# saholmes/stark-mlwe

Measured on AMD Instinct MI355X. Metric: prove ms + Fr-NTT achieved GB/s, 2^20/2^24 trace at 1/2/4/8 GPUs, higher is better.
Workload: dtype u256 (4x u64 Montgomery limbs, Pallas Fr); 1 GPU; one 2^20-row trace x 4 columns (2^20 rows per GPU), blowup 8: LDE (iNTT + coset NTT) + DEEP-ALI merge + FRI folds + Poseidon leaf hashes + Poseidon-Merkle trees (schedule [16,16,8]), kernels only; log_trace_per_gpu=20, log_blowup=3, field=pallas_fr

## Files before the change

stark_mlwe_amd/csrc/capi_core.hip:

```cpp
#include <algorithm>
#include <cstring>
#include "poseidon_launch.hpp"
#include "pow_table.hpp"

using namespace stark;

namespace stark {

static int32_t pool_poison_fill(stark_ctx* ctx, void* p, size_t bytes) {
    STARK_HIP(ctx, hipMemsetAsync(p, ctx->opt.pool_poison, bytes, ctx->stream));
    STARK_HIP(ctx, hipStreamSynchronize(ctx->stream));
    return STARK_OK;
}

int32_t ctx_scratch(stark_ctx* ctx, size_t bytes, void** out) {
    if (bytes > ctx->scratch_bytes) {
        if (ctx->scratch) STARK_HIP(ctx, hipStreamSynchronize(ctx->stream));
        ctx->scratch_bytes = 0; STARK_HIP(ctx, ctx->scratch.alloc(bytes)); ctx->scratch_bytes = bytes;
    }
    if (ctx->opt.pool_poison >= 0 && ctx->scratch_bytes) STARK_TRY(pool_poison_fill(ctx, ctx->scratch.p, ctx->scratch_bytes));
    *out = ctx->scratch.p; return STARK_OK;
}

int32_t ctx_upload_staged(stark_ctx* ctx, void* dst, const void* src, size_t bytes) {
    if (!bytes) return STARK_OK;
    auto& q = ctx->staged;
    for (size_t i = 0; i < q.size();) {
        if (hipEventQuery(q[i].done) == hipSuccess) { (void)hipEventDestroy(q[i].done); q[i] = std::move(q.back()); q.pop_back(); } else ++i;
    }
    (void)hipGetLastError();
    stark_ctx::StagedUpload u; u.host.reset(new uint8_t[bytes]); memcpy(u.host.get(), src, bytes);
    STARK_HIP(ctx, hipEventCreateWithFlags(&u.done, hipEventDisableTiming));
    const uint8_t* from = u.host.get();
    q.push_back(std::move(u));
    STARK_HIP(ctx, hipMemcpyAsync(dst, from, bytes, hipMemcpyHostToDevice, ctx->stream));
    STARK_HIP(ctx, hipEventRecord(q.back().done, ctx->stream));
    return STARK_OK;
}

static inline size_t pool_round(size_t bytes) {
    if (bytes < 256) return 256;
    if (bytes <= (1u << 20)) { size_t r = 256; while (r < bytes) r <<= 1; return r; }
    return (bytes + (1u << 20) - 1) & ~(size_t)((1u << 20) - 1);
}
int32_t ctx_alloc(stark_ctx* ctx, size_t bytes, void** out) {
    const size_t sz = pool_round(bytes);
    auto it = ctx->pool_free.find(sz);
    if (it != ctx->pool_free.end() && !it->second.empty()) {
        void* p = it->second.back(); it->second.pop_back(); ctx->pool_cached_bytes -= sz;
        ctx->pool_live[p] = sz; *out = p;
        return ctx->opt.pool_poison >= 0 ? pool_poison_fill(ctx, p, sz) : STARK_OK;
    }
    void* p = nullptr; hipError_t e = hipMalloc(&p, sz);
    if (e != hipSuccess) {
        (void)hipGetLastError();
        (void)hipStreamSynchronize(ctx->stream);
        for (auto& kv : ctx->pool_free) { for (void* q : kv.second) (void)hipFree(q); kv.second.clear(); }
        ctx->pool_cached_bytes = 0;
        e = hipMalloc(&p, sz);
        if (e != hipSuccess) { (void)hipGetLastError(); return ctx->fail(STARK_ERR_OOM, "device allocation of " + std::to_string(sz) + " bytes failed"); }
    }
    ctx->pool_live[p] = sz; *out = p;
    return ctx->opt.pool_poison >= 0 ? pool_poison_fill(ctx, p, sz) : STARK_OK;
}
void ctx_release(stark_ctx* ctx, void* p) {
    if (!p || !ctx) return;
    auto it = ctx->pool_live.find(p);
    if (it == ctx->pool_live.end()) { ctx->err = "ctx_release: the pointer is not a live block of this context's pool (left alone)"; return; }
    const size_t sz = it->second; ctx->pool_live.erase(it);
    ctx->pool_free[sz].push_back(p); ctx->pool_cached_bytes += sz;
}
int32_t ctx_enter(stark_ctx* ctx) {
    if (!ctx) return STARK_ERR_INVALID_ARG;
    int cur = -1;
    if (hipGetDevice(&cur) != hipSuccess || cur != ctx->device) STARK_HIP(ctx, hipSetDevice(ctx->device));
    return STARK_OK;
}

int32_t ctx_side_stream(stark_ctx* ctx, hipStream_t* out) {
    if (!ctx->side_stream) { STARK_HIP(ctx, hipStreamCreateWithFlags(&ctx->side_stream, hipStreamNonBlocking)); STARK_HIP(ctx, hipEventCreateWithFlags(&ctx->ev_fork, hipEventDisableTiming)); }
    *out = ctx->side_stream; return STARK_OK;
}
int32_t ctx_fork(stark_ctx* ctx, hipStream_t* side) {
    STARK_TRY(ctx_side_stream(ctx, side));
    if (hipEventRecord(ctx->ev_fork, ctx->stream) != hipSuccess || hipStreamWaitEvent(*side, ctx->ev_fork, 0) != hipSuccess) return ctx->fail(STARK_ERR_HIP, "fork");
    return STARK_OK;
}
int32_t ctx_join(stark_ctx* ctx) {
    if (hipEventRecord(ctx->ev_fork, ctx->side_stream) != hipSuccess || hipStreamWaitEvent(ctx->stream, ctx->ev_fork, 0) != hipSuccess) return ctx->fail(STARK_ERR_HIP, "join");
    return STARK_OK;
}

static int32_t params_finish(stark_ctx* ctx, stark_params* P) {
    if (host::rp_for_width(P->ref.t) < 0) return ctx->fail(STARK_ERR_UNSUPPORTED, "Poseidon width must be one of 9,17,33,65,129");
    P->kc = host::make_kernel_consts(P->ref);
    if (!P->kc.ok) return ctx->fail(STARK_ERR_UNSUPPORTED, "MDS matrix has a singular leading minor: LU/sparse kernel form unavailable");
    const host::KernelConsts& k = P->kc;
    std::vector<fr_t> blob; auto put = [&](const std::vector<fr_t>& v) { size_t off = blob.size(); blob.insert(blob.end(), v.begin(), v.end()); return off; };
    size_t o_rcf = put(k.rc_full), o_rcp = put(k.rc_partial), o_lu = put(k.lu), o_pre = put(k.lu_pre), o_row0 = put(k.row0), o_sp = put(k.sparse), o_mds = put(k.mds), o_mpre = put(k.mds_pre), o_gam = put(k.gamma);
    const size_t o_29 = blob.size();
    { std::vector<uint32_t> w29; for (auto* v : {&k.lu29, &k.lu_pre29, &k.row0_29, &k.sparse29, &k.gamma29, &k.mds29, &k.mds_pre29, &k.chain_a, &k.chain_g, &k.chain_w, &k.rc_full29}) w29.insert(w29.end(), v->begin(), v->end());
      while (w29.size() % 8) w29.push_back(0);
      blob.resize(o_29 + w29.size() / 8); memcpy((void*)(blob.data() + o_29), w29.data(), w29.size() * 4); }
    const size_t o_frag = blob.size(), frag_elems = (k.mds_frag.size() + sizeof(fr_t) - 1) / sizeof(fr_t);
    if (!k.mds_frag.empty()) { blob.resize(o_frag + 2 * frag_elems); memcpy((void*)(blob.data() + o_frag), k.mds_frag.data(), k.mds_frag.size()); memcpy((void*)(blob.data() + o_frag + frag_elems), k.mds_pre_frag.data(), k.mds_pre_frag.size()); }
    const size_t o_b8 = blob.size(), ef_elems = (k.blk8s_efrag.size() + sizeof(fr_t) - 1) / sizeof(fr_t), lf_bytes = k.blk8s_lfrag.size() + 1024, lf_elems = (lf_bytes + sizeof(fr_t) - 1) / sizeof(fr_t),
                 gf_elems = (k.blk8s_gfrag.size() + sizeof(fr_t) - 1) / sizeof(fr_t), rcs_elems = k.rc_partial_scaled.size(), un_elems = (k.blk8_unscale29.size() * 4 + sizeof(fr_t) - 1) / sizeof(fr_t);
    const bool have_b8 = !k.blk8s_efrag.empty();
    if (have_b8) { blob.resize(o_b8 + ef_elems + lf_elems + gf_elems + rcs_elems + un_elems);
                   int8_t* const b8 = (int8_t*)(blob.data() + o_b8);
                   memcpy(b8, k.blk8s_efrag.data(), k.blk8s_efrag.size());
                   memcpy(b8 + ef_elems * sizeof(fr_t), k.blk8s_lfrag.data(), k.blk8s_lfrag.size()); memcpy(b8 + ef_elems * sizeof(fr_t) + k.blk8s_lfrag.size(), k.blk8_lfrag.data() + k.blk8_lfrag.size() - 1024, 1024);
                   memcpy(b8 + (ef_elems + lf_elems) * sizeof(fr_t), k.blk8s_gfrag.data(), k.blk8s_gfrag.size());
                   memcpy(b8 + (ef_elems + lf_elems + gf_elems) * sizeof(fr_t), k.rc_partial_scaled.data(), rcs_elems * sizeof(fr_t));
                   memcpy(b8 + (ef_elems + lf_elems + gf_elems + rcs_elems) * sizeof(fr_t), k.blk8_unscale29.data(), k.blk8_unscale29.size() * 4); }
    STARK_TRY(P->blob.fill_sync(ctx, blob.data(), blob.size() * sizeof(fr_t)));
    fr_t* const dev = P->blob.fr();
    P->dev.t = k.t; P->dev.rf = k.rf; P->dev.rp = k.rp;
    P->dev.rc_full = dev + o_rcf; P->dev.rc_partial = dev + o_rcp; P->dev.lu = dev + o_lu; P->dev.lu_pre = dev + o_pre;
    P->dev.row0 = dev + o_row0; P->dev.sparse = dev + o_sp; P->dev.mds = dev + o_mds; P->dev.mds_pre = dev + o_mpre; P->dev.gamma = dev + o_gam;
    { const uint32_t* b29 = reinterpret_cast<const uint32_t*>(dev + o_29);
      P->dev.lu29 = b29; P->dev.lu_pre29 = b29 + k.lu29.size(); P->dev.row0_29 = P->dev.lu_pre29 + k.lu_pre29.size();
      P->dev.sparse29 = P->dev.row0_29 + k.row0_29.size(); P->dev.gamma29 = P->dev.sparse29 + k.sparse29.size();
      P->dev.mds29 = P->dev.gamma29 + k.gamma29.size(); P->dev.mds_pre29 = P->dev.mds29 + k.mds29.size();
      const uint32_t* ch = P->dev.mds_pre29 + k.mds_pre29.size();
      P->dev.chain_a = k.chain_a.empty() ? nullptr : ch; P->dev.chain_g = k.chain_a.empty() ? nullptr : ch + k.chain_a.size(); P->dev.chain_w = k.chain_a.empty() ? nullptr : ch + k.chain_a.size() + k.chain_g.size();
      P->dev.rc_full29 = ch + k.chain_a.size() + k.chain_g.size() + k.chain_w.size(); }
    P->dev.blk8_efrag = have_b8 ? (const void*)(dev + o_b8) : nullptr; P->dev.blk8_lfrag = have_b8 ? (const void*)(dev + o_b8 + ef_elems) : nullptr;
    P->dev.blk8_gfrag = have_b8 ? (const void*)(dev + o_b8 + ef_elems + lf_elems) : nullptr;
    P->dev.blk8_unit_frag = have_b8 ? (const void*)((const int8_t*)P->dev.blk8_lfrag + k.blk8s_lfrag.size()) : nullptr;
    P->dev.rc_partial_scaled = have_b8 ? dev + o_b8 + ef_elems + lf_elems + gf_elems : nullptr;
    P->dev.mds_frag = k.mds_frag.empty() ? nullptr : (const void*)(dev + o_frag); P->dev.mds_pre_frag = k.mds_frag.empty() ? nullptr : (const void*)(dev + o_frag + frag_elems);
    return STARK_OK;
}
static int32_t params_from_consts(stark_ctx* ctx, const host::PoseidonConsts& c, std::unique_ptr<stark_params>& out) {
    std::unique_ptr<stark_params> P(new stark_params()); P->ctx = ctx; P->ref = c;
    STARK_TRY(params_finish(ctx, P.get()));
    out = std::move(P); return STARK_OK;
}
static int32_t params_for_caller(stark_ctx* ctx, const host::PoseidonConsts& c, stark_params** out) {
    std::unique_ptr<stark_params> P; STARK_TRY(params_from_consts(ctx, c, P));
    P->ref_.bind(ctx); *out = P.release(); return STARK_OK;
}
int32_t ctx_transcript_params(stark_ctx* ctx, stark_params** out) {
    if (!ctx->tparams) STARK_TRY(params_from_consts(ctx, host::consts_transcript(), ctx->tparams));
    if (out) *out = ctx->tparams.get();
    return STARK_OK;
}
int32_t ctx_merkle_params(stark_ctx* ctx, int t, stark_params** out) {
    auto it = ctx->merkle_params.find(t);
    if (it == ctx->merkle_params.end()) {
        if (host::rp_for_width(t) < 0) return ctx->fail(STARK_ERR_UNSUPPORTED, "unsupported Poseidon width");
        std::unique_ptr<stark_params> P; STARK_TRY(params_from_consts(ctx, host::consts_for_width(t), P));
        *out = P.get(); ctx->merkle_params[t] = std::move(P); return STARK_OK;
    }
    *out = it->second.get(); return STARK_OK;
}
int32_t ctx_commit_params(stark_ctx* ctx, stark_params** out) {
    std::unique_ptr<stark_params>& slot = ctx->merkle_params[-17];
    if (!slot) STARK_TRY(params_from_consts(ctx, host::derive_consts("POSEIDON-T17-X5-SEED", 17, 8, 64), slot));
    *out = slot.get(); return STARK_OK;
}

}

extern "C" {

int32_t stark_version(void) { return 1; }

int32_t stark_ctx_create(int32_t device, void* stream, stark_ctx_t** out) {
    if (!out) return STARK_ERR_INVALID_ARG;
    int ndev = 0;
    if (hipGetDeviceCount(&ndev) != hipSuccess || ndev <= 0 || device < 0 || device >= ndev) return STARK_ERR_HIP;
    if (hipSetDevice(device) != hipSuccess) return STARK_ERR_HIP;
    std::unique_ptr<stark_ctx> c(new stark_ctx()); c->device = device;
    if (stream == STARK_STREAM_PRIVATE) { if (hipStreamCreateWithFlags(&c->stream, hipStreamNonBlocking) != hipSuccess) return STARK_ERR_HIP; c->own_stream = true; }
    else { c->stream = (hipStream_t)stream; c->own_stream = false; }
    if (hipEventCreate(&c->ev0) != hipSuccess || hipEventCreate(&c->ev1) != hipSuccess) return STARK_ERR_HIP;
    { int cus = 0; if (hipDeviceGetAttribute(&cus, hipDeviceAttributeMultiprocessorCount, device) == hipSuccess && cus > 0) c->num_cus = cus; }
    stark::ntt_set_attrs();
    stark::poseidon_set_attrs();
    *out = c.release(); return STARK_OK;
}
}
static void ctx_teardown(stark_ctx* ctx) {
    (void)hipSetDevice(ctx->device); (void)hipStreamSynchronize(ctx->stream);
    stark::comm_destroy(ctx);
    stark::ntt_plans_free(ctx);
    for (auto& kv : ctx->pool_free) for (void* q : kv.second) (void)hipFree(q);
    for (auto& kv : ctx->pool_live) (void)hipFree(kv.first);
    if (ctx->pinned) (void)hipHostFree(ctx->pinned);
    for (auto& u : ctx->staged) (void)hipEventDestroy(u.done);
    if (ctx->ev0) (void)hipEventDestroy(ctx->ev0); if (ctx->ev1) (void)hipEventDestroy(ctx->ev1);
    if (ctx->side_stream) (void)hipStreamDestroy(ctx->side_stream);
    if (ctx->ev_fork) (void)hipEventDestroy(ctx->ev_fork);
    if (ctx->own_stream) (void)hipStreamDestroy(ctx->stream);
    delete ctx;
}
namespace stark {
void ctx_ref(stark_ctx* c) { ++c->live_handles; }
void ctx_unref(stark_ctx* c) { if (--c->live_handles == 0 && c->destroy_pending) ctx_teardown(c); }
}
extern "C" {
int32_t stark_ctx_destroy(stark_ctx_t* ctx) {
    if (!ctx) return STARK_ERR_INVALID_ARG;
    if (ctx->destroy_pending) return STARK_ERR_INVALID_ARG;
    STARK_TRY(ctx_enter(ctx));
    (void)hipStreamSynchronize(ctx->stream);
    if (ctx->live_handles > 0) { ctx->destroy_pending = true; return STARK_OK; }
    ctx_teardown(ctx); return STARK_OK;
}
int32_t stark_ctx_sync(stark_ctx_t* ctx) { if (!ctx) return STARK_ERR_INVALID_ARG; STARK_TRY(ctx_enter(ctx)); STARK_HIP(ctx, hipStreamSynchronize(ctx->stream)); return STARK_OK; }
int32_t stark_ctx_trim(stark_ctx_t* ctx) {
    if (!ctx) return STARK_ERR_INVALID_ARG; STARK_TRY(ctx_enter(ctx));
    STARK_HIP(ctx, hipStreamSynchronize(ctx->stream));
    for (auto& kv : ctx->pool_free) { for (void* q : kv.second) (void)hipFree(q); kv.second.clear(); }
    ctx->pool_cached_bytes = 0;
    stark::ntt_plans_free(ctx);
    ctx->scratch.reset(); ctx->scratch_bytes = 0;
    return STARK_OK;
}
size_t stark_ctx_cached_bytes(stark_ctx_t* ctx) { return ctx ? ctx->pool_cached_bytes : 0; }
}
struct OptionDef { const char* key; const char* (*set)(stark_ctx::Options&, int64_t); };
static const OptionDef kOptions[] = {
    {"ntt_direct_max_log", [](stark_ctx::Options& o, int64_t v) -> const char* { if (v < 0 || v > 30) return "0..30"; o.ntt_direct_max_log = (int)v; return nullptr; }},
    {"ntt_merged_coset", [](stark_ctx::Options& o, int64_t v) -> const char* { o.ntt_merged_coset = v != 0; return nullptr; }},
    {"ntt_log_tile", [](stark_ctx::Options& o, int64_t v) -> const char* { if (v != -1 && (v < 8 || v > 12)) return "8..12, or -1 for the default"; o.ntt_log_tile_forced = v != -1; o.ntt_log_tile = v == -1 ? 11 : (int)v; return nullptr; }},
    {"ntt_min_waves", [](stark_ctx::Options& o, int64_t v) -> const char* { if (v != 2 && v != 4) return "2 or 4"; o.ntt_min_waves = (int)v; return nullptr; }},
    {"poseidon_lane_only", [](stark_ctx::Options& o, int64_t v) -> const char* { o.poseidon_lane_only = v != 0; return nullptr; }},
    {"sponge_one_wave", [](stark_ctx::Options& o, int64_t v) -> const char* { o.sponge_one_wave = v != 0; return nullptr; }},
    {"sponge_debug", [](stark_ctx::Options& o, int64_t v) -> const char* { o.sponge_debug = (int)v; return nullptr; }},
    {"merkle_node16_pair", [](stark_ctx::Options& o, int64_t v) -> const char* { o.merkle_node16_pair = v != 0; return nullptr; }},
    {"poseidon_block8", [](stark_ctx::Options& o, int64_t v) -> const char* { o.poseidon_block8 = v != 0; return nullptr; }},
    {"merkle_wave_pair", [](stark_ctx::Options& o, int64_t v) -> const char* { o.merkle_wave_pair = v != 0; return nullptr; }},
    {"fri_side_pair", [](stark_ctx::Options& o, int64_t v) -> const char* { o.fri_side_pair = v != 0; return nullptr; }},
    {"sumcheck_verify_batch_max_slots", [](stark_ctx::Options& o, int64_t v) -> const char* { if (v < 1) return "at least 1"; o.sumcheck_verify_batch_max_slots = (size_t)v; return nullptr; }},
    {"ntt_batch_max_elems", [](stark_ctx::Options& o, int64_t v) -> const char* { if (v < 1 || v > ((int64_t)1 << 28)) return "1..2^28"; o.ntt_batch_max_elems = (size_t)v; return nullptr; }},
    {"prove_batch_max_rows", [](stark_ctx::Options& o, int64_t v) -> const char* { if (v < 1 || v > ((int64_t)1 << 28)) return "1..2^28"; o.prove_batch_max_rows = (size_t)v; return nullptr; }},
    {"mle_log_tile", [](stark_ctx::Options& o, int64_t v) -> const char* { if (v != -1 && (v < 3 || v > 12)) return "3..12, or -1 for the default"; o.mle_log_tile = (int)v; return nullptr; }},
    {"mle_lane_contiguous", [](stark_ctx::Options& o, int64_t v) -> const char* { if (v < -1 || v > 1) return "0 or 1, or -1 for the default"; o.mle_lane_contiguous = (int)v; return nullptr; }},
    {"lagrange_max_partials", [](stark_ctx::Options& o, int64_t v) -> const char* { if (v != -1 && (v < 1 || v > ((int64_t)1 << 28))) return "1..2^28, or -1 for the default"; o.lagrange_max_partials = v == -1 ? (size_t)1 << 21 : (size_t)v; return nullptr; }},
    {"lagrange_wide_acc", [](stark_ctx::Options& o, int64_t v) -> const char* { if (v < -1 || v > 1) return "0 or 1, or -1 for the default"; o.lagrange_wide_acc = (int)v; return nullptr; }},
    {"lagrange_col_groups", [](stark_ctx::Options& o, int64_t v) -> const char* { if (v != -1 && (v < 1 || v > 65535)) return "1..65535, or -1 for automatic"; o.lagrange_col_groups = (int)v; return nullptr; }},
    {"pool_poison", [](stark_ctx::Options& o, int64_t v) -> const char* { if (v < -1 || v > 255) return "0..255, or -1 for off"; o.pool_poison = (int)v; return nullptr; }},
};
extern "C" {
int32_t stark_ctx_set_option(stark_ctx_t* ctx, const char* key, int64_t value) {
    if (!ctx || !key) return STARK_ERR_INVALID_ARG;
    STARK_TRY(ctx_enter(ctx));
    const std::string k(key);
    const OptionDef* def = nullptr; std::string known;
    for (const OptionDef& d : kOptions) { if (k == d.key) def = &d; known += (known.empty() ? "" : ", ") + std::string(d.key); }
    if (!def) return ctx->fail(STARK_ERR_INVALID_ARG, "unknown option '" + k + "' (" + known + ")");
    if (const char* range = def->set(ctx->opt, value)) return ctx->fail(STARK_ERR_INVALID_ARG, k + ": " + range);
    STARK_HIP(ctx, hipStreamSynchronize(ctx->stream));
    stark::ntt_plans_free(ctx);
    return STARK_OK;
}
const char* stark_last_error(stark_ctx_t* ctx) { return ctx ? ctx->err.c_str() : "null context"; }
int32_t stark_malloc(stark_ctx_t* ctx, size_t bytes, void** dptr) { if (!ctx || !dptr) return STARK_ERR_INVALID_ARG; STARK_TRY(ctx_enter(ctx)); STARK_HIP(ctx, hipMalloc(dptr, bytes ? bytes : 32)); return STARK_OK; }
int32_t stark_free(stark_ctx_t* ctx, void* dptr) { if (!ctx) return STARK_ERR_INVALID_ARG; STARK_TRY(ctx_enter(ctx)); STARK_HIP(ctx, hipStreamSynchronize(ctx->stream)); STARK_HIP(ctx, hipFree(dptr)); return STARK_OK; }
int32_t stark_memcpy_h2d(stark_ctx_t* ctx, void* d, const void* s, size_t bytes) {
    if (!ctx) return STARK_ERR_INVALID_ARG;
    STARK_TRY(ctx_enter(ctx));
    return DevMem::fill_sync(ctx, d, s, bytes); }
int32_t stark_memcpy_d2h(stark_ctx_t* ctx, void* d, const void* s, size_t bytes) {
    if (!ctx) return STARK_ERR_INVALID_ARG;
    STARK_TRY(ctx_enter(ctx));
    STARK_HIP(ctx, hipMemcpyAsync(d, s, bytes, hipMemcpyDeviceToHost, ctx->stream)); STARK_HIP(ctx, hipStreamSynchronize(ctx->stream)); return STARK_OK; }
int32_t stark_timer_start(stark_ctx_t* ctx) { if (!ctx) return STARK_ERR_INVALID_ARG; STARK_HIP(ctx, hipEventRecord(ctx->ev0, ctx->stream)); return STARK_OK; }
int32_t stark_timer_stop_ms(stark_ctx_t* ctx, float* ms) {
    if (!ctx || !ms) return STARK_ERR_INVALID_ARG;
    STARK_TRY(ctx_enter(ctx));
    STARK_HIP(ctx, hipEventRecord(ctx->ev1, ctx->stream)); STARK_HIP(ctx, hipEventSynchronize(ctx->ev1)); STARK_HIP(ctx, hipEventElapsedTime(ms, ctx->ev0, ctx->ev1)); return STARK_OK; }

}
#define STARK_DIAG_ITERS 2048
static __global__ void __launch_bounds__(1024) k_diag_mac_rate(uint32_t* out, uint32_t seed) {
    uint32_t a0 = seed + threadIdx.x, a1 = a0 * 3 + 1, a2 = a0 * 5 + 2, a3 = a0 * 7 + 3, a4 = a0 * 9 + 4, a5 = a0 * 11 + 5, a6 = a0 * 13 + 6, a7 = a0 * 15 + 7;
    uint64_t d0 = a0, d1 = a1, d2 = a2, d3 = a3, d4 = a4, d5 = a5, d6 = a6, d7 = a7; const uint32_t b = seed | 1;
#define STARK_DIAG_MAD(i) asm volatile("v_mad_u64_u32 %0, vcc, %1, %2, %0" : "+v"(d##i) : "v"(a##i), "v"(b) : "vcc");
    for (int i = 0; i < STARK_DIAG_ITERS; ++i) { STARK_DIAG_MAD(0) STARK_DIAG_MAD(1) STARK_DIAG_MAD(2) STARK_DIAG_MAD(3) STARK_DIAG_MAD(4) STARK_DIAG_MAD(5) STARK_DIAG_MAD(6) STARK_DIAG_MAD(7) }
#undef STARK_DIAG_MAD
// ... 52 lines not shown
```

stark_mlwe_amd/csrc/capi_poseidon.hip:

```cpp
#include <algorithm>
#include <cstring>
#include <type_traits>
#include "poseidon_launch.hpp"
#include "poseidon_dev.hpp"
#include "poseidon_pair.hpp"
#include "poseidon_coop.hpp"
#include "poseidon_chain.hpp"
#include "poseidon_wave.hpp"
#include "poseidon_transcript.hpp"
#include "fri_dev.hpp"
#include "merkle_batch.hpp"

using namespace stark;

static const size_t kMaxLds = 160 * 1024;
static inline int poseidon_block(int t) { return (size_t)t * 32 * 64 <= kMaxLds ? 64 : 32; }
static inline size_t poseidon_lds(int t, int block) { return (size_t)t * 32 * block; }
enum class PoseidonForm { Lane, WavePair, OneWave, FiveWave, Wide };
enum class PoseidonOp { MerkleLevel, LeafLayer, TrHash, ColumnSponges, RaggedSponges, DeviceTranscript };
constexpr size_t kChainMaxNodes = 256, kChainMaxLeaves = 2048, kChainMaxSponges = 512, kCoopMaxNodes = 4096, kCoopMaxLeaves = 4096, kCoopMaxSponges = 4096;
static PoseidonForm poseidon_form(const stark_ctx* ctx, const stark_params* p, PoseidonOp op, size_t n) {
    const PoseidonDev& d = p->dev;
    const bool lane_only = ctx->opt.poseidon_lane_only, one_wave = ctx->opt.sponge_one_wave;
    const bool chain = !lane_only && !one_wave && d.t == 17 && d.rf == 8 && d.rp == 64 && d.chain_a;
// ... 35 lines not shown
        stark_params* tp = nullptr; STARK_TRY(ctx_transcript_params(ctx, &tp));
        const host::PoseidonConsts& c = tp->ref;
        fr_t blob[17 + 51 + 40];
        for (auto& x : blob) x = host::h_zero();
        for (int j = 0; j < 17; ++j) blob[j] = init[j];
        fr_t x[17]; for (int j = 0; j < 17; ++j) x[j] = fr_pow5<PallasFr>(host::h_add(init[j], c.rc_full[j]));
        for (int i = 0; i < 17; ++i) {
            fr_t k = host::h_zero();
            for (int j = 0; j < 17; ++j) if (j != 4 && j != 5) k = host::h_add(k, host::h_mul(c.mds[(size_t)i * 17 + j], x[j]));
            blob[17 + i] = k; blob[34 + i] = c.mds[(size_t)i * 17 + 4]; blob[51 + i] = c.mds[(size_t)i * 17 + 5];
            uint32_t* m45 = reinterpret_cast<uint32_t*>(&blob[68]);
            const fr_t k20 = fr_from_u64<PallasFr>(1ull << FR29_SBOX_SHIFT);
            fr29_const_from<PallasFr>(host::h_mul(c.mds[(size_t)i * 17 + 4], k20), m45 + 9 * i); fr29_const_from<PallasFr>(host::h_mul(c.mds[(size_t)i * 17 + 5], k20), m45 + 9 * (17 + i));
        }
        DevMem d; STARK_TRY(d.fill_sync(ctx, blob, sizeof(blob)));
        ctx->leaf_init = std::move(d);
    }
    *out = ctx->leaf_init.fr(); return STARK_OK;
}

namespace stark {

static int32_t tr_frame(stark_ctx* ctx, const char* tag, fr_t** dev, int* np, int* ns) {
    const std::string key(tag);
    auto it = ctx->tr_frames.find(key);
    if (it == ctx->tr_frames.end()) {
        std::vector<fr_t> fr; const int p = host::tr_hash_frame(tag, fr);
        DevMem d; STARK_TRY(d.fill_sync(ctx, fr.data(), fr.size() * sizeof(fr_t)));
        it = ctx->tr_frames.emplace(key, std::move(d)).first; ctx->tr_frame_dims[key] = {p, (int)fr.size() - p};
    }
    *dev = it->second.fr(); *np = ctx->tr_frame_dims[key].first; *ns = ctx->tr_frame_dims[key].second; return STARK_OK;
}
static int32_t launch_tr_hash(stark_ctx* ctx, stark_params* tp, PoseidonForm form, const TrStream& T, fr_t* out_dev) {
    const bool ragged = T.layout == TrStream::Ragged;
    switch (form) {
    case PoseidonForm::FiveWave:
        if (ragged) hipLaunchKernelGGL(k_tr_hash_chain_ragged, dim3((unsigned)T.n), dim3(320), chain_lds_bytes(), ctx->stream, tp->dev, T, row_consts_of(ctx), out_dev);
        else hipLaunchKernelGGL(k_tr_hash_chain, dim3((unsigned)T.n), dim3(320), chain_lds_bytes(), ctx->stream, tp->dev, T, row_consts_of(ctx), out_dev);
        break;
    case PoseidonForm::OneWave:
        if (ragged) hipLaunchKernelGGL((k_tr_hash_coop<true, true>), dim3((unsigned)T.n), dim3(64), coop_lds_bytes(17), ctx->stream, tp->dev, T, out_dev);
        else if (T.layout == TrStream::Equal) hipLaunchKernelGGL(k_tr_hash_coop<false>, dim3((unsigned)T.n), dim3(64), coop_lds_bytes(17), ctx->stream, tp->dev, T, out_dev);
        else hipLaunchKernelGGL(k_tr_hash_coop<true>, dim3((unsigned)T.n), dim3(64), coop_lds_bytes(17), ctx->stream, tp->dev, T, out_dev);
        break;
    default: {
        const int block = 64;
        if (ragged) hipLaunchKernelGGL(k_tr_hash_ragged, dim3((unsigned)((T.n + block - 1) / block)), dim3(block), poseidon_lds(17, block), ctx->stream, tp->dev, T, out_dev);
        else hipLaunchKernelGGL(k_tr_hash, dim3((unsigned)((T.n + block - 1) / block)), dim3(block), poseidon_lds(17, block), ctx->stream, tp->dev, T, out_dev);
    } }
    STARK_HIP(ctx, hipGetLastError());
    return STARK_OK;
}
int32_t tr_hash_dev(stark_ctx* ctx, const char* tag, const fr_t* fields_dev, size_t k, size_t n, fr_t* out_dev) {
    stark_params* tp = nullptr; STARK_TRY(ctx_transcript_params(ctx, &tp));
    fr_t* frame = nullptr; int np = 0, ns = 0; STARK_TRY(tr_frame(ctx, tag, &frame, &np, &ns));
    if (n == 0) return STARK_OK;
    const TrStream T = TrStream::equal(frame, np, ns, fields_dev, k, n, host::h_tag("FSv1-TRANSCRIPT-INIT"));
    return launch_tr_hash(ctx, tp, poseidon_form(ctx, tp, PoseidonOp::TrHash, n), T, out_dev);
}
static int32_t tr_hash_columns(stark_ctx* ctx, const char* const tags[4], const fr_t* const cols[4], const fr_t* const* ptrs_dev, size_t nblocks, size_t n0, fr_t* out_dev) {
    stark_params* tp = nullptr; STARK_TRY(ctx_transcript_params(ctx, &tp));
    TrStream T{}; T.layout = ptrs_dev ? TrStream::BatchColumns : TrStream::Columns; T.n = nblocks; T.batch = ptrs_dev; T.cap = host::h_tag("FSv1-TRANSCRIPT-INIT");
    for (int c = 0; c < 4; ++c) {
        fr_t* frame = nullptr; int np = 0, ns = 0; STARK_TRY(tr_frame(ctx, tags[c], &frame, &np, &ns));
        T.prefix[c] = frame; T.np[c] = np; T.suffix[c] = frame + np; T.ns[c] = ns; T.fields[c] = cols ? cols[c] : nullptr; T.k[c] = n0;
    }
    return launch_tr_hash(ctx, tp, poseidon_form(ctx, tp, PoseidonOp::ColumnSponges, nblocks), T, out_dev);
}
int32_t tr_hash_columns4_dev(stark_ctx* ctx, const char* const tags[4], const fr_t* const cols[4], size_t n0, fr_t* out4_dev) {
    return tr_hash_columns(ctx, tags, cols, nullptr, 4, n0, out4_dev);
}
int32_t tr_hash_columns_batch_dev(stark_ctx* ctx, const char* const tags[4], const fr_t* const* ptrs_dev, size_t batch, size_t n0, fr_t* out_dev) {
    return tr_hash_columns(ctx, tags, nullptr, ptrs_dev, 4 * batch, n0, out_dev);
}
int32_t tr_hash_many_dev(stark_ctx* ctx, size_t n, const char* const* tags, const fr_t* const* fields, const size_t* k, fr_t* out_dev, bool column_sponges) {
    stark_params* tp = nullptr; STARK_TRY(ctx_transcript_params(ctx, &tp));
    std::vector<TrFrameRef> fr(n);
    for (size_t i = 0; i < n; ++i) { fr_t* frame = nullptr; STARK_TRY(tr_frame(ctx, tags[i], &frame, &fr[i].np, &fr[i].ns)); fr[i].frame = frame; }
    if (n == 0) return STARK_OK;
    if (n > 0x7fffffffu) return ctx->fail(STARK_ERR_UNSUPPORTED, "tr_hash_many: more than 2^31 - 1 items in one call");
    const std::vector<TrStream::Item> items = tr_ragged_items(fr.data(), fields, k, n);
    DevBuf d; STARK_HIP(ctx, d.alloc(ctx, n * sizeof(TrStream::Item))); STARK_TRY(ctx_upload_staged(ctx, d.p, items.data(), n * sizeof(TrStream::Item)));
    const TrStream T = tr_ragged_stream((const TrStream::Item*)d.p, n, host::h_tag("FSv1-TRANSCRIPT-INIT"));
    return launch_tr_hash(ctx, tp, poseidon_form(ctx, tp, column_sponges ? PoseidonOp::ColumnSponges : PoseidonOp::RaggedSponges, n), T, out_dev);
}
int32_t tr_hash_host1(stark_ctx* ctx, const char* tag, const std::vector<fr_t>& fields, fr_t* out) {
    DevBuf in, o; STARK_HIP(ctx, in.alloc(ctx, fields.size() * sizeof(fr_t))); STARK_HIP(ctx, o.alloc(ctx, sizeof(fr_t)));
    STARK_TRY(ctx_upload_staged(ctx, in.p, fields.data(), fields.size() * sizeof(fr_t)));
    STARK_TRY(tr_hash_dev(ctx, tag, in.fr(), fields.size(), 1, o.fr()));
    STARK_HIP(ctx, o.download_sync(out, sizeof(fr_t)));
    return STARK_OK;
}
int32_t tr_stream_on(stark_ctx* ctx, stark_params* tp, fr_t* state, uint32_t* pos, const fr_t* fields, size_t n, bool finish, fr_t* out) {
    if (poseidon_form(ctx, tp, PoseidonOp::DeviceTranscript, 1) == PoseidonForm::FiveWave)
        hipLaunchKernelGGL(k_tr_stream_chain, dim3(1), dim3(320), chain_lds_bytes(), ctx->stream, tp->dev, row_consts_of(ctx), state, pos, fields, (uint64_t)n, finish ? 1 : 0, finish ? out : (fr_t*)nullptr);
    else
        hipLaunchKernelGGL(k_tr_stream, dim3(1), dim3(64), coop_lds_bytes(17), ctx->stream, tp->dev, state, pos, fields, (uint64_t)n, finish ? 1 : 0, finish ? out : (fr_t*)nullptr);
    STARK_HIP(ctx, hipGetLastError()); return STARK_OK;
}
int32_t tr_batch_on(stark_ctx* ctx, stark_params* tp, const TrBatchStream& T, size_t n_for_form) {
    if (!T.n_active) return STARK_OK;
    if (poseidon_form(ctx, tp, PoseidonOp::DeviceTranscript, n_for_form) == PoseidonForm::FiveWave)
        for (uint32_t sg = 0; sg < (uint32_t)T.nseg; ++sg)
            hipLaunchKernelGGL(k_tr_batch_chain, dim3((unsigned)T.n_active), dim3(320), chain_lds_bytes(), ctx->stream, tp->dev, row_consts_of(ctx), T, sg);
    else
        hipLaunchKernelGGL(k_tr_batch, dim3((unsigned)T.n_active), dim3(64), coop_lds_bytes(17), ctx->stream, tp->dev, T);
    STARK_HIP(ctx, hipGetLastError()); return STARK_OK;
}

}

extern "C" {

int32_t stark_poseidon_permute_batch_dev(stark_ctx_t* ctx, stark_params_t* p, uint64_t* states, size_t n) {
    if (!ctx || !p || (!states && n)) return STARK_ERR_INVALID_ARG;
    STARK_TRY(ctx_enter(ctx));
    if (!n) return STARK_OK;
    const int block = poseidon_block(p->dev.t);
    hipLaunchKernelGGL(k_permute_batch, dim3((unsigned)((n + block - 1) / block)), dim3(block), poseidon_lds(p->dev.t, block), ctx->stream, p->dev, as_fr(states), n);
    STARK_HIP(ctx, hipGetLastError()); return STARK_OK;
}
int32_t stark_poseidon_permute_batch(stark_ctx_t* ctx, stark_params_t* p, uint64_t* states, size_t n) {
    if (!ctx || !p || (!states && n)) return STARK_ERR_INVALID_ARG;
    STARK_TRY(ctx_enter(ctx));
    size_t bytes = n * p->dev.t * sizeof(fr_t); DevBuf d; CallerUploads up(ctx); STARK_HIP(ctx, up.up(d, states, bytes));
    STARK_TRY(stark_poseidon_permute_batch_dev(ctx, p, (uint64_t*)d.p, n));
    STARK_HIP(ctx, up.download_sync(states, d.p, bytes));
    return STARK_OK;
}
static int32_t hash_stream(stark_ctx_t* ctx, stark_params_t* p, int mode, const uint64_t* a, size_t na, const uint64_t* b, size_t nb, const fr_t& tag, size_t n, uint64_t* out) {
    DevBuf da, db, dout; CallerUploads up(ctx);
    STARK_HIP(ctx, up.up(da, a, n * na * sizeof(fr_t))); STARK_HIP(ctx, up.up(db, b, n * nb * sizeof(fr_t))); STARK_HIP(ctx, dout.alloc(ctx, n * sizeof(fr_t)));
    const int block = poseidon_block(p->dev.t);
    hipLaunchKernelGGL(k_hash_stream, dim3((unsigned)((n + block - 1) / block)), dim3(block), poseidon_lds(p->dev.t, block), ctx->stream, p->dev, mode, da.fr(), na, db.fr(), nb, tag, n, dout.fr());
    STARK_HIP(ctx, hipGetLastError());
    STARK_HIP(ctx, up.download_sync(out, dout.p, n * sizeof(fr_t)));
    return STARK_OK;
}
int32_t stark_poseidon_hash_with_ds_dynamic(stark_ctx_t* ctx, stark_params_t* p, const uint64_t* ds, size_t nds, const uint64_t* in, size_t cnt, size_t n, uint64_t* out) {
    if (!ctx || !p || !out || (!ds && nds) || (!in && cnt)) return STARK_ERR_INVALID_ARG;
    STARK_TRY(ctx_enter(ctx));
    if (!n) return STARK_OK;
    return hash_stream(ctx, p, 0, ds, nds, in, cnt, host::h_zero(), n, out);
}
int32_t stark_poseidon_hash_with_ds(stark_ctx_t* ctx, stark_params_t* p, const uint64_t* in, size_t cnt, const uint64_t* ds_tag, uint64_t* out) {
    if (!ctx || !p || !out || !ds_tag || (!in && cnt)) return STARK_ERR_INVALID_ARG;
    STARK_TRY(ctx_enter(ctx));
    if (p->dev.t != 17) return ctx->fail(STARK_ERR_INVALID_ARG, "hash_with_ds is the fixed t=17 sponge");
    return hash_stream(ctx, p, 1, nullptr, 0, in, cnt, load_fr(ds_tag), 1, out);
}
}
static int32_t pair_block8_form(stark_ctx* ctx, const stark_params* p, bool* on) {
    *on = ctx->opt.poseidon_block8 && p->dev.t == 17 && p->dev.rp % 8 == 0;
    if (*on && (!p->dev.blk8_efrag || !p->dev.blk8_lfrag || !p->dev.blk8_unit_frag || !p->dev.blk8_gfrag || !p->dev.rc_partial_scaled)) return ctx->fail(STARK_ERR_UNSUPPORTED, "poseidon_block8: the parameter set has no block-8 tables");
    return STARK_OK;
}
template <class DS>
static int32_t launch_ds(stark_ctx_t* ctx, hipStream_t st, stark_params_t* p, const DS& D, fr_t* out) {
    if (!D.n_out) return STARK_OK;
    const int t = p->dev.t; const unsigned nodes = (unsigned)D.n_out, pairs = (unsigned)((D.n_out + 63) / 64);
    bool b8 = false; STARK_TRY(pair_block8_form(ctx, p, &b8));
    switch (poseidon_form(ctx, p, PoseidonOp::MerkleLevel, D.n_out)) {
    case PoseidonForm::FiveWave: hipLaunchKernelGGL(k_hash_ds_chain<DS>, dim3(nodes), dim3(320), chain_lds_bytes(), st, p->dev, D, row_consts_of(ctx), out); break;
    case PoseidonForm::OneWave:
        if (t == 17) hipLaunchKernelGGL((k_hash_ds_coop<17, DS>), dim3(nodes), dim3(64), coop_lds_bytes(17), st, p->dev, D, out);
        else hipLaunchKernelGGL((k_hash_ds_coop<9, DS>), dim3(nodes), dim3(64), coop_lds_bytes(9), st, p->dev, D, out);
        break;
    case PoseidonForm::WavePair:
        if constexpr (std::is_same<DS, DsStream>::value) {
            if (t == 17 && ctx->opt.merkle_node16_pair && D.mode == 0 && D.arity == 16 && D.n_in == 16 * D.n_out) {
                if (b8) hipLaunchKernelGGL(k_node16_pair<true>, dim3(pairs), dim3(128), pair_lds_bytes(17), st, p->dev, D.arity_f, D.level_f, D.label_f, D.pos0, D.in0, D.n_out, out);
                else hipLaunchKernelGGL(k_node16_pair<false>, dim3(pairs), dim3(128), pair_lds_bytes(17), st, p->dev, D.arity_f, D.level_f, D.label_f, D.pos0, D.in0, D.n_out, out);
                break;
            }
        }
        if (t == 17 && b8) hipLaunchKernelGGL((k_hash_ds2<17, DS, true>), dim3(pairs), dim3(128), pair_lds_bytes(17), st, p->dev, D, out);
        else if (t == 17) hipLaunchKernelGGL((k_hash_ds2<17, DS>), dim3(pairs), dim3(128), pair_lds_bytes(17), st, p->dev, D, out);
        else hipLaunchKernelGGL((k_hash_ds2<9, DS>), dim3(pairs), dim3(128), pair_lds_bytes(9), st, p->dev, D, out);
        break;
    case PoseidonForm::Wide:
        if (t == 33) hipLaunchKernelGGL((k_hash_ds_wave<33, DS>), dim3(nodes), dim3(64), wave_lds_bytes(t), st, p->dev, D, out);
        else if (t == 65) hipLaunchKernelGGL((k_hash_ds_wave<65, DS>), dim3(nodes), dim3(64), wave_lds_bytes(t), st, p->dev, D, out);
        else hipLaunchKernelGGL((k_hash_ds_wave<129, DS>), dim3(nodes), dim3(64), wave_lds_bytes(t), st, p->dev, D, out);
        break;
    case PoseidonForm::Lane: {
        const int block = poseidon_block(t);
        hipLaunchKernelGGL(k_hash_ds<DS>, dim3((unsigned)((D.n_out + block - 1) / block)), dim3(block), poseidon_lds(t, block), st, p->dev, D, out);
    } }
    STARK_HIP(ctx, hipGetLastError()); return STARK_OK;
}
int32_t stark::hash_ds_on(stark_ctx* ctx, hipStream_t st, stark_params* p, const DsStream& D, fr_t* out) { return launch_ds(ctx, st, p, D, out); }
int32_t stark::hash_ds_on(stark_ctx* ctx, hipStream_t st, stark_params* p, const DsGatherStream& D, fr_t* out) { return launch_ds(ctx, st, p, D, out); }
int32_t stark::hash_ds_on(stark_ctx* ctx, hipStream_t st, stark_params* p, const DsBatchStream& D, fr_t* out) { return launch_ds(ctx, st, p, D, out); }
int32_t stark::hash_ds_on(stark_ctx* ctx, hipStream_t st, stark_params* p, const DsBatchPairStream& D, fr_t* out) { return launch_ds(ctx, st, p, D, out); }
int32_t stark::hash_ds_on(stark_ctx* ctx, hipStream_t st, stark_params* p, const DsBatchPairPtrStream& D, fr_t* out) { return launch_ds(ctx, st, p, D, out); }
static void lds_attr(const void* kernel) { (void)hipFuncSetAttribute(kernel, hipFuncAttributeMaxDynamicSharedMemorySize, (int)kMaxLds); }
template <class DS>
static void ds_attrs() {
    lds_attr((const void*)k_hash_ds<DS>); lds_attr((const void*)k_hash_ds2<17, DS>); lds_attr((const void*)k_hash_ds2<17, DS, true>); lds_attr((const void*)k_hash_ds2<9, DS>); lds_attr((const void*)k_hash_ds_chain<DS>);
}
void stark::poseidon_set_attrs() {
    ds_attrs<DsStream>(); ds_attrs<DsGatherStream>(); ds_attrs<DsBatchStream>(); ds_attrs<DsBatchPairStream>(); ds_attrs<DsBatchPairPtrStream>();
    for (const void* k : {(const void*)k_leaf_pair, (const void*)k_permute_batch, (const void*)k_tr_hash, (const void*)k_hash_stream, (const void*)k_leaf_pair2<false>, (const void*)k_leaf_pair2<true>, (const void*)k_node16_pair<false>, (const void*)k_node16_pair<true>,
                          (const void*)k_tr_hash_chain, (const void*)k_tr_hash_chain_ragged, (const void*)k_tr_hash_ragged, (const void*)k_leaf_pair_chain, (const void*)k_tr_stream_chain, (const void*)k_tr_batch_chain})
        lds_attr(k);
}
extern "C" {
int32_t stark_poseidon_hash_ds_batch_dev(stark_ctx_t* ctx, stark_params_t* p, size_t arity, uint32_t level, uint64_t pos0, uint64_t label, const uint64_t* in, size_t n_in, uint64_t* out) {
    if (!ctx || !p || !in || !out || arity == 0) return STARK_ERR_INVALID_ARG;
    STARK_TRY(ctx_enter(ctx));
    if (host::width_for_arity(arity) != p->dev.t) return ctx->fail(STARK_ERR_INVALID_ARG, "arity incompatible with Poseidon width");
    STARK_TRY(ctx_enter(ctx));
    return hash_ds_on(ctx, ctx->stream, p, DsStream::make(0, arity, level, pos0, label, as_fr(in), nullptr, n_in), as_fr(out));
}
int32_t stark_poseidon_hash_ds_batch(stark_ctx_t* ctx, stark_params_t* p, size_t arity, uint32_t level, uint64_t pos0, uint64_t label, const uint64_t* in, size_t n_in, uint64_t* out) {
    if (!ctx || !p || !in || !out || arity == 0) return STARK_ERR_INVALID_ARG;
    STARK_TRY(ctx_enter(ctx));
    size_t n_out = (n_in + arity - 1) / arity; DevBuf di, dout; CallerUploads up(ctx); STARK_HIP(ctx, up.up(di, in, n_in * sizeof(fr_t))); STARK_HIP(ctx, dout.alloc(ctx, n_out * sizeof(fr_t)));
    STARK_TRY(stark_poseidon_hash_ds_batch_dev(ctx, p, arity, level, pos0, label, (const uint64_t*)di.p, n_in, (uint64_t*)dout.p));
    STARK_HIP(ctx, up.download_sync(out, dout.p, n_out * sizeof(fr_t)));
    return STARK_OK;
}
}
namespace stark {
static bool same_consts(const host::PoseidonConsts& a, const host::PoseidonConsts& b) {
    if (a.t != b.t || a.rf != b.rf || a.rp != b.rp || a.mds.size() != b.mds.size() || a.rc_full.size() != b.rc_full.size() || a.rc_partial.size() != b.rc_partial.size()) return false;
    for (size_t i = 0; i < a.mds.size(); ++i) if (!fr_eq(a.mds[i], b.mds[i])) return false;
    for (size_t i = 0; i < a.rc_full.size(); ++i) if (!fr_eq(a.rc_full[i], b.rc_full[i])) return false;
    for (size_t i = 0; i < a.rc_partial.size(); ++i) if (!fr_eq(a.rc_partial[i], b.rc_partial[i])) return false;
    return true;
}
int32_t leaf_pair_hash_on(stark_ctx* ctx, hipStream_t st, const fr_t* f, const fr_t* f_next, size_t n, size_t m, fr_t* h) {
    if (!n) return STARK_OK;
    stark_params* tp = nullptr; STARK_TRY(ctx_transcript_params(ctx, &tp));
    fr_t* init = nullptr; STARK_TRY(ctx_leaf_init(ctx, &init));
    const LeafStream L{init, f, f_next, m, n};
    bool b8 = false; STARK_TRY(pair_block8_form(ctx, tp, &b8));
    switch (poseidon_form(ctx, tp, PoseidonOp::LeafLayer, n)) {
    case PoseidonForm::FiveWave: hipLaunchKernelGGL(k_leaf_pair_chain, dim3((unsigned)n), dim3(320), chain_lds_bytes(), st, tp->dev, row_consts_of(ctx), L, h); break;
    case PoseidonForm::OneWave: hipLaunchKernelGGL(k_leaf_pair_coop, dim3((unsigned)n), dim3(64), coop_lds_bytes(17), st, tp->dev, L, h); break;
    case PoseidonForm::WavePair:
        if (b8) hipLaunchKernelGGL(k_leaf_pair2<true>, dim3((unsigned)((n + 63) / 64)), dim3(128), pair_lds_bytes(17), st, tp->dev, init + 17, f, f_next, n, m, h);
        else hipLaunchKernelGGL(k_leaf_pair2<false>, dim3((unsigned)((n + 63) / 64)), dim3(128), pair_lds_bytes(17), st, tp->dev, init + 17, f, f_next, n, m, h);
        break;
    default: hipLaunchKernelGGL(k_leaf_pair, dim3((unsigned)((n + 63) / 64)), dim3(64), poseidon_lds(17, 64), st, tp->dev, L, h);
    }
    STARK_HIP(ctx, hipGetLastError()); return STARK_OK;
}
}
extern "C" {
int32_t stark_leaf_pair_hash_dev(stark_ctx_t* ctx, stark_params_t* tp, const uint64_t* f, const uint64_t* f_next, size_t n, size_t m, uint64_t* h) {
    if (!ctx || (!f && n) || (!h && n) || m == 0) return STARK_ERR_INVALID_ARG;
    STARK_TRY(ctx_enter(ctx));
    if (tp) {
        if (tp->dev.t != 17) return ctx->fail(STARK_ERR_INVALID_ARG, "leaf hash uses the t=17 transcript permutation");
        stark_params* mine = nullptr; STARK_TRY(ctx_transcript_params(ctx, &mine));
        if (tp != mine && !same_consts(tp->ref, mine->ref)) return ctx->fail(STARK_ERR_INVALID_ARG, "hash_leaf_pair is defined over transcript::default_params(); the handle holds other constants");
    }
    return leaf_pair_hash_on(ctx, ctx->stream, as_fr(f), as_fr(f_next), n, m, as_fr(h));
}
int32_t stark_leaf_pair_hash(stark_ctx_t* ctx, stark_params_t* tp, const uint64_t* f, const uint64_t* f_next, size_t n, size_t m, uint64_t* h) {
    if (!ctx || (!f && n) || (!h && n) || m == 0) return STARK_ERR_INVALID_ARG;
    STARK_TRY(ctx_enter(ctx));
    size_t nn = f_next ? (n + m - 1) / m : 0; DevBuf df, dn, dh; CallerUploads up(ctx);
    STARK_HIP(ctx, up.up(df, f, n * sizeof(fr_t))); STARK_HIP(ctx, up.up(dn, f_next, nn * sizeof(fr_t))); STARK_HIP(ctx, dh.alloc(ctx, n * sizeof(fr_t)));
    STARK_TRY(stark_leaf_pair_hash_dev(ctx, tp, (const uint64_t*)df.p, f_next ? (const uint64_t*)dn.p : nullptr, n, m, (uint64_t*)dh.p));
    STARK_HIP(ctx, up.download_sync(h, dh.p, n * sizeof(fr_t))); return STARK_OK;
}
int32_t stark_tr_hash_fields_tagged_dev(stark_ctx_t* ctx, stark_params_t* tp, const char* tag, const uint64_t* fields, size_t k, size_t n, uint64_t* out) {
    if (!ctx || !tag || (!fields && k && n) || (!out && n)) return STARK_ERR_INVALID_ARG;
    STARK_TRY(ctx_enter(ctx));
    (void)tp;
    return tr_hash_dev(ctx, tag, as_fr(fields), k, n, as_fr(out));
}
int32_t stark_tr_hash_fields_tagged(stark_ctx_t* ctx, stark_params_t* tp, const char* tag, const uint64_t* fields, size_t k, size_t n, uint64_t* out) {
    if (!ctx || !tag || (!fields && k && n) || (!out && n)) return STARK_ERR_INVALID_ARG;
    STARK_TRY(ctx_enter(ctx));
    DevBuf di, dout; CallerUploads up(ctx); STARK_HIP(ctx, up.up(di, fields, n * k * sizeof(fr_t))); STARK_HIP(ctx, dout.alloc(ctx, n * sizeof(fr_t)));
    STARK_TRY(stark_tr_hash_fields_tagged_dev(ctx, tp, tag, (const uint64_t*)di.p, k, n, (uint64_t*)dout.p));
    STARK_HIP(ctx, up.download_sync(out, dout.p, n * sizeof(fr_t))); return STARK_OK;
}
int32_t stark_tr_hash_many_dev(stark_ctx_t* ctx, size_t n, const char* const* tags, const uint64_t* const* fields, const size_t* k, uint64_t* out) {
    if (!ctx) return STARK_ERR_INVALID_ARG;
    if (!n) return STARK_OK;
    if (!tags || !k || !out) return STARK_ERR_INVALID_ARG;
    STARK_TRY(ctx_enter(ctx));
    const uintptr_t o0 = (uintptr_t)out, o1 = o0 + n * sizeof(fr_t);
    for (size_t i = 0; i < n; ++i) {
        if (!tags[i]) return ctx->fail(STARK_ERR_INVALID_ARG, "tr_hash_many: null tag " + std::to_string(i));
        if (!k[i]) continue;
        if (!fields || !fields[i]) return ctx->fail(STARK_ERR_INVALID_ARG, "tr_hash_many: null fields with k > 0, item " + std::to_string(i));
        const uintptr_t f0 = (uintptr_t)fields[i];
        if (f0 < o1 && o0 < f0 + k[i] * sizeof(fr_t)) return ctx->fail(STARK_ERR_INVALID_ARG, "tr_hash_many: out overlaps the fields of item " + std::to_string(i));
    }
    return tr_hash_many_dev(ctx, n, tags, reinterpret_cast<const fr_t* const*>(fields), k, as_fr(out), false);
}

}
namespace stark {
int32_t merkle_build_on(stark_ctx* ctx, hipStream_t st, stark_params* p, size_t arity, uint64_t label, const fr_t* leaves, size_t n, int pairs, const fr_t* cp, size_t cp_div,
                        uint64_t first_pos, uint32_t level0, size_t stop_at_len, DevBuf&& level0_block, std::unique_ptr<stark_tree>& out) {
    if (n == 0) return ctx->fail(STARK_ERR_INVALID_ARG, "no leaves");
    if (host::width_for_arity(arity) != p->dev.t) return ctx->fail(STARK_ERR_INVALID_ARG, "arity incompatible with Poseidon width");
    if (arity == 1 && n > 1) return ctx->fail(STARK_ERR_UNSUPPORTED, "arity 1 with more than one leaf never terminates in the reference");
    std::unique_ptr<stark_tree> T(new stark_tree(ctx, p, arity, label));
    auto add_level = [&](DevBuf&& b, size_t len) { T->levels.push_back(b.fr()); T->lens.push_back(len); T->blocks.push_back(std::move(b)); };
    const bool moved_in = level0_block.p && !pairs;
// ... 178 lines not shown
```

stark_mlwe_amd/csrc/fr29.hpp:

```cpp
#pragma once
#include "fr.hpp"

namespace stark {

constexpr uint32_t FR_M29 = (1u << 29) - 1;
struct fr29_t { uint32_t l[9]; };
struct fr_wide29 { uint64_t c[18]; };

template <class F> constexpr uint32_t fr_p29(int i) {
    const int lo = 29 * i, w = lo >> 5, s = lo & 31;
    const uint64_t x = (w < 8 ? (uint64_t)F::P(w) : 0ull) | (w + 1 < 8 ? ((uint64_t)F::P(w + 1) << 32) : 0ull);
    return (uint32_t)(x >> s) & FR_M29;
}

template <class F> constexpr int fr29_max_terms() {
    int nz = 0;
    for (int j = 1; j < 9; ++j) nz += fr_p29<F>(j) != 0 ? 1 : 0;
    return (64 - (nz + 1)) / 8;
}

FR_HD fr29_t fr29_unpack(const fr_t& x) {
    fr29_t r;
#pragma unroll
    for (int i = 0; i < 9; ++i) {
        const int lo = 29 * i, w = lo >> 5, s = lo & 31;
        uint32_t v = x.v[w] >> s;
        if (s > 3 && w + 1 < 8) v |= x.v[w + 1] << (32 - s);
        r.l[i] = v & FR_M29;
    }
    return r;
}
FR_HD void fr_wide29_zero(fr_wide29& w) {
#pragma unroll
    for (int k = 0; k < 18; ++k) w.c[k] = 0;
}
FR_HD void fr_wide29_mac(fr_wide29& w, const uint32_t* __restrict__ a_, const fr29_t& b) {
#if defined(__HIP_DEVICE_COMPILE__)
    typedef const __attribute__((address_space(4))) uint32_t* cptr_t;
    cptr_t a = (cptr_t)a_;
#else
    const uint32_t* a = a_;
#endif
#pragma unroll
    for (int i = 0; i < 9; ++i) {
        const uint32_t ai = a[i];
#pragma unroll
        for (int j = 0; j < 9; ++j) w.c[i + j] += (uint64_t)ai * b.l[j];
    }
}
FR_HD void fr_wide29_mac_regs(fr_wide29& w, const uint32_t* a, const fr29_t& b) {
#pragma unroll
    for (int i = 0; i < 9; ++i)
#pragma unroll
        for (int j = 0; j < 9; ++j) w.c[i + j] += (uint64_t)a[i] * b.l[j];
}
FR_HD void fr_wide29_norm(fr_wide29& w) {
#pragma unroll
    for (int k = 0; k < 17; ++k) { w.c[k + 1] += w.c[k] >> 29; w.c[k] &= FR_M29; }
}
template <class F, bool MAC_POW2 = false> FR_HD void fr_wide29_mont(fr_wide29& w, uint32_t* l) {
    uint32_t pj[9];
#pragma unroll
    for (int j = 1; j < 9; ++j) pj[j] = fr_p29<F>(j);
#if defined(__HIP_DEVICE_COMPILE__)
    if (MAC_POW2) {
#pragma unroll
        for (int j = 1; j < 9; ++j) if (fr_p29<F>(j) != 0 && (fr_p29<F>(j) & (fr_p29<F>(j) - 1)) == 0) asm("" : "+v"(pj[j]));
    }
#endif
#pragma unroll
    for (int k = 0; k < 9; ++k) {
        const uint64_t t = w.c[k];
        const uint32_t m = (0u - (uint32_t)t) & FR_M29;
        w.c[k + 1] += (t + FR_M29) >> 29;
#pragma unroll
        for (int j = 1; j < 9; ++j)
            if (fr_p29<F>(j) != 0) w.c[k + j] += (uint64_t)m * pj[j];
    }
    uint64_t carry = 0;
#pragma unroll
    for (int i = 0; i < 9; ++i) { const uint64_t v = w.c[9 + i] + carry; l[i] = i < 8 ? ((uint32_t)v & FR_M29) : (uint32_t)v; carry = v >> 29; }
}
template <class F> FR_HD fr_t fr29_pack_reduce(const uint32_t* l) {
    uint32_t t[9];
#pragma unroll
    for (int wd = 0; wd < 8; ++wd) {
        const int lo = 32 * wd, i = lo / 29, s = lo - 29 * i;
        uint32_t v = l[i] >> s;
        if (i + 1 < 9) v |= l[i + 1] << (29 - s);
        if (29 - s + 29 < 32 && i + 2 < 9) v |= l[i + 2] << (58 - s);
        t[wd] = v;
    }
    t[8] = 0;
    fr_cond_sub<F>(t, t[8]);
    fr_t z;
#pragma unroll
    for (int i = 0; i < 8; ++i) z.v[i] = t[i];
    return z;
}
template <class F> FR_HD fr_t fr_wide29_reduce_lazy(fr_wide29& w) {
    uint32_t l[9]; fr_wide29_mont<F>(w, l);
    fr_t z;
#pragma unroll
    for (int wd = 0; wd < 8; ++wd) {
        const int lo = 32 * wd, i = lo / 29, s = lo - 29 * i;
        uint32_t v = l[i] >> s;
        if (i + 1 < 9) v |= l[i + 1] << (29 - s);
        if (29 - s + 29 < 32 && i + 2 < 9) v |= l[i + 2] << (58 - s);
        z.v[wd] = v;
    }
    return z;
}
template <class F, bool MAC_POW2 = false> FR_HD fr_t fr_wide29_reduce(fr_wide29& w) {
    uint32_t l[9]; fr_wide29_mont<F, MAC_POW2>(w, l);
    return fr29_pack_reduce<F>(l);
}
template <class F> FR_HD void lazy_reduce29(fr29_t& a) {
    const uint32_t q = a.l[8] >> 22; const int64_t k = q ? (int64_t)q - 1 : 0;
    int64_t carry = 0;
#pragma unroll
    for (int i = 0; i < 9; ++i) {
        const int64_t d = (int64_t)a.l[i] - k * (int64_t)fr_p29<F>(i) + carry;
        if (i < 8) { a.l[i] = (uint32_t)d & FR_M29; carry = d >> 29; } else a.l[8] = (uint32_t)d;
    }
}
template <class F> FR_HD fr_t fr29_canon_lazy(fr29_t v) {
    lazy_reduce29<F>(v);
    fr_t z = fr29_pack_reduce<F>(v.l);
    fr_cond_sub<F>(z.v, 0u);
    return z;
}

template <class F, bool MAC_POW2 = false> FR_HD fr29_t fr29_sqr_mont(const fr29_t& a) {
    fr_wide29 w; fr_wide29_zero(w);
#pragma unroll
    for (int i = 0; i < 9; ++i) {
        w.c[2 * i] += (uint64_t)a.l[i] * a.l[i];
#pragma unroll
        for (int j = i + 1; j < 9; ++j) w.c[i + j] += (uint64_t)a.l[i] * (a.l[j] << 1);
    }
    fr29_t r; fr_wide29_mont<F, MAC_POW2>(w, r.l); return r;
}
template <class F, bool MAC_POW2 = false> FR_HD fr29_t fr29_mul_mont(const fr29_t& a, const fr29_t& b) {
    fr_wide29 w; fr_wide29_zero(w);
#pragma unroll
    for (int i = 0; i < 9; ++i)
#pragma unroll
        for (int j = 0; j < 9; ++j) w.c[i + j] += (uint64_t)a.l[i] * b.l[j];
    fr29_t r; fr_wide29_mont<F, MAC_POW2>(w, r.l); return r;
}
constexpr int FR29_SBOX_SHIFT = 20;
template <class F> FR_HD fr_t fr_pow5_r29(const fr_t& x) {
    const fr29_t u = fr29_unpack(x);
    const fr29_t x2 = fr29_sqr_mont<F>(u), x4 = fr29_sqr_mont<F>(x2), x5 = fr29_mul_mont<F>(u, x4);
    return fr29_pack_reduce<F>(x5.l);
}

FR_HD void fr29_norm(fr29_t& a) {
#pragma unroll
    for (int i = 0; i < 8; ++i) { a.l[i + 1] += a.l[i] >> 29; a.l[i] &= FR_M29; }
}
template <class F> FR_HD void fr29_partial_reduce(fr29_t& x) {
    constexpr uint64_t d = (uint64_t)fr_p29<F>(8) + 1, magic = ((1ull << 52) + d - 1) / d;
    fr29_norm(x);
    const uint32_t q = (uint32_t)(((uint64_t)x.l[8] * magic) >> 52);
    int64_t carry = 0;
#pragma unroll
    for (int i = 0; i < 9; ++i) {
        const int64_t t = (int64_t)x.l[i] + carry - (int64_t)((uint64_t)q * fr_p29<F>(i));
        if (i < 8) { x.l[i] = (uint32_t)t & FR_M29; carry = t >> 29; } else x.l[8] = (uint32_t)t;
    }
}
template <class F> FR_HD void ntt29_butterfly(fr29_t& a, fr29_t& b, const fr29_t& tw, const uint32_t* __restrict__ D, bool norm) {
    if (norm) { fr29_norm(a); fr29_norm(b); }
    const fr29_t p = fr29_mul_mont<F, true>(tw, b);
#pragma unroll
    for (int k = 0; k < 9; ++k) { const uint32_t av = a.l[k]; a.l[k] = av + p.l[k]; b.l[k] = av + D[k] - p.l[k]; }
}
template <class F, bool FRESH> FR_HD void ntt29_butterfly_w1(fr29_t& a, fr29_t& b, const uint32_t* __restrict__ D) {
    if (!FRESH) fr29_partial_reduce<F>(b);
#pragma unroll
    for (int k = 0; k < 9; ++k) { const uint32_t av = a.l[k], bv = b.l[k]; a.l[k] = av + bv; b.l[k] = av + D[k] - bv; }
}
template <class F, int HEAD> FR_HD void ntt29_head(fr29_t (&x)[1 << HEAD], const fr29_t& w1, const fr29_t& w2, const fr29_t& w3, const uint32_t* __restrict__ D) {
#pragma unroll
    for (int g = 0; g < (1 << (HEAD - 1)); ++g) ntt29_butterfly_w1<F, true>(x[2 * g], x[2 * g + 1], D);
    if constexpr (HEAD >= 2) {
#pragma unroll
        for (int g = 0; g < (1 << (HEAD - 2)); ++g) {
            ntt29_butterfly_w1<F, false>(x[4 * g], x[4 * g + 2], D);
            ntt29_butterfly<F>(x[4 * g + 1], x[4 * g + 3], w2, D, false);
        }
    }
    if constexpr (HEAD == 3) {
        ntt29_butterfly_w1<F, false>(x[0], x[4], D);
        ntt29_butterfly<F>(x[1], x[5], w1, D, false);
        ntt29_butterfly<F>(x[2], x[6], w2, D, false);
        ntt29_butterfly<F>(x[3], x[7], w3, D, false);
    }
}
FR_HD bool ntt29_norm_before(int s) { return s > 1 && (s - 1) % 3 == 0; }
FR_HD bool ntt29_norm_after(int stages) { return stages >= 1 && (stages - 1) % 3 == 2; }
template <class F> inline void ntt29_offset(uint32_t D[9]) {
    uint64_t cy = 0; uint32_t c[9];
    for (int i = 0; i < 9; ++i) { const uint64_t v = (uint64_t)fr_p29<F>(i) * 4 + cy; c[i] = i < 8 ? (uint32_t)(v & FR_M29) : (uint32_t)v; cy = v >> 29; }
    for (int i = 0; i < 9; ++i) D[i] = c[i] + (i < 8 ? (1u << 29) : 0u) - (i > 0 ? 1u : 0u);
}

template <class F> inline void fr29_const_from(const fr_t& c_R, uint32_t out[9]) {
    const fr_t c32 = fr_mul_portable<F>(c_R, fr_from_u64<F>(32));
    const fr29_t u = fr29_unpack(c32);
    for (int i = 0; i < 9; ++i) out[i] = u.l[i];
}

}
```

stark_mlwe_amd/csrc/host_util.hpp:

```cpp
#pragma once
#include <cstdint>
#include <cstring>
#include <string>
#include <vector>
#include "fr.hpp"
#include "fr29.hpp"

namespace stark {
namespace host {

struct Blake3 {
    static constexpr uint32_t kIV[8] = {0x6A09E667u, 0xBB67AE85u, 0x3C6EF372u, 0xA54FF53Au, 0x510E527Fu, 0x9B05688Cu, 0x1F83D9ABu, 0x5BE0CD19u};
    enum : uint32_t { F_CHUNK_START = 1, F_CHUNK_END = 2, F_PARENT = 4, F_ROOT = 8 };
    static uint32_t ror(uint32_t x, unsigned n) { return (x >> n) | (x << (32 - n)); }
    static void mix(uint32_t* v, int a, int b, int c, int d, uint32_t x, uint32_t y) {
        v[a] += v[b] + x; v[d] = ror(v[d] ^ v[a], 16); v[c] += v[d]; v[b] = ror(v[b] ^ v[c], 12);
        v[a] += v[b] + y; v[d] = ror(v[d] ^ v[a], 8);  v[c] += v[d]; v[b] = ror(v[b] ^ v[c], 7);
    }
    static void compress(const uint32_t h[8], const uint8_t block[64], uint32_t blen, uint64_t ctr, uint32_t flags, uint32_t out[16]) {
        static const uint8_t sched[7][16] = {
            {0, 1, 2, 3, 4, 5, 6, 7, 8, 9, 10, 11, 12, 13, 14, 15}, {2, 6, 3, 10, 7, 0, 4, 13, 1, 11, 12, 5, 9, 14, 15, 8},
            {3, 4, 10, 12, 13, 2, 7, 14, 6, 5, 9, 0, 11, 15, 8, 1}, {10, 7, 12, 9, 14, 3, 13, 15, 4, 0, 11, 2, 5, 8, 1, 6},
            {12, 13, 9, 11, 15, 10, 14, 8, 7, 2, 5, 3, 0, 1, 6, 4}, {9, 14, 11, 5, 8, 12, 15, 1, 13, 3, 0, 10, 2, 6, 4, 7},
            {11, 15, 5, 0, 1, 9, 8, 6, 14, 10, 2, 12, 3, 4, 7, 13}};
// ... 2 lines not shown
        for (int i = 0; i < 8; ++i) v[i] = h[i];
        for (int i = 0; i < 4; ++i) v[8 + i] = kIV[i];
        v[12] = (uint32_t)ctr; v[13] = (uint32_t)(ctr >> 32); v[14] = blen; v[15] = flags;
        for (int r = 0; r < 7; ++r) {
            const uint8_t* s = sched[r];
            mix(v, 0, 4, 8, 12, m[s[0]], m[s[1]]);   mix(v, 1, 5, 9, 13, m[s[2]], m[s[3]]);
            mix(v, 2, 6, 10, 14, m[s[4]], m[s[5]]);  mix(v, 3, 7, 11, 15, m[s[6]], m[s[7]]);
            mix(v, 0, 5, 10, 15, m[s[8]], m[s[9]]);  mix(v, 1, 6, 11, 12, m[s[10]], m[s[11]]);
            mix(v, 2, 7, 8, 13, m[s[12]], m[s[13]]); mix(v, 3, 4, 9, 14, m[s[14]], m[s[15]]);
        }
        for (int i = 0; i < 8; ++i) { out[i] = v[i] ^ v[i + 8]; out[i + 8] = v[i + 8] ^ h[i]; }
    }
    struct Node { uint32_t h[8]; uint8_t block[64]; uint32_t blen; uint64_t ctr; uint32_t flags; };
    static void cv_of(const Node& n, uint32_t extra, uint32_t cv[8]) { uint32_t o[16]; compress(n.h, n.block, n.blen, n.ctr, n.flags | extra, o); memcpy(cv, o, 32); }
    static Node chunk_node(const uint8_t* p, size_t len, uint64_t index) {
        Node n; memcpy(n.h, kIV, 32); n.ctr = index;
        size_t off = 0; bool first = true;
        while (len - off > 64) {
            uint32_t o[16]; compress(n.h, p + off, 64, index, first ? F_CHUNK_START : 0, o); memcpy(n.h, o, 32);
            off += 64; first = false;
        }
        memset(n.block, 0, 64); memcpy(n.block, p + off, len - off); n.blen = (uint32_t)(len - off);
        n.flags = (first ? F_CHUNK_START : 0) | F_CHUNK_END;
        return n;
    }
    static Node subtree(const uint8_t* p, size_t len, uint64_t index) {
        if (len <= 1024) return chunk_node(p, len, index);
        size_t chunks = (len + 1023) / 1024, left = 1; while (left * 2 < chunks) left *= 2;
        Node l = subtree(p, left * 1024, index), r = subtree(p + left * 1024, len - left * 1024, index + left);
        Node n; memcpy(n.h, kIV, 32); n.ctr = 0; n.blen = 64; n.flags = F_PARENT;
        uint32_t a[8], b[8]; cv_of(l, 0, a); cv_of(r, 0, b);
        for (int i = 0; i < 8; ++i) for (int j = 0; j < 4; ++j) { n.block[4 * i + j] = (uint8_t)(a[i] >> (8 * j)); n.block[32 + 4 * i + j] = (uint8_t)(b[i] >> (8 * j)); }
        return n;
    }
    static void hash(const uint8_t* p, size_t len, uint8_t out[32]) {
        Node root = subtree(p, len, 0);
        if (root.flags & F_PARENT) root.ctr = 0;
        uint32_t cv[8]; cv_of(root, F_ROOT, cv);
        for (int i = 0; i < 8; ++i) for (int j = 0; j < 4; ++j) out[4 * i + j] = (uint8_t)(cv[i] >> (8 * j));
    }
};

struct ChaCha12Rng {
    uint32_t st[16]; uint32_t out[16]; unsigned have = 0;
    explicit ChaCha12Rng(const uint8_t seed[32]) {
        st[0] = 0x61707865u; st[1] = 0x3320646eu; st[2] = 0x79622d32u; st[3] = 0x6b206574u;
        for (int i = 0; i < 8; ++i) st[4 + i] = (uint32_t)seed[4 * i] | (uint32_t)seed[4 * i + 1] << 8 | (uint32_t)seed[4 * i + 2] << 16 | (uint32_t)seed[4 * i + 3] << 24;
        st[12] = st[13] = st[14] = st[15] = 0;
    }
    static uint32_t rol(uint32_t x, unsigned n) { return (x << n) | (x >> (32 - n)); }
    void block() {
        uint32_t x[16]; memcpy(x, st, 64);
        auto Q = [&](int a, int b, int c, int d) {
            x[a] += x[b]; x[d] = rol(x[d] ^ x[a], 16); x[c] += x[d]; x[b] = rol(x[b] ^ x[c], 12);
            x[a] += x[b]; x[d] = rol(x[d] ^ x[a], 8);  x[c] += x[d]; x[b] = rol(x[b] ^ x[c], 7); };
        for (int i = 0; i < 6; ++i) { Q(0, 4, 8, 12); Q(1, 5, 9, 13); Q(2, 6, 10, 14); Q(3, 7, 11, 15); Q(0, 5, 10, 15); Q(1, 6, 11, 12); Q(2, 7, 8, 13); Q(3, 4, 9, 14); }
        for (int i = 0; i < 16; ++i) out[i] = x[i] + st[i];
        if (++st[12] == 0) ++st[13];
        have = 16;
    }
    uint32_t next_u32() { if (!have) block(); return out[16 - have--]; }
    uint64_t next_u64() { uint64_t lo = next_u32(), hi = next_u32(); return lo | hi << 32; }
};

typedef PallasFr PF;
inline fr_t h_one() { return fr_one<PF>(); }
inline fr_t h_zero() { return fr_zero<PF>(); }
inline fr_t h_mul(const fr_t& a, const fr_t& b) { return fr_mul<PF>(a, b); }
inline fr_t h_add(const fr_t& a, const fr_t& b) { return fr_add<PF>(a, b); }
inline fr_t h_sub(const fr_t& a, const fr_t& b) { return fr_sub<PF>(a, b); }
inline fr_t h_u64(uint64_t x) { return fr_from_u64<PF>(x); }
inline fr_t h_from_le_bytes_mod_order(const uint8_t* b, size_t n) {
    fr_t acc = h_zero(); const fr_t two32 = h_u64(1ull << 32);
    size_t nw = (n + 3) / 4;
    for (size_t k = nw; k-- > 0;) {
        uint32_t w = 0; for (size_t j = 0; j < 4; ++j) if (4 * k + j < n) w |= (uint32_t)b[4 * k + j] << (8 * j);
        acc = h_add(h_mul(acc, two32), h_u64(w));
    }
    return acc;
}
inline void h_to_bytes_le(const fr_t& a, uint8_t out[32]) {
    fr_t c = fr_to_canonical<PF>(a);
    for (int i = 0; i < 8; ++i) for (int j = 0; j < 4; ++j) out[4 * i + j] = (uint8_t)(c.v[i] >> (8 * j));
}
inline fr_t h_fr_from_hash(const char* tag, const std::vector<uint8_t>& data) {
    std::vector<uint8_t> buf(tag, tag + strlen(tag)); buf.insert(buf.end(), data.begin(), data.end());
    uint8_t d[32]; Blake3::hash(buf.data(), buf.size(), d);
    uint8_t wide[64]; memset(wide, 0, 64); memcpy(wide, d, 32);
    return h_from_le_bytes_mod_order(wide, 64);
}
inline fr_t h_tag(const char* s) {
    size_t n = strlen(s);
    if (n <= 32) { uint8_t le[32] = {0}; memcpy(le, s, n); return h_from_le_bytes_mod_order(le, 32); }
    fr_t acc = h_zero();
    for (size_t off = 0; off < n; off += 32) { uint8_t le[32] = {0}; size_t c = n - off < 32 ? n - off : 32; memcpy(le, s + off, c); acc = h_add(acc, h_from_le_bytes_mod_order(le, 32)); }
    return acc;
}
inline std::vector<fr_t> h_words(const char* s) {
    std::vector<fr_t> out; size_t n = strlen(s);
    for (size_t off = 0; off < n; off += 31) { uint8_t le[32] = {0}; size_t c = n - off < 31 ? n - off : 31; memcpy(le, s + off, c); out.push_back(h_from_le_bytes_mod_order(le, 32)); }
    return out;
}
inline int tr_hash_frame(const char* tag, std::vector<fr_t>& frame) {
    const fr_t AB = h_tag("FSv1-ABSORB-BYTES"), CH = h_tag("FSv1-CHALLENGE");
    frame.clear();
    frame.push_back(AB); for (auto& w : h_words("FRI/FS")) frame.push_back(w);
    frame.push_back(AB); for (auto& w : h_words(tag)) frame.push_back(w);
    const int np = (int)frame.size();
    frame.push_back(CH); frame.push_back(AB); for (auto& w : h_words("out")) frame.push_back(w);
    return np;
}

struct PoseidonConsts {
    int t = 0, rf = 0, rp = 0;
    std::vector<fr_t> mds;
    std::vector<fr_t> rc_full;
    std::vector<fr_t> rc_partial;
};
inline void put64(std::vector<uint8_t>& v, uint64_t x) { for (int j = 0; j < 8; ++j) v.push_back((uint8_t)(x >> (8 * j))); }
inline PoseidonConsts derive_consts(const std::string& seed, int t, int rf, int rp) {
    PoseidonConsts c; c.t = t; c.rf = rf; c.rp = rp;
    c.mds.resize((size_t)t * t); c.rc_full.resize((size_t)rf * t); c.rc_partial.resize(rp);
    for (int i = 0; i < t; ++i) for (int j = 0; j < t; ++j) { std::vector<uint8_t> d; put64(d, i); put64(d, j); d.insert(d.end(), seed.begin(), seed.end()); c.mds[(size_t)i * t + j] = h_fr_from_hash("POSEIDON-MDS", d); }
    for (int r = 0; r < rf; ++r) for (int i = 0; i < t; ++i) { std::vector<uint8_t> d; put64(d, r); put64(d, i); d.insert(d.end(), seed.begin(), seed.end()); c.rc_full[(size_t)r * t + i] = h_fr_from_hash("POSEIDON-RC-FULL", d); }
    for (int r = 0; r < rp; ++r) { std::vector<uint8_t> d; put64(d, r); d.insert(d.end(), seed.begin(), seed.end()); c.rc_partial[r] = h_fr_from_hash("POSEIDON-RC-PART", d); }
    return c;
}
inline int width_for_arity(size_t arity) { return arity <= 8 ? 9 : arity <= 16 ? 17 : arity <= 32 ? 33 : arity <= 64 ? 65 : arity <= 128 ? 129 : -1; }
inline int rp_for_width(int t) { switch (t) { case 9: return 60; case 17: return 64; case 33: return 68; case 65: return 76; case 129: return 84; default: return -1; } }
inline PoseidonConsts consts_for_width(int t) {
    std::string seed = "POSEIDON-PALLAS-T"; for (int j = 0; j < 8; ++j) seed.push_back((char)(((uint64_t)t >> (8 * j)) & 0xff));
    return derive_consts(seed, t, 8, rp_for_width(t));
}
inline PoseidonConsts consts_transcript() { return derive_consts("POSEIDON-T17-X5-TRANSCRIPT", 17, 8, 64); }

struct KernelConsts {
    int t = 0, rf = 0, rp = 0;
    std::vector<fr_t> rc_full, rc_partial;
    std::vector<fr_t> lu, lu_pre;
    std::vector<fr_t> row0;
    std::vector<fr_t> sparse;
    std::vector<fr_t> mds;
    std::vector<fr_t> mds_pre;
    std::vector<fr_t> gamma;
    std::vector<uint32_t> lu29, lu_pre29, row0_29, sparse29, gamma29;
    std::vector<uint32_t> mds29, mds_pre29;
    std::vector<uint32_t> rc_full29;
    std::vector<int8_t> mds_frag, mds_pre_frag;
    std::vector<uint32_t> chain_a, chain_g, chain_w;
    std::vector<int8_t> blk8_efrag, blk8_lfrag, blk8_gfrag;
    std::vector<uint32_t> gamma8_29;
    std::vector<fr_t> blk8_lambda, rc_partial_scaled;
    std::vector<int8_t> blk8s_efrag, blk8s_lfrag, blk8s_gfrag;
    std::vector<uint32_t> blk8_unscale29;
    bool ok = false;
};
template <class Pred> inline std::vector<uint32_t> to_radix29(const std::vector<fr_t>& v, Pred scaled) {
    const fr_t k = fr_from_u64<PF>(1ull << FR29_SBOX_SHIFT);
    std::vector<uint32_t> o(v.size() * 9);
    for (size_t i = 0; i < v.size(); ++i) fr29_const_from<PF>(scaled(i) ? fr_mul<PF>(v[i], k) : v[i], &o[9 * i]);
    return o;
}
inline void mfma_frag_of(fr_t g, int8_t* out) {
    const fr_t k256 = fr_from_u64<PF>(256);
    int8_t d[32][32];
    for (int b = 0; b < 32; ++b, g = h_mul(g, k256)) {
        const fr_t c = fr_to_canonical<PF>(g); int cy = 0;
        for (int k = 0; k < 32; ++k) { const int v = (int)((c.v[k >> 2] >> (8 * (k & 3))) & 0xff) + 0x80 + cy; cy = v >> 8; d[b][k] = (int8_t)((v & 0xff) - 0x80); }
    }
    for (int l = 0; l < 64; ++l) for (int j = 0; j < 16; ++j) out[(size_t)l * 16 + j] = d[16 * (l >> 5) + j][l & 31];
}
inline std::vector<int8_t> mfma_frags(const fr_t* mat, int rows, int cols, const fr_t& scale) {
    std::vector<int8_t> out((size_t)rows * cols * 64 * 16, 0);
    for (int i = 0; i < rows; ++i) for (int e = 0; e < cols; ++e) mfma_frag_of(h_mul(mat[(size_t)i * cols + e], scale), &out[((size_t)i * cols + e) * 64 * 16]);
    return out;
}
inline std::vector<int8_t> mfma_frags(const std::vector<fr_t>& mat, int t) { return mfma_frags(mat.data(), t, t, fr_from_u64<PF>(1ull << FR29_SBOX_SHIFT)); }
inline bool mat_inverse(std::vector<fr_t> a, int n, std::vector<fr_t>& inv) {
    inv.assign((size_t)n * n, h_zero()); for (int i = 0; i < n; ++i) inv[(size_t)i * n + i] = h_one();
    for (int c = 0; c < n; ++c) {
        int p = -1; for (int r = c; r < n; ++r) if (!fr_is_zero(a[(size_t)r * n + c])) { p = r; break; }
        if (p < 0) return false;
        if (p != c) for (int k = 0; k < n; ++k) { std::swap(a[(size_t)p * n + k], a[(size_t)c * n + k]); std::swap(inv[(size_t)p * n + k], inv[(size_t)c * n + k]); }
        fr_t pi = fr_inv<PF>(a[(size_t)c * n + c]);
        for (int k = 0; k < n; ++k) { a[(size_t)c * n + k] = h_mul(a[(size_t)c * n + k], pi); inv[(size_t)c * n + k] = h_mul(inv[(size_t)c * n + k], pi); }
        for (int r = 0; r < n; ++r) if (r != c) {
            fr_t f = a[(size_t)r * n + c]; if (fr_is_zero(f)) continue;
            for (int k = 0; k < n; ++k) { a[(size_t)r * n + k] = h_sub(a[(size_t)r * n + k], h_mul(f, a[(size_t)c * n + k])); inv[(size_t)r * n + k] = h_sub(inv[(size_t)r * n + k], h_mul(f, inv[(size_t)c * n + k])); }
        }
    }
    return true;
}
inline bool lu_pack(const std::vector<fr_t>& m, int n, std::vector<fr_t>& lu) {
    lu = m;
    for (int k = 0; k < n; ++k) {
        if (fr_is_zero(lu[(size_t)k * n + k])) return false;
        fr_t pi = fr_inv<PF>(lu[(size_t)k * n + k]);
        for (int i = k + 1; i < n; ++i) {
            fr_t f = h_mul(lu[(size_t)i * n + k], pi); lu[(size_t)i * n + k] = f;
            for (int j = k + 1; j < n; ++j) lu[(size_t)i * n + j] = h_sub(lu[(size_t)i * n + j], h_mul(f, lu[(size_t)k * n + j]));
        }
    }
    return true;
}
inline KernelConsts make_kernel_consts(const PoseidonConsts& c) {
    KernelConsts k; k.t = c.t; k.rf = c.rf; k.rp = c.rp; k.rc_full = c.rc_full; k.rc_partial = c.rc_partial; k.mds = c.mds;
    const int t = c.t, n = t - 1;
    k.row0.assign(c.mds.begin(), c.mds.begin() + t);
    std::vector<fr_t> cur = c.mds;
    k.sparse.assign((size_t)c.rp * (2 * t - 1), h_zero());
    for (int r = c.rp - 1; r >= 0; --r) {
        std::vector<fr_t> hat((size_t)n * n), hinv;
        for (int i = 0; i < n; ++i) for (int j = 0; j < n; ++j) hat[(size_t)i * n + j] = cur[(size_t)(i + 1) * t + (j + 1)];
        if (!mat_inverse(hat, n, hinv)) return k;
        fr_t* sp = &k.sparse[(size_t)r * (2 * t - 1)];
        sp[0] = cur[0];
        for (int j = 0; j < n; ++j) { fr_t acc = h_zero(); for (int q = 0; q < n; ++q) acc = h_add(acc, h_mul(cur[(size_t)0 * t + (q + 1)], hinv[(size_t)q * n + j])); sp[1 + j] = acc; }
        for (int i = 0; i < n; ++i) sp[t + i] = cur[(size_t)(i + 1) * t + 0];
        std::vector<fr_t> nxt((size_t)t * t);
        for (int j = 0; j < t; ++j) nxt[j] = c.mds[j];
        for (int i = 0; i < n; ++i) for (int j = 0; j < t; ++j) { fr_t acc = h_zero(); for (int q = 0; q < n; ++q) acc = h_add(acc, h_mul(hat[(size_t)i * n + q], c.mds[(size_t)(q + 1) * t + j])); nxt[(size_t)(i + 1) * t + j] = acc; }
        cur.swap(nxt);
    }
    if (c.rp % 4) return k;
    k.gamma.assign((size_t)(c.rp / 4) * 6, h_zero());
    for (int b = 0; b < c.rp / 4; ++b)
        for (int q = 1; q < 4; ++q)
            for (int p2 = 0; p2 < q; ++p2) {
                const fr_t* uq = &k.sparse[(size_t)(4 * b + q) * (2 * t - 1)];
                const fr_t* wp = &k.sparse[(size_t)(4 * b + p2) * (2 * t - 1)];
                fr_t acc = h_zero();
                for (int j = 1; j < t; ++j) acc = h_add(acc, h_mul(uq[j], wp[t - 1 + j]));
                k.gamma[(size_t)b * 6 + q * (q - 1) / 2 + p2] = acc;
            }
    if (!lu_pack(c.mds, t, k.lu)) return k;
    if (!lu_pack(cur, t, k.lu_pre)) return k;
    k.mds_pre = cur;
    const auto upper = [t](size_t i) { return (int)(i % t) >= (int)(i / t); };
    const auto all = [](size_t) { return true; };
    const auto a_and_w = [t](size_t i) { const int c = (int)(i % (2 * t - 1)); return c == 0 || c >= t; };
    k.lu29 = to_radix29(k.lu, upper); k.lu_pre29 = to_radix29(k.lu_pre, upper); k.row0_29 = to_radix29(k.row0, all);
    k.sparse29 = to_radix29(k.sparse, a_and_w); k.gamma29 = to_radix29(k.gamma, all);
    k.mds29 = to_radix29(k.mds, all); k.mds_pre29 = to_radix29(k.mds_pre, all);
    k.rc_full29.resize(k.rc_full.size() * 9);
    for (size_t i = 0; i < k.rc_full.size(); ++i) { const fr29_t u = fr29_unpack(k.rc_full[i]); for (int j = 0; j < 9; ++j) k.rc_full29[9 * i + j] = u.l[j]; }
    if (t == 17) { k.mds_frag = mfma_frags(k.mds, t); k.mds_pre_frag = mfma_frags(k.mds_pre, t); }
    if (t == 17 && c.rp % 8 == 0) {
        const int nb = c.rp / 8, w = 2 * t - 1;
        const fr_t s20 = fr_from_u64<PF>(1ull << FR29_SBOX_SHIFT);
        std::vector<fr_t> g8((size_t)nb * 28, h_zero()), um((size_t)8 * n), wm((size_t)n * 8);
        const fr_t kappa = fr_inv<PF>(s20), a_inv = fr_inv<PF>(c.mds[0]);
        std::vector<fr_t> yinv(c.rp), ums((size_t)8 * n), wms((size_t)n * 8);
        k.blk8_lambda.assign((size_t)c.rp + 1, h_one()); k.rc_partial_scaled.resize(c.rp);
        for (int q = 0; q < c.rp; ++q) {
            const fr_t l5k = h_mul(fr_pow5<PF>(k.blk8_lambda[q]), kappa);
            k.blk8_lambda[q + 1] = h_mul(l5k, a_inv); yinv[q] = fr_inv<PF>(l5k);
            k.rc_partial_scaled[q] = h_mul(k.blk8_lambda[q], c.rc_partial[q]);
        }
        k.blk8_unscale29.resize(9); fr29_const_from<PF>(fr_inv<PF>(k.blk8_lambda[c.rp]), k.blk8_unscale29.data());
        for (int b = 0; b < nb; ++b) {
            for (int q = 0; q < 8; ++q) for (int j = 1; j < t; ++j) {
                um[(size_t)q * n + (j - 1)] = k.sparse[(size_t)(8 * b + q) * w + j];
                wm[(size_t)(j - 1) * 8 + q] = k.sparse[(size_t)(8 * b + q) * w + t - 1 + j];
            }
            const std::vector<int8_t> ef = mfma_frags(um.data(), 8, n, h_one()), lf = mfma_frags(wm.data(), n, 8, s20);
            k.blk8_efrag.insert(k.blk8_efrag.end(), ef.begin(), ef.end()); k.blk8_lfrag.insert(k.blk8_lfrag.end(), lf.begin(), lf.end());
            for (int q = 1; q < 8; ++q) for (int p2 = 0; p2 < q; ++p2) {
                fr_t acc = h_zero();
                for (int j = 0; j < n; ++j) acc = h_add(acc, h_mul(um[(size_t)q * n + j], wm[(size_t)j * 8 + p2]));
                g8[(size_t)b * 28 + q * (q - 1) / 2 + p2] = acc;
                k.blk8_gfrag.resize(k.blk8_gfrag.size() + 1024); mfma_frag_of(h_mul(acc, s20), &k.blk8_gfrag[k.blk8_gfrag.size() - 1024]);
                k.blk8s_gfrag.resize(k.blk8s_gfrag.size() + 1024); mfma_frag_of(h_mul(h_mul(acc, k.blk8_lambda[8 * b + q + 1]), yinv[8 * b + p2]), &k.blk8s_gfrag[k.blk8s_gfrag.size() - 1024]);
            }
            for (int q = 0; q < 8; ++q) for (int j = 0; j < n; ++j) {
                ums[(size_t)q * n + j] = h_mul(um[(size_t)q * n + j], k.blk8_lambda[8 * b + q + 1]);
                wms[(size_t)j * 8 + q] = h_mul(wm[(size_t)j * 8 + q], yinv[8 * b + q]);
            }
            const std::vector<int8_t> efs = mfma_frags(ums.data(), 8, n, h_one()), lfs = mfma_frags(wms.data(), n, 8, h_one());
            k.blk8s_efrag.insert(k.blk8s_efrag.end(), efs.begin(), efs.end()); k.blk8s_lfrag.insert(k.blk8s_lfrag.end(), lfs.begin(), lfs.end());
        }
        k.blk8_lfrag.resize(k.blk8_lfrag.size() + 1024); mfma_frag_of(h_one(), &k.blk8_lfrag[k.blk8_lfrag.size() - 1024]);
        k.gamma8_29 = to_radix29(g8, all);
    }
    if (t == 17 && c.rp == 64) {
        const int rp = c.rp, w = 2 * t - 1;
        const fr_t scale = fr_from_u64<PF>(1ull << 25);
        auto limbs = [&](const fr_t& v, uint32_t* out) { const fr29_t u = fr29_unpack(h_mul(v, scale)); for (int i = 0; i < 9; ++i) out[i] = u.l[i]; };
        k.chain_a.assign((size_t)rp * 64, 0u); k.chain_g.assign((size_t)rp * 9 * 64, 0u); k.chain_w.assign((size_t)rp * (t - 1) * 9, 0u);
        for (int q = 0; q < rp; ++q) {
            uint32_t l[9]; limbs(k.sparse[(size_t)q * w], l);
            for (int i = 0; i < 9; ++i) k.chain_a[(size_t)q * 64 + 16 + i] = l[i];
            for (int j = 1; j < t; ++j) limbs(k.sparse[(size_t)q * w + t - 1 + j], &k.chain_w[((size_t)q * (t - 1) + (j - 1)) * 9]);
        }
        for (int q = 1; q < rp; ++q)
            for (int p2 = 0; p2 < q; ++p2) {
                const fr_t* uq = &k.sparse[(size_t)q * w]; const fr_t* wp = &k.sparse[(size_t)p2 * w];
                fr_t acc = h_zero();
                for (int j = 1; j < t; ++j) acc = h_add(acc, h_mul(uq[j], wp[t - 1 + j]));
                uint32_t l[9]; limbs(acc, l);
                if (q == p2 + 1) { for (int i = 0; i < 9; ++i) k.chain_a[(size_t)p2 * 64 + 32 + i] = l[i]; }
                else for (int i = 0; i < 9; ++i) k.chain_g[((size_t)p2 * 9 + i) * 64 + q] = l[i];
            }
    }
    k.ok = true;
    return k;
}

inline void permute_dense(fr_t* s, const PoseidonConsts& c) {
    const int t = c.t, half = c.rf / 2; std::vector<fr_t> o(t);
    auto mds = [&]() { for (int i = 0; i < t; ++i) { fr_t acc = h_zero(); for (int j = 0; j < t; ++j) acc = h_add(acc, h_mul(c.mds[(size_t)i * t + j], s[j])); o[i] = acc; } for (int i = 0; i < t; ++i) s[i] = o[i]; };
    for (int r = 0; r < half; ++r) { for (int i = 0; i < t; ++i) s[i] = fr_pow5<PF>(h_add(s[i], c.rc_full[(size_t)r * t + i])); mds(); }
    for (int r = 0; r < c.rp; ++r) { s[0] = fr_pow5<PF>(h_add(s[0], c.rc_partial[r])); mds(); }
    for (int r = half; r < c.rf; ++r) { for (int i = 0; i < t; ++i) s[i] = fr_pow5<PF>(h_add(s[i], c.rc_full[(size_t)r * t + i])); mds(); }
}

}
}
```

stark_mlwe_amd/csrc/hostcheck.cpp:

```cpp
#include <algorithm>
#include <atomic>
#include <cstring>
#include <vector>
#include "fr.hpp"
#include "host_util.hpp"
#include "poseidon_dev.hpp"
#include "fri_plan.hpp"
#include "fri_verify.hpp"
#include "fri_verify_batch.hpp"
#include "mfma_digits.hpp"
#include "poseidon_chain.hpp"
#include "fri_batch.hpp"
#include "ntt_batch_plan.hpp"
#include "sumcheck_impl.hpp"
#include "mle_dev.hpp"
#include "merkle_batch.hpp"
#include "lagrange_dev.hpp"

using namespace stark;

static fr_t ld4(const uint64_t* p) { fr_t x; for (int i = 0; i < 4; ++i) { x.v[2 * i] = (uint32_t)p[i]; x.v[2 * i + 1] = (uint32_t)(p[i] >> 32); } return x; }
static void st4(uint64_t* p, const fr_t& x) { for (int i = 0; i < 4; ++i) p[i] = (uint64_t)x.v[2 * i] | ((uint64_t)x.v[2 * i + 1] << 32); }

static int g_alloc_fill = 0;
static std::vector<uint64_t> hc_block(size_t bytes) { std::vector<uint64_t> v((bytes + 7) / 8 + 1); memset(v.data(), g_alloc_fill, v.size() * sizeof(uint64_t)); return v; }
static std::vector<fr_t> hc_fr_block(size_t n) { std::vector<fr_t> v(n); if (n) memset((void*)v.data(), g_alloc_fill, n * sizeof(fr_t)); return v; }
struct HostArena {
    std::vector<std::vector<uint64_t>> mem;
    int32_t alloc(size_t bytes, void** out) { mem.push_back(hc_block(bytes)); *out = mem.back().data(); return 0; }
    int32_t upload(void* dst, const void* src, size_t bytes) { memcpy(dst, src, bytes); return 0; }
    template <class T> int32_t put(const std::vector<T>& h, T** out) {
        void* p = nullptr; alloc(std::max<size_t>(h.size(), 1) * sizeof(T), &p);
        if (!h.empty()) upload(p, h.data(), h.size() * sizeof(T));
        *out = (T*)p; return 0;
    }
    int32_t download(void* dst, const void* src, size_t bytes) { memcpy(dst, src, bytes); return 0; }
};

struct HcParams { host::PoseidonConsts ref; host::KernelConsts kc; PoseidonDev dev; };
static void bind(HcParams* P) {
    P->kc = host::make_kernel_consts(P->ref);
    P->dev.t = P->kc.t; P->dev.rf = P->kc.rf; P->dev.rp = P->kc.rp; P->dev.rc_full = P->kc.rc_full.data(); P->dev.rc_partial = P->kc.rc_partial.data();
    P->dev.lu = P->kc.lu.data(); P->dev.lu_pre = P->kc.lu_pre.data(); P->dev.row0 = P->kc.row0.data(); P->dev.sparse = P->kc.sparse.data(); P->dev.mds = P->kc.mds.data(); P->dev.mds_pre = P->kc.mds_pre.data(); P->dev.gamma = P->kc.gamma.data();
    P->dev.lu29 = P->kc.lu29.data(); P->dev.lu_pre29 = P->kc.lu_pre29.data(); P->dev.row0_29 = P->kc.row0_29.data(); P->dev.sparse29 = P->kc.sparse29.data(); P->dev.gamma29 = P->kc.gamma29.data(); P->dev.mds29 = P->kc.mds29.data(); P->dev.mds_pre29 = P->kc.mds_pre29.data(); P->dev.rc_full29 = P->kc.rc_full29.data();
    P->dev.mds_frag = nullptr; P->dev.mds_pre_frag = nullptr; P->dev.blk8_efrag = nullptr; P->dev.blk8_lfrag = nullptr; P->dev.blk8_unit_frag = nullptr; P->dev.blk8_gfrag = nullptr; P->dev.rc_partial_scaled = nullptr;
    P->dev.chain_a = P->kc.chain_a.empty() ? nullptr : P->kc.chain_a.data(); P->dev.chain_g = P->kc.chain_g.empty() ? nullptr : P->kc.chain_g.data(); P->dev.chain_w = P->kc.chain_w.empty() ? nullptr : P->kc.chain_w.data();
}

extern "C" {

int hc_set_alloc_fill(int byte) { if (byte < 0 || byte > 255) return -1; const int old = g_alloc_fill; g_alloc_fill = byte; return old; }
int hc_alloc_probe(size_t bytes, uint8_t* out) { const std::vector<uint64_t> v = hc_block(bytes); memcpy(out, v.data(), bytes); return 0; }

int hc_fr_op(int field, int op, const uint64_t* a, const uint64_t* b, uint64_t* out) {
    fr_t x = ld4(a), y = b ? ld4(b) : x, z;
    if (field == 0) {
        switch (op) { case 0: z = fr_add<PallasFr>(x, y); break; case 1: z = fr_sub<PallasFr>(x, y); break; case 2: z = fr_mul<PallasFr>(x, y); break; case 3: z = fr_inv<PallasFr>(x); break;
            case 4: z = fr_from_u64<PallasFr>(a[0]); break; case 5: z = fr_to_canonical<PallasFr>(x); break; case 6: z = fr_root_of_unity<PallasFr>((unsigned)a[0]); break;
            case 7: z = fr_pow_u64<PallasFr>(x, b[0]); break; case 8: z = fr_pow5_r29<PallasFr>(x); break; default: return -1; }
    } else {
        switch (op) { case 0: z = fr_add<Bls12381Fr>(x, y); break; case 1: z = fr_sub<Bls12381Fr>(x, y); break; case 2: z = fr_mul<Bls12381Fr>(x, y); break; case 3: z = fr_inv<Bls12381Fr>(x); break;
            case 4: z = fr_from_u64<Bls12381Fr>(a[0]); break; case 5: z = fr_to_canonical<Bls12381Fr>(x); break; case 6: z = fr_root_of_unity<Bls12381Fr>((unsigned)a[0]); break;
            case 7: z = fr_pow_u64<Bls12381Fr>(x, b[0]); break; case 8: z = fr_pow5_r29<Bls12381Fr>(x); break; default: return -1; }
    }
    st4(out, z); return 0;
}
int hc_wide_dot(const uint64_t* a, const uint64_t* b, size_t n, uint64_t* out) {
    DotAcc d; d.init();
    for (size_t i = 0; i < n; ++i) { uint32_t c[9]; fr29_const_from<PF>(ld4(a + 4 * i), c); d.mac(c, ld4(b + 4 * i)); }
    st4(out, d.finish()); return 0;
}
int hc_wide_dot32(const uint64_t* a, const uint64_t* b, size_t n, uint64_t* out) {
    if (n > 24) return -1;
    fr_wide w; fr_wide_zero(w);
    for (size_t i = 0; i < n; ++i) fr_wide_mac_f<PF>(w, ld4(a + 4 * i), ld4(b + 4 * i));
    st4(out, fr_wide_reduce<PF>(w)); return 0;
}
}
template <class F> static int hc_ntt29_impl(uint64_t* data, int log_b, int inverse, uint64_t* max_limb, uint64_t* max_top) {
    if (log_b < 1 || log_b > 16) return -1;
    const size_t B = (size_t)1 << log_b;
    fr_t w = fr_root_of_unity<F>((unsigned)log_b); if (inverse) w = fr_inv<F>(w);
    const fr_t k32 = fr_from_u64<F>(32);
    std::vector<fr29_t> tw(B / 2), x(B);
    { fr_t acc = k32; for (size_t i = 0; i < B / 2; ++i) { tw[i] = fr29_unpack(acc); acc = fr_mul<F>(acc, w); } }
    uint32_t D[9]; ntt29_offset<F>(D);
    auto brev = [&](size_t v) { size_t r = 0; for (int i = 0; i < log_b; ++i) r |= ((v >> i) & 1) << (log_b - 1 - i); return r; };
    for (size_t p = 0; p < B; ++p) x[brev(p)] = fr29_unpack(ld4(data + 4 * p));
    uint64_t ml = 0, mt = 0;
    const int head = log_b >= 3 ? 3 : log_b;
    {
        const fr29_t w1 = tw[log_b >= 3 ? B >> 3 : 0], w2 = tw[log_b >= 2 ? B >> 2 : 0], w3 = tw[log_b >= 3 ? 3 * (B >> 3) : 0];
        for (size_t g = 0; g < (B >> head); ++g) {
            fr29_t* xs = &x[g << head];
            if (head == 3) ntt29_head<F, 3>(*reinterpret_cast<fr29_t (*)[8]>(xs), w1, w2, w3, D);
            else if (head == 2) ntt29_head<F, 2>(*reinterpret_cast<fr29_t (*)[4]>(xs), w1, w2, w3, D);
            else ntt29_head<F, 1>(*reinterpret_cast<fr29_t (*)[2]>(xs), w1, w2, w3, D);
        }
    }
    for (int s = head + 1; s <= log_b; ++s) {
        const size_t half = (size_t)1 << (s - 1); const bool nrm = ntt29_norm_before(s);
        for (size_t bq = 0; bq < B / 2; ++bq) {
            const size_t j = bq & (half - 1), grp = bq >> (s - 1), i0 = (grp << s) + j, i1 = i0 + half;
            fr29_t a = x[i0], b = x[i1];
            { fr29_t bb = b, aa = a; if (nrm) { fr29_norm(bb); fr29_norm(aa); } for (int k = 0; k < 8; ++k) { ml = std::max<uint64_t>(ml, bb.l[k]); ml = std::max<uint64_t>(ml, aa.l[k]); } mt = std::max<uint64_t>(mt, std::max(bb.l[8], aa.l[8])); }
            ntt29_butterfly<F>(a, b, tw[j << (log_b - s)], D, nrm);
            x[i0] = a; x[i1] = b;
        }
    }
    const bool nrm_out = ntt29_norm_after(log_b);
    fr_t mult = k32; if (inverse) mult = fr_mul<F>(k32, fr_inv<F>(fr_from_u64<F>((uint64_t)B)));
    for (size_t k = 0; k < B; ++k) {
        fr29_t y = x[k];
        for (int i = 0; i < 8; ++i) ml = std::max<uint64_t>(ml, nrm_out ? 0 : y.l[i]);
        if (inverse) {
            if (nrm_out) fr29_norm(y);
            mt = std::max<uint64_t>(mt, y.l[8]);
            const fr29_t r = fr29_mul_mont<F>(fr29_unpack(mult), y);
            st4(data + 4 * k, fr29_pack_reduce<F>(r.l));
        } else {
            fr29_partial_reduce<F>(y);
            st4(data + 4 * k, fr29_pack_reduce<F>(y.l));
        }
    }
    if (max_limb) *max_limb = ml; if (max_top) *max_top = mt;
    return 0;
}
extern "C" {
int hc_partial_reduce(int field, uint32_t* limbs, size_t n) {
    for (size_t i = 0; i < n; ++i) {
        fr29_t x; for (int k = 0; k < 9; ++k) x.l[k] = limbs[9 * i + k];
        if (field == 0) fr29_partial_reduce<PallasFr>(x); else fr29_partial_reduce<Bls12381Fr>(x);
        for (int k = 0; k < 9; ++k) limbs[9 * i + k] = x.l[k];
    }
    return 0;
}
int hc_ntt29(int field, uint64_t* data, int log_b, int inverse, uint64_t* max_limb, uint64_t* max_top) {
    return field == 0 ? hc_ntt29_impl<PallasFr>(data, log_b, inverse, max_limb, max_top) : hc_ntt29_impl<Bls12381Fr>(data, log_b, inverse, max_limb, max_top);
}
int hc_blake3(const uint8_t* p, size_t n, uint8_t* out32) { host::Blake3::hash(p, n, out32); return 0; }
int hc_chacha12_u64s(const uint8_t* seed32, size_t n, uint64_t* out) { host::ChaCha12Rng r(seed32); for (size_t i = 0; i < n; ++i) out[i] = r.next_u64(); return 0; }
int hc_from_le_bytes_mod_order(const uint8_t* b, size_t n, uint64_t* out) { st4(out, host::h_from_le_bytes_mod_order(b, n)); return 0; }
int hc_to_bytes_le(const uint64_t* a, uint8_t* out32) { host::h_to_bytes_le(ld4(a), out32); return 0; }

void* hc_params_new(int kind, int t, const char* seed) {
    HcParams* P = new HcParams();
    P->ref = kind == 0 ? host::consts_for_width(t) : kind == 1 ? host::consts_transcript() : host::derive_consts(seed, 17, 8, 64);
    bind(P); return P;
}
void* hc_params_upload(int t, int rf, int rp, const uint64_t* mds, const uint64_t* rc_full, const uint64_t* rc_partial) {
    if (!mds || !rc_full || !rc_partial || t < 2 || rf <= 0 || (rf & 1) || rp <= 0) return nullptr;
    HcParams* P = new HcParams();
    P->ref.t = t; P->ref.rf = rf; P->ref.rp = rp;
    P->ref.mds.resize((size_t)t * t); P->ref.rc_full.resize((size_t)rf * t); P->ref.rc_partial.resize(rp);
    for (size_t i = 0; i < P->ref.mds.size(); ++i) P->ref.mds[i] = ld4(mds + 4 * i);
    for (size_t i = 0; i < P->ref.rc_full.size(); ++i) P->ref.rc_full[i] = ld4(rc_full + 4 * i);
    for (size_t i = 0; i < P->ref.rc_partial.size(); ++i) P->ref.rc_partial[i] = ld4(rc_partial + 4 * i);
    bind(P); return P;
}
int hc_params_ok(void* h) { return ((HcParams*)h)->kc.ok ? 1 : 0; }
void hc_params_free(void* h) { delete (HcParams*)h; }
int hc_params_export(void* h, uint64_t* mds, uint64_t* rc_full, uint64_t* rc_partial) {
    HcParams* P = (HcParams*)h;
    for (size_t i = 0; i < P->ref.mds.size(); ++i) st4(mds + 4 * i, P->ref.mds[i]);
    for (size_t i = 0; i < P->ref.rc_full.size(); ++i) st4(rc_full + 4 * i, P->ref.rc_full[i]);
    for (size_t i = 0; i < P->ref.rc_partial.size(); ++i) st4(rc_partial + 4 * i, P->ref.rc_partial[i]);
    return 0;
}
int hc_full_round_linear(void* h, int which, int pre, uint64_t* states, size_t n) {
    HcParams* P = (HcParams*)h; const int t = P->dev.t;
    if (t != 17 || P->kc.mds_frag.empty()) return -1;
    std::vector<fr_t> st(t), out(t);
    const std::vector<int8_t>& F = pre ? P->kc.mds_pre_frag : P->kc.mds_frag;
    for (size_t s = 0; s < n; ++s) {
        for (int j = 0; j < t; ++j) st[j] = ld4(states + 4 * (s * t + j));
        if (which == 0) { ArrayState a{st.data()}; apply_lu(a, pre ? P->dev.lu_pre29 : P->dev.lu29, t); out = st; }
        else {
            std::vector<fr_t> xd(t); for (int e = 0; e < t; ++e) xd[e] = recode_signed(st[e]);
            for (int i = 0; i < t; ++i) {
                int32_t S[32];
                for (int r = 0; r < 32; ++r) { int64_t acc = 0;
                    for (int e = 0; e < t; ++e) for (int kh = 0; kh < 2; ++kh) { const int8_t* a = &F[((((size_t)i * t + e) * 64) + (r + 32 * kh)) * 16];
                        const int8_t* b = reinterpret_cast<const int8_t*>(xd[e].v) + 16 * kh; for (int j = 0; j < 16; ++j) acc += (int64_t)a[j] * b[j]; }
                    if (acc > 0x7fffffffll || acc < -0x80000000ll) return -2; S[r] = (int32_t)acc; }
                int64_t col[9]; mfma_cols_of_sums(S, col);
                out[i] = mfma_finish_cols(col);
            }
        }
        for (int j = 0; j < t; ++j) st4(states + 4 * (s * t + j), out[j]);
    }
    return 0;
}
size_t hc_mfma_frag_table(void* h, int pre, int8_t* out, size_t cap) {
    HcParams* P = (HcParams*)h; const std::vector<int8_t>& F = pre ? P->kc.mds_pre_frag : P->kc.mds_frag;
    if (out) memcpy(out, F.data(), std::min(cap, F.size()));
    return F.size();
}
int hc_mfma_finish(const int32_t* sums, size_t n, uint64_t* out) {
    for (size_t s = 0; s < n; ++s) {
        const int32_t* S = sums + 32 * s;
        for (int c = 0; c < 32; ++c) if (S[c] >= (1 << 24) || S[c] <= -(1 << 24)) return -1;
        int64_t col[9]; mfma_cols_of_sums(S, col);
        st4(out + 4 * s, mfma_finish_cols(col));
    }
    return 0;
}
int hc_mfma_finish_limbs(const int32_t* sums, size_t n, uint32_t* out) {
    for (size_t s = 0; s < n; ++s) {
        const int32_t* S = sums + 32 * s;
        for (int c = 0; c < 32; ++c) if (S[c] >= (1 << 24) || S[c] <= -(1 << 24)) return -1;
        int64_t col[9]; mfma_cols_of_sums(S, col);
        mfma_finish_limbs(col, out + 9 * s);
    }
    return 0;
}
int hc_sbox_lazy29(const uint32_t* l, const uint32_t* c, size_t n, uint64_t* out, uint64_t* colmax) {
    for (size_t s = 0; s < n; ++s) {
        const uint32_t* ls = l + 9 * s; const uint32_t* cs = c + 9 * s;
        for (int i = 0; i < 9; ++i) if (ls[i] >= (i < 8 ? 1u << 29 : 1u << 24) || cs[i] >= (i < 8 ? 1u << 29 : 1u << 23)) return -1;
        const fr_t z = sbox_lazy29(ls, cs);
        Lazy29Wide wide; const fr29_t x5 = wide.pow5(ls, cs);
        const fr_t zw = fr29_pack_reduce<PF>(x5.l);
        if (colmax) { colmax[2 * s] = (uint64_t)wide.max_col; colmax[2 * s + 1] = (uint64_t)(wide.max_col >> 64); }
        if ((wide.max_col >> 64) == 0 && memcmp(&z, &zw, sizeof(fr_t)) != 0) return -2;
        st4(out + 4 * s, z);
    }
    return 0;
}
static int blk8_tile_sums(const int8_t* const* frag, const fr_t* xd, int K, int32_t* S) {
    for (int r = 0; r < 32; ++r) { int64_t acc = 0;
        for (int k = 0; k < K; ++k) for (int kh = 0; kh < 2; ++kh) { const int8_t* a = frag[k] + (size_t)(r + 32 * kh) * 16;
            const int8_t* b = reinterpret_cast<const int8_t*>(xd[k].v) + 16 * kh; for (int j = 0; j < 16; ++j) acc += (int64_t)a[j] * b[j]; }
        if (acc >= (1 << 24) || acc <= -(1 << 24)) return -2; S[r] = (int32_t)acc; }
    return 0;
}
static fr_t blk8_finish_sums(const int32_t* S) { int64_t col[9]; mfma_cols_of_sums(S, col); return mfma_finish_cols(col); }
static void blk8_finish_sums_limbs(const int32_t* S, uint32_t* l) { int64_t col[9]; mfma_cols_of_sums(S, col); mfma_finish_limbs(col, l); }
static int blk8_tile(const int8_t* const* frag, const fr_t* xd, int K, fr_t& out) { int32_t S[32]; const int rc = blk8_tile_sums(frag, xd, K, S); if (rc) return rc; out = blk8_finish_sums(S); return 0; }
static std::atomic<int32_t> g_blk8_row23_max{0};
int32_t hc_blk8_row23_max(int reset) { return reset ? g_blk8_row23_max.exchange(0) : g_blk8_row23_max.load(); }
int hc_permute_block8(void* h, uint64_t* states, size_t n) {
    HcParams* P = (HcParams*)h; const host::KernelConsts& k = P->kc; const int t = k.t, half = k.rf / 2;
    if (t != 17 || k.blk8s_efrag.empty() || k.blk8s_gfrag.empty() || k.blk8_unscale29.empty() || k.mds_frag.empty()) return -1;
    const int8_t* unit = k.blk8_lfrag.data() + k.blk8_lfrag.size() - 1024;
    std::vector<fr_t> st(t), xd(t), o(t);
    auto sbox = [&](int r) { for (int j = 0; j < t; ++j) xd[j] = recode_signed(fr_pow5_r29<PF>(fr_add<PF>(st[j], k.rc_full[(size_t)r * t + j]))); };
    auto product = [&](const std::vector<int8_t>& F, int next) -> int {
        for (int i = 0; i < t; ++i) {
            const int8_t* fr[17]; for (int e = 0; e < t; ++e) fr[e] = &F[((size_t)i * t + e) * 1024];
            int32_t S[32]; const int rc = blk8_tile_sums(fr, xd.data(), t, S); if (rc) return rc;
            if (next < 0) o[i] = blk8_finish_sums(S);
            else { uint32_t l[9]; blk8_finish_sums_limbs(S, l); o[i] = recode_signed(sbox_lazy29(l, &k.rc_full29[((size_t)next * t + i) * 9])); }
        }
        if (next < 0) st = o; else xd = o;
        return 0; };
    for (size_t s = 0; s < n; ++s) {
        for (int j = 0; j < t; ++j) st[j] = ld4(states + 4 * (s * t + j));
        sbox(0);
        for (int r = 0; r < half; ++r) { const int rc = product(r == half - 1 ? k.mds_pre_frag : k.mds_frag, r == half - 1 ? -1 : r + 1); if (rc) return rc; }
        fr_t s0 = st[0], rec[17], y[8], yd[9], kx[23];
        for (int j = 1; j < t; ++j) rec[j] = recode_signed(st[j]);
        const int nb = k.rp / 8;
        for (int b = 0; b < nb; ++b) {
            const int8_t* ef = k.blk8s_efrag.data() + (size_t)b * 8 * 16 * 1024; const int8_t* lf = k.blk8s_lfrag.data() + (size_t)b * 16 * 8 * 1024;
            const int8_t* gf = k.blk8s_gfrag.data() + (size_t)b * 28 * 1024;
            for (int j = 0; j < 16; ++j) kx[j] = rec[1 + j];
            for (int q = 0; q < 8; ++q) {
                const int8_t* fr[23]; for (int j = 0; j < 16; ++j) fr[j] = ef + ((size_t)q * 16 + j) * 1024;
                for (int p2 = 0; p2 < q; ++p2) { fr[16 + p2] = gf + ((size_t)q * (q - 1) / 2 + p2) * 1024; kx[16 + p2] = yd[p2]; }
                int32_t S[32]; { const int rc = blk8_tile_sums(fr, kx, 16 + q, S); if (rc) return rc; }
                if (q == 7) { int32_t m = 0; for (int c = 0; c < 32; ++c) m = std::max(m, S[c] < 0 ? -S[c] : S[c]);
                              int32_t seen = g_blk8_row23_max.load(); while (m > seen && !g_blk8_row23_max.compare_exchange_weak(seen, m)) {} }
                const fr_t H = blk8_finish_sums(S);
                y[q] = fr_pow5_r29<PF>(fr_add<PF>(s0, k.rc_partial_scaled[8 * b + q]));
                yd[q] = recode_signed(y[q]);
                s0 = fr_add<PF>(y[q], H);
            }
            for (int j = 1; j < t; ++j) {
                const int8_t* fr[9]; for (int p2 = 0; p2 < 8; ++p2) fr[p2] = lf + ((size_t)(j - 1) * 8 + p2) * 1024; fr[8] = unit;
                yd[8] = rec[j];
                if (b == nb - 1) {
                    int32_t S[32]; { const int rc = blk8_tile_sums(fr, yd, 9, S); if (rc) return rc; }
                    uint32_t l[9]; blk8_finish_sums_limbs(S, l); xd[j] = recode_signed(sbox_lazy29(l, &k.rc_full29[((size_t)half * t + j) * 9]));
                } else { fr_t z; { const int rc = blk8_tile(fr, yd, 9, z); if (rc) return rc; } rec[j] = recode_signed(z); }
            }
        }
        s0 = fr_mul_c29(k.blk8_unscale29.data(), s0);
        xd[0] = recode_signed(fr_pow5_r29<PF>(fr_add<PF>(s0, k.rc_full[(size_t)half * t])));
        for (int r = half; r < k.rf; ++r) { const int rc = product(k.mds_frag, r == k.rf - 1 ? -1 : r + 1); if (rc) return rc; }
        for (int j = 0; j < t; ++j) st4(states + 4 * (s * t + j), st[j]);
    }
    return 0;
}
size_t hc_blk8_table(void* h, int which, void* out, size_t cap) {
    HcParams* P = (HcParams*)h; const host::KernelConsts& k = P->kc;
    if (which >= 4) {
        std::vector<uint8_t> lam;
        if (which == 8 && !k.blk8_lambda.empty()) { lam.resize(k.blk8_lambda.size() * sizeof(fr_t) + k.blk8_unscale29.size() * 4);
            memcpy(lam.data(), k.blk8_lambda.data(), k.blk8_lambda.size() * sizeof(fr_t)); memcpy(lam.data() + k.blk8_lambda.size() * sizeof(fr_t), k.blk8_unscale29.data(), k.blk8_unscale29.size() * 4); }
        const void* src = which == 4 ? (const void*)k.blk8s_efrag.data() : which == 5 ? (const void*)k.blk8s_lfrag.data() : which == 6 ? (const void*)k.blk8s_gfrag.data() : which == 7 ? (const void*)k.rc_partial_scaled.data() : (const void*)lam.data();
        const size_t len = which == 4 ? k.blk8s_efrag.size() : which == 5 ? k.blk8s_lfrag.size() : which == 6 ? k.blk8s_gfrag.size() : which == 7 ? k.rc_partial_scaled.size() * sizeof(fr_t) : which == 8 ? lam.size() : 0;
        if (out && len) memcpy(out, src, std::min(cap, len));
        return len;
    }
    const void* src = which == 0 ? (const void*)k.blk8_efrag.data() : which == 1 ? (const void*)k.blk8_lfrag.data() : which == 3 ? (const void*)k.blk8_gfrag.data() : (const void*)k.gamma8_29.data();
    const size_t len = which == 0 ? k.blk8_efrag.size() : which == 1 ? k.blk8_lfrag.size() : which == 3 ? k.blk8_gfrag.size() : k.gamma8_29.size() * 4;
    if (out && len) memcpy(out, src, std::min(cap, len));
    return len;
}
size_t hc_rc_full29_table(void* h, uint32_t* out, size_t cap) {
    const std::vector<uint32_t>& v = ((HcParams*)h)->kc.rc_full29;
    if (out && !v.empty()) memcpy(out, v.data(), std::min(cap, v.size()) * 4);
    return v.size();
}
int hc_blk8_finish_with_base(void* h, const int32_t* sums, const uint64_t* bases, size_t n, uint64_t* out) {
    HcParams* P = (HcParams*)h; if (P->kc.blk8_lfrag.empty()) return -3;
    const int8_t* unit = P->kc.blk8_lfrag.data() + P->kc.blk8_lfrag.size() - 1024;
    for (size_t s = 0; s < n; ++s) {
        const fr_t bd = recode_signed(ld4(bases + 4 * s)); int32_t U[32], S[32];
        if (blk8_tile_sums(&unit, &bd, 1, U)) return -1;
        for (int c = 0; c < 32; ++c) { const int64_t v = (int64_t)sums[32 * s + c] + U[c]; if (v >= (1 << 24) || v <= -(1 << 24)) return -1; S[c] = (int32_t)v; }
        st4(out + 4 * s, blk8_finish_sums(S));
    }
    return 0;
}
int hc_permute_kernel_form(void* h, uint64_t* states, size_t n) {
    HcParams* P = (HcParams*)h; int t = P->dev.t; std::vector<fr_t> st(t);
    for (size_t i = 0; i < n; ++i) { for (int j = 0; j < t; ++j) st[j] = ld4(states + 4 * (i * t + j)); ArrayState s{st.data()}; permute_core(s, P->dev, false); for (int j = 0; j < t; ++j) st4(states + 4 * (i * t + j), st[j]); }
    return 0;
}
int hc_permute_chain_model(void* h, uint64_t* states, size_t n) {
    HcParams* P = (HcParams*)h; const int t = P->ref.t, half = P->ref.rf / 2; if (!P->dev.chain_a) return -1;
    std::vector<fr_t> st(t), o(t);
    auto dense = [&](const std::vector<fr_t>& M) { for (int i = 0; i < t; ++i) { fr_t acc = host::h_zero(); for (int j = 0; j < t; ++j) acc = host::h_add(acc, host::h_mul(M[(size_t)i * t + j], st[j])); o[i] = acc; } st = o; };
    for (size_t i = 0; i < n; ++i) {
        for (int j = 0; j < t; ++j) st[j] = ld4(states + 4 * (i * t + j));
        for (int r = 0; r < half; ++r) { for (int j = 0; j < t; ++j) st[j] = fr_pow5<PallasFr>(host::h_add(st[j], P->ref.rc_full[(size_t)r * t + j])); dense(r == half - 1 ? P->kc.mds_pre : P->kc.mds); }
        chain_partial_model(st.data(), P->dev);
        for (int r = half; r < P->ref.rf; ++r) { for (int j = 0; j < t; ++j) st[j] = fr_pow5<PallasFr>(host::h_add(st[j], P->ref.rc_full[(size_t)r * t + j])); dense(P->kc.mds); }
        for (int j = 0; j < t; ++j) st4(states + 4 * (i * t + j), st[j]);
    }
    return 0;
}
int hc_row_consts(uint32_t* out14) { const RowConstsHost K = row_consts_host(); for (int i = 0; i < 9; ++i) out14[i] = K.ni[i]; for (int i = 0; i < 5; ++i) out14[9 + i] = K.t[i]; return 0; }
size_t hc_chain_table(void* h, int which, uint32_t* out, size_t cap) {
    HcParams* P = (HcParams*)h; const std::vector<uint32_t>& v = which == 0 ? P->kc.chain_a : which == 1 ? P->kc.chain_g : P->kc.chain_w;
    if (out) for (size_t i = 0; i < v.size() && i < cap; ++i) out[i] = v[i];
    return v.size();
}
int hc_permute_dense(void* h, uint64_t* states, size_t n) {
    HcParams* P = (HcParams*)h; int t = P->ref.t; std::vector<fr_t> st(t);
    for (size_t i = 0; i < n; ++i) { for (int j = 0; j < t; ++j) st[j] = ld4(states + 4 * (i * t + j)); host::permute_dense(st.data(), P->ref); for (int j = 0; j < t; ++j) st4(states + 4 * (i * t + j), st[j]); }
    return 0;
}
}
static void leaf_init(fr_t init[17]) {
    const fr_t AB = host::h_tag("FSv1-ABSORB-BYTES"), CH = host::h_tag("FSv1-CHALLENGE");
    for (int j = 0; j < 17; ++j) init[j] = host::h_zero();
    init[0] = AB; init[1] = host::h_words("FRI/leaf/poseidon")[0]; init[2] = AB; init[3] = host::h_words("FRI/leaf")[0];
    init[6] = CH; init[7] = AB; init[8] = host::h_words("leaf")[0]; init[16] = host::h_tag("FSv1-TRANSCRIPT-INIT");
}
extern "C" {
int hc_leaf_pair(void* tparams, const uint64_t* f, const uint64_t* f_next, size_t n, size_t m, uint64_t* hout) {
    HcParams* P = (HcParams*)tparams;
    fr_t init[17]; leaf_init(init);
    std::vector<fr_t> fv(n), nv(f_next ? (n + m - 1) / m : 0);
    for (size_t i = 0; i < fv.size(); ++i) fv[i] = ld4(f + 4 * i);
    for (size_t i = 0; i < nv.size(); ++i) nv[i] = ld4(f_next + 4 * i);
    const LeafStream L{init, fv.data(), f_next ? nv.data() : nullptr, m, n};
    fr_t st[17];
    for (size_t i = 0; i < n; ++i) { ArrayState s{st}; st4(hout + 4 * i, leaf_pair_body(s, P->dev, L, i)); }
    return 0;
}
int hc_hash_ds_level(void* params, int mode, size_t arity, uint32_t level, uint64_t pos0, uint64_t label, const uint64_t* in0, const uint64_t* in1, size_t n_in, uint64_t* out) {
    HcParams* P = (HcParams*)params;
    std::vector<fr_t> a(n_in), b(in1 ? n_in : 0), st(P->dev.t);
    for (size_t i = 0; i < n_in; ++i) { a[i] = ld4(in0 + 4 * i); if (in1) b[i] = ld4(in1 + 4 * i); }
    const DsStream D = DsStream::make(mode, arity, level, pos0, label, a.data(), in1 ? b.data() : nullptr, n_in);
    for (size_t k = 0; k < D.n_out; ++k) { ArrayState s{st.data()}; st4(out + 4 * k, hash_ds_body(s, P->dev, D, k)); }
    return 0;
}
int hc_tr_hash(void* tparams, const char* tag, const uint64_t* fields, size_t k, size_t n, uint64_t* out) {
    HcParams* P = (HcParams*)tparams;
    std::vector<fr_t> fr; const int np = host::tr_hash_frame(tag, fr);
    std::vector<fr_t> fl(n * k); for (size_t i = 0; i < n * k; ++i) fl[i] = ld4(fields + 4 * i);
    const TrStream T = TrStream::equal(fr.data(), np, (int)fr.size() - np, fl.data(), k, n, host::h_tag("FSv1-TRANSCRIPT-INIT"));
    fr_t st[17];
    for (size_t i = 0; i < n; ++i) { ArrayState s{st}; st4(out + 4 * i, tr_hash_body(s, P->dev, T, i)); }
    return 0;
}
int hc_tr_frame_dims(const char* tag, int* np, int* ns) { std::vector<fr_t> fr; *np = host::tr_hash_frame(tag, fr); *ns = (int)fr.size() - *np; return 0; }
int hc_tr_hash_many(void* tparams, size_t n, const char* const* tags, const uint64_t* const* fields, const size_t* k, uint64_t* out, size_t* launch_order) {
    HcParams* P = (HcParams*)tparams;
    std::vector<std::vector<fr_t>> frames(n), fl(n); std::vector<TrFrameRef> fr(n); std::vector<const fr_t*> fp(n, nullptr);
    for (size_t i = 0; i < n; ++i) {
        const int np = host::tr_hash_frame(tags[i], frames[i]); fr[i] = TrFrameRef{frames[i].data(), np, (int)frames[i].size() - np};
        if (!k[i]) continue;
        if (!fields || !fields[i]) return -1;
        fl[i].resize(k[i]); for (size_t q = 0; q < k[i]; ++q) fl[i][q] = ld4(fields[i] + 4 * q);
        fp[i] = fl[i].data();
    }
    const std::vector<TrStream::Item> items = tr_ragged_items(fr.data(), fp.data(), k, n);
    const TrStream T = tr_ragged_stream(items.data(), n, host::h_tag("FSv1-TRANSCRIPT-INIT"));
    fr_t st[17];
    for (size_t j = 0; j < n; ++j) {
        ArrayState s{st}; size_t slot = n; const fr_t d = tr_hash_body<true>(s, P->dev, T, j, &slot);
        if (slot >= n) return -2;
        st4(out + 4 * slot, d); if (launch_order) launch_order[j] = slot;
    }
    return 0;
}
size_t hc_mixed_prove_groups(size_t B, const size_t* n0, const size_t* schedule, const size_t* sched_off, const size_t* r, size_t* group_of, size_t* order) {
    const std::vector<std::vector<size_t>> G = mixed_prove_groups(B, n0, schedule, sched_off, r);
    size_t pos = 0;
    for (size_t g = 0; g < G.size(); ++g) for (size_t i : G[g]) { group_of[i] = g; order[pos++] = i; }
    return G.size();
}
int hc_hash_stream(void* params, int mode, const uint64_t* a, size_t na, const uint64_t* b, size_t nb, const uint64_t* tag, size_t n, uint64_t* out) {
    HcParams* P = (HcParams*)params;
    std::vector<fr_t> av(n * na), bv(n * nb), st(P->dev.t);
    for (size_t i = 0; i < n * na; ++i) av[i] = ld4(a + 4 * i); for (size_t i = 0; i < n * nb; ++i) bv[i] = ld4(b + 4 * i);
    for (size_t k = 0; k < n; ++k) { ArrayState s{st.data()}; st4(out + 4 * k, hash_stream_body(s, P->dev, mode, av.data(), na, bv.data(), nb, tag ? ld4(tag) : host::h_zero(), k)); }
    return 0;
}

struct HcHasher : TrHasher {
    void* tp; explicit HcHasher(void* p) : tp(p) {}
    int32_t hash(const char* tag, const fr_t* fields, size_t k, size_t n, fr_t* out) override {
        std::vector<uint64_t> in(4 * k * n), o(4 * n);
        for (size_t i = 0; i < k * n; ++i) st4(in.data() + 4 * i, fields[i]);
        int rc = hc_tr_hash(tp, tag, in.data(), k, n, o.data()); if (rc) return rc;
        for (size_t i = 0; i < n; ++i) out[i] = ld4(o.data() + 4 * i);
        return 0;
    }
};
struct HcPlan { FriPlan plan; void* tp; };
void* hc_fri_plan_create(void* tparams, const uint64_t* roots, size_t n0, const size_t* schedule, size_t L, size_t r) {
    std::vector<fr_t> rt(L + 1); for (size_t l = 0; l <= L; ++l) rt[l] = ld4(roots + 4 * l);
    HcPlan* P = new HcPlan(); P->tp = tparams; P->plan.r = r; std::string err;
    if (!P->plan.shape.make(n0, schedule, L, rt.data(), err)) { delete P; return nullptr; }
    HcHasher H(tparams); if (fri_plan_make(P->plan, H)) { delete P; return nullptr; }
    return P;
}
size_t hc_fri_plan_num_requests(void* p) { return ((HcPlan*)p)->plan.req.size(); }
int hc_fri_plan_requests(void* p, uint32_t* kind, uint32_t* which, uint32_t* level, uint64_t* index) {
// ... 496 lines not shown
```

stark_mlwe_amd/csrc/mfma_digits.hpp:

```cpp
#pragma once
#include "fr.hpp"
#include "fr29.hpp"

namespace stark {

typedef PallasFr PF;
static_assert(fr_p29<PF>(4) < (1u << 10) && fr_p29<PF>(5) == 0 && fr_p29<PF>(6) == 0 && fr_p29<PF>(7) == 0 && fr_p29<PF>(8) == (1u << 22), "r = 2^254 + t with t below 2^126");

FR_HD fr_t recode_signed(const fr_t& x) {
    fr_t y; uint64_t c = 0;
#pragma unroll
    for (int i = 0; i < 8; ++i) { const uint64_t t = (uint64_t)x.v[i] + 0x80808080u + c; y.v[i] = (uint32_t)t ^ 0x80808080u; c = t >> 32; }
    return y;
}
template <class V> FR_HD void mfma_fold_rows(int64_t* col, const V& lo, const V& hi) {
#pragma unroll
    for (int q = 0; q < 4; ++q)
#pragma unroll
        for (int hh = 0; hh < 2; ++hh)
#pragma unroll
            for (int p = 0; p < 2; ++p) {
                const V& a = hh ? hi : lo;
                const int64_t pair = (int64_t)a[4 * q + 2 * p] + (int64_t)a[4 * q + 2 * p + 1] * 256;
                const int c = 8 * q + 4 * hh + 2 * p, k = (8 * c) / 29, sh = 8 * c - 29 * k;
                col[k] += pair * ((int64_t)1 << sh);
            }
}
FR_HD void mfma_finish_limbs(int64_t* col, uint32_t* l) {
#pragma unroll
    for (int k = 0; k < 8; ++k) { col[k + 1] += col[k] >> 29; l[k] = (uint32_t)col[k] & FR_M29; }
    const int64_t top = col[8];
    const int32_t q1 = (int32_t)(top >> 22) - 1;
    l[8] = ((uint32_t)top & ((1u << 22) - 1)) + (1u << 22);
    int64_t carry = 0;
#pragma unroll
    for (int i = 0; i < 5; ++i) { const int64_t d = (int64_t)l[i] - (int64_t)q1 * (int64_t)fr_p29<PF>(i) + carry; l[i] = (uint32_t)d & FR_M29; carry = d >> 29; }
    int32_t c32 = (int32_t)carry;
#pragma unroll
    for (int i = 5; i < 9; ++i) { const int32_t d = (int32_t)l[i] + c32; if (i < 8) { l[i] = (uint32_t)d & FR_M29; c32 = d >> 29; } else l[8] = (uint32_t)d; }
}
FR_HD fr_t mfma_finish_cols(int64_t* col) {
    uint32_t l[9];
    mfma_finish_limbs(col, l);
    fr_t z = fr29_pack_reduce<PF>(l);
    fr_cond_sub<PF>(z.v, 0u);
    return z;
}
FR_HD fr_t sbox_lazy29(const uint32_t* l, const uint32_t* __restrict__ c_) {
#if defined(__HIP_DEVICE_COMPILE__)
    typedef const __attribute__((address_space(4))) uint32_t* cptr_t;
    cptr_t c = (cptr_t)c_;
#else
    const uint32_t* c = c_;
#endif
    fr29_t u;
#pragma unroll
    for (int i = 0; i < 9; ++i) u.l[i] = l[i] + c[i];
    const fr29_t x2 = fr29_sqr_mont<PF>(u), x4 = fr29_sqr_mont<PF>(x2), x5 = fr29_mul_mont<PF>(u, x4);
    return fr29_pack_reduce<PF>(x5.l);
}
#if !defined(__HIP_DEVICE_COMPILE__)
inline void mfma_cols_of_sums(const int32_t* S, int64_t* col) {
    int32_t lo[16], hi[16];
    for (int reg = 0; reg < 16; ++reg) { const int row = (reg & 3) + 8 * (reg >> 2); lo[reg] = S[row]; hi[reg] = S[row + 4]; }
    for (int k = 0; k < 9; ++k) col[k] = 0;
    mfma_fold_rows(col, lo, hi);
}
struct Lazy29Wide {
    typedef unsigned __int128 u128;
    u128 max_col = 0;
    void mont(u128* w, uint32_t* l) {
        for (int k = 0; k < 9; ++k) {
            const u128 t = w[k]; if (t > max_col) max_col = t;
            const uint32_t m = (0u - (uint32_t)t) & FR_M29;
            w[k + 1] += (t + FR_M29) >> 29;
            for (int j = 1; j < 9; ++j) if (fr_p29<PF>(j) != 0) w[k + j] += (u128)m * fr_p29<PF>(j);
        }
        u128 carry = 0;
        for (int i = 0; i < 9; ++i) { const u128 v = w[9 + i] + carry; if (w[9 + i] > max_col) max_col = w[9 + i]; l[i] = i < 8 ? ((uint32_t)v & FR_M29) : (uint32_t)v; carry = v >> 29; }
    }
    fr29_t sqr(const fr29_t& a) {
        u128 w[18]; for (int k = 0; k < 18; ++k) w[k] = 0;
        for (int i = 0; i < 9; ++i) { w[2 * i] += (u128)a.l[i] * a.l[i]; for (int j = i + 1; j < 9; ++j) w[i + j] += (u128)a.l[i] * ((uint64_t)a.l[j] << 1); }
        fr29_t r; mont(w, r.l); return r;
    }
    fr29_t mul(const fr29_t& a, const fr29_t& b) {
        u128 w[18]; for (int k = 0; k < 18; ++k) w[k] = 0;
        for (int i = 0; i < 9; ++i) for (int j = 0; j < 9; ++j) w[i + j] += (u128)a.l[i] * b.l[j];
        fr29_t r; mont(w, r.l); return r;
    }
    fr29_t pow5(const uint32_t* l, const uint32_t* c) {
        fr29_t u; for (int i = 0; i < 9; ++i) u.l[i] = l[i] + c[i];
        const fr29_t x2 = sqr(u), x4 = sqr(x2); return mul(u, x4);
    }
};
#endif

}
```

stark_mlwe_amd/csrc/poseidon_pair.hpp:

```cpp
#pragma once
#include "fr.hpp"
#include "dev_common.hpp"
#include "poseidon_params.hpp"
#include "poseidon_dev.hpp"
#include "poseidon_streams.hpp"
#include "mfma_digits.hpp"

#if defined(__HIPCC__)
namespace stark {

template <int T> struct PairCfg {
#ifndef STARK_NXD17
#define STARK_NXD17 5
#endif
    static constexpr int NXD = T == 17 ? STARK_NXD17 : 2;
#ifndef STARK_NXU17
#define STARK_NXU17 8
#endif
    static constexpr int NXU = T == 17 ? STARK_NXU17 : (T - 1) / 2;
    static constexpr int NX = (T - 1) / 2;
    static constexpr int EXTRA = 3;
    __host__ __device__ static constexpr int xslot(int p) { return p == 0 ? 0 : T + (p - 1); }
    __host__ __device__ static constexpr int dslot(int q) { return 1 + (q % NXD); }
    __host__ __device__ static constexpr size_t lds_bytes() { return (size_t)(T + EXTRA) * 2 * 64 * 16; }
};
static inline size_t pair_lds_bytes(int t) { return t == 17 ? PairCfg<17>::lds_bytes() : PairCfg<9>::lds_bytes(); }

struct PairState {
    uint4* st;
    int lane; bool isY;
    __device__ __forceinline__ fr_t ld(int j) const {
        uint4 lo = st[(2 * j) * 64 + lane], hi = st[(2 * j + 1) * 64 + lane];
        fr_t x; x.v[0] = lo.x; x.v[1] = lo.y; x.v[2] = lo.z; x.v[3] = lo.w; x.v[4] = hi.x; x.v[5] = hi.y; x.v[6] = hi.z; x.v[7] = hi.w; return x;
    }
    __device__ __forceinline__ void sto(int j, const fr_t& x) const {
        st[(2 * j) * 64 + lane] = make_uint4(x.v[0], x.v[1], x.v[2], x.v[3]);
        st[(2 * j + 1) * 64 + lane] = make_uint4(x.v[4], x.v[5], x.v[6], x.v[7]);
    }
};

template <int T>
__device__ __forceinline__ void pair_apply_lu(const PairState& s, const uint32_t* lu) {
    const int yo = s.isY ? 1 : 0;
#pragma unroll 1
    for (int k = 0; 2 * k < T; ++k) {
        const int i = 2 * k + yo; const bool have = i < T;
        fr_t res;
        if (have) { DotAcc w; w.init(); _Pragma("unroll 1") for (int j = i; j < T; ++j) w.mac(c29(lu, i * T + j), s.ld(j)); res = w.finish(); }
        __syncthreads();
        if (have) s.sto(i, res);
    }
    __syncthreads();
#pragma unroll 1
    for (int k = 0; T - 1 - 2 * k >= 1; ++k) {
        const int i = T - 1 - 2 * k - yo; const bool have = i >= 1;
        fr_t res;
        if (have) { DotAcc w; w.init(); _Pragma("unroll 1") for (int j = 0; j < i; ++j) w.mac(c29(lu, i * T + j), s.ld(j)); res = fr_add<PF>(s.ld(i), w.finish()); }
        __syncthreads();
        if (have) s.sto(i, res);
    }
    __syncthreads();
}
template <int T, bool RECODE = false>
__device__ __forceinline__ void pair_sbox_full(const PairState& s, const fr_t* rc) {
    const int j0 = s.isY ? PairCfg<T>::NX : 0, j1 = s.isY ? T : PairCfg<T>::NX;
    for (int j = j0; j < j1; ++j) { const fr_t x = fr_pow5_r29<PF>(fr_add<PF>(s.ld(j), rc[j])); s.sto(j, RECODE ? recode_signed(x) : x); }
    __syncthreads();
}

typedef int mfma_v4i __attribute__((ext_vector_type(4)));
typedef int mfma_v16i __attribute__((ext_vector_type(16)));
__device__ __forceinline__ void mfma_zero_tile(mfma_v16i (&acc)[2]) {
#pragma unroll
    for (int ct = 0; ct < 2; ++ct)
#pragma unroll
        for (int r = 0; r < 16; ++r) acc[ct][r] = 0;
}
__device__ __forceinline__ void mfma_post_cols(const mfma_v16i (&acc)[2], int64_t* col) {
    mfma_v16i lo, hi;
#pragma unroll
    for (int r = 0; r < 16; ++r) {
        const auto sw = __builtin_amdgcn_permlane32_swap((unsigned)acc[0][r], (unsigned)acc[1][r], false, false);
        lo[r] = (int)sw[0]; hi[r] = (int)sw[1];
    }
#pragma unroll
    for (int k = 0; k < 9; ++k) col[k] = 0;
    mfma_fold_rows(col, lo, hi);
}
__device__ __forceinline__ fr_t mfma_post(const mfma_v16i (&acc)[2]) {
    int64_t col[9];
    mfma_post_cols(acc, col);
    return mfma_finish_cols(col);
}
__device__ __forceinline__ void pair_sto_sbox29(const PairState& s, int j, const uint32_t* l, const uint32_t* rc29, bool recode) {
    const fr_t y = sbox_lazy29(l, rc29);
    s.sto(j, recode ? recode_signed(y) : y);
}
__device__ __forceinline__ void pair_mds_sbox_mfma(const PairState& s, const void* frag, const uint32_t* rc29, bool recode) {
    constexpr int T = 17;
    const int lane = s.lane, h = lane >> 5;
    mfma_v4i b[T][2];
#pragma unroll
    for (int e = 0; e < T; ++e)
#pragma unroll
        for (int ct = 0; ct < 2; ++ct) { const uint4 u = s.st[(2 * e + h) * 64 + 32 * ct + (lane & 31)]; b[e][ct] = mfma_v4i{(int)u.x, (int)u.y, (int)u.z, (int)u.w}; }
    __syncthreads();
    const mfma_v4i* A = reinterpret_cast<const mfma_v4i*>(frag) + lane;
#pragma unroll 1
    for (int i = s.isY ? 1 : 0; i < T; i += 2) {
        mfma_v16i acc[2];
        mfma_zero_tile(acc);
        const mfma_v4i* Ai = A + (size_t)i * T * 64;
#pragma unroll
        for (int e = 0; e < T; ++e) {
            const mfma_v4i a = Ai[(size_t)e * 64];
#pragma unroll
            for (int ct = 0; ct < 2; ++ct) acc[ct] = __builtin_amdgcn_mfma_i32_32x32x32_i8(a, b[e][ct], acc[ct], 0, 0, 0);
        }
        int64_t col[9];
        mfma_post_cols(acc, col);
        if (rc29) { uint32_t l[9]; mfma_finish_limbs(col, l); pair_sto_sbox29(s, i, l, c29(rc29, i), recode); }
        else s.sto(i, mfma_finish_cols(col));
    }
    __syncthreads();
}

struct Blk8Tabs {
    const mfma_v4i* efrag;
    const mfma_v4i* lfrag;
    const mfma_v4i* unit;
    const mfma_v4i* gfrag;
    const fr_t* rc;
};
struct Blk8Cfg {
    static constexpr int NLX = 8;
    __host__ __device__ static constexpr int ymail(int q) { return 17 + (q & 1); }
    __host__ __device__ static constexpr int hmail(int q) { return (q & 1) ? 19 : 0; }
};
__device__ __forceinline__ void blk8_load_frags16(mfma_v4i (&a)[16], const mfma_v4i* A, int lane) {
#pragma unroll
    for (int e = 0; e < 16; ++e) a[e] = (A + (size_t)e * 64)[lane];
}
__device__ __forceinline__ mfma_v4i blk8_b_of_slot(const PairState& s, int j, int ct) {
    const uint4 u = s.st[(2 * j + (s.lane >> 5)) * 64 + 32 * ct + (s.lane & 31)];
    return mfma_v4i{(int)u.x, (int)u.y, (int)u.z, (int)u.w};
}
template <int Q>
__device__ __forceinline__ void blk8_round_x(const PairState& s, const Blk8Tabs& Tb, fr_t& s0, mfma_v4i (&b)[8][2]) {
    __builtin_amdgcn_sched_barrier(0);
    const fr_t y = fr_pow5_r29<PF>(fr_add<PF>(s0, Tb.rc[Q]));
    s.sto(Blk8Cfg::ymail(Q), recode_signed(y));
    __syncthreads();
    s0 = fr_add<PF>(y, s.ld(Blk8Cfg::hmail(Q)));
    b[Q][0] = blk8_b_of_slot(s, Blk8Cfg::ymail(Q), 0); b[Q][1] = blk8_b_of_slot(s, Blk8Cfg::ymail(Q), 1);
}
template <int Q>
__device__ __forceinline__ void blk8_round_y(const PairState& s, const Blk8Tabs& Tb, mfma_v4i (&b)[8][2], mfma_v4i (&a)[16], mfma_v4i (&g)[7]) {
    __builtin_amdgcn_sched_barrier(0);
    const int lane = s.lane;
    mfma_v16i acc[2];
    mfma_zero_tile(acc);
#pragma unroll
    for (int e = 0; e < 16; ++e)
#pragma unroll
        for (int ct = 0; ct < 2; ++ct) acc[ct] = __builtin_amdgcn_mfma_i32_32x32x32_i8(a[e], blk8_b_of_slot(s, e + 1, ct), acc[ct], 0, 0, 0);
    if constexpr (Q > 0) {
#pragma unroll
        for (int p = 0; p < Q; ++p)
#pragma unroll
            for (int ct = 0; ct < 2; ++ct) acc[ct] = __builtin_amdgcn_mfma_i32_32x32x32_i8(g[p], b[p][ct], acc[ct], 0, 0, 0);
    }
    if constexpr (Q < 7) {
        blk8_load_frags16(a, Tb.efrag + (size_t)(Q + 1) * 16 * 64, lane);
#pragma unroll
        for (int p = 0; p <= Q; ++p) g[p] = (Tb.gfrag + (size_t)((Q + 1) * Q / 2 + p) * 64)[lane];
    }
    s.sto(Blk8Cfg::hmail(Q), mfma_post(acc));
    __syncthreads();
    b[Q][0] = blk8_b_of_slot(s, Blk8Cfg::ymail(Q), 0); b[Q][1] = blk8_b_of_slot(s, Blk8Cfg::ymail(Q), 1);
}
template <int NLX>
__device__ __forceinline__ void blk8_lane_rows(const PairState& s, const Blk8Tabs& Tb, const mfma_v4i (&b)[8][2], bool last, const uint32_t* rc29_next = nullptr, bool recode_next = true) {
    static_assert(NLX >= 1 && NLX <= 15, "shares");
    const int lane = s.lane;
    const int j0 = s.isY ? NLX + 1 : 1, j1 = s.isY ? 16 : NLX;
    const mfma_v4i aunit = Tb.unit[lane];
    mfma_v4i a[8];
#pragma unroll
    for (int p = 0; p < 8; ++p) a[p] = (Tb.lfrag + ((size_t)(j0 - 1) * 8 + p) * 64)[lane];
#pragma unroll 1
    for (int j = j0; j <= j1; ++j) {
        mfma_v16i acc[2];
        mfma_zero_tile(acc);
#pragma unroll
        for (int p = 0; p < 8; ++p)
#pragma unroll
            for (int ct = 0; ct < 2; ++ct) acc[ct] = __builtin_amdgcn_mfma_i32_32x32x32_i8(a[p], b[p][ct], acc[ct], 0, 0, 0);
#pragma unroll
        for (int ct = 0; ct < 2; ++ct) acc[ct] = __builtin_amdgcn_mfma_i32_32x32x32_i8(aunit, blk8_b_of_slot(s, j, ct), acc[ct], 0, 0, 0);
        const int jn = j < j1 ? j + 1 : j1;
#pragma unroll
        for (int p = 0; p < 8; ++p) a[p] = (Tb.lfrag + ((size_t)(jn - 1) * 8 + p) * 64)[lane];
        if (rc29_next) { int64_t col[9]; uint32_t l[9]; mfma_post_cols(acc, col); mfma_finish_limbs(col, l); pair_sto_sbox29(s, j, l, c29(rc29_next, j), recode_next); }
        else { const fr_t z = mfma_post(acc); s.sto(j, last ? z : recode_signed(z)); }
    }
    __syncthreads();
}
template <int NLX>
__device__ __forceinline__ void pair_block8(const PairState& s, const Blk8Tabs& Tb, fr_t& s0, bool last, const uint32_t* rc29_next = nullptr, const fr_t* rc_next = nullptr, bool recode_next = true,
                                            const uint32_t* unscale29 = nullptr) {
    mfma_v4i b[8][2];
    if (!s.isY) {
        blk8_round_x<0>(s, Tb, s0, b); blk8_round_x<1>(s, Tb, s0, b); blk8_round_x<2>(s, Tb, s0, b); blk8_round_x<3>(s, Tb, s0, b);
        blk8_round_x<4>(s, Tb, s0, b); blk8_round_x<5>(s, Tb, s0, b); blk8_round_x<6>(s, Tb, s0, b); blk8_round_x<7>(s, Tb, s0, b);
    } else {
        mfma_v4i a[16], g[7];
        blk8_load_frags16(a, Tb.efrag, s.lane);
        blk8_round_y<0>(s, Tb, b, a, g); blk8_round_y<1>(s, Tb, b, a, g); blk8_round_y<2>(s, Tb, b, a, g); blk8_round_y<3>(s, Tb, b, a, g);
        blk8_round_y<4>(s, Tb, b, a, g); blk8_round_y<5>(s, Tb, b, a, g); blk8_round_y<6>(s, Tb, b, a, g); blk8_round_y<7>(s, Tb, b, a, g);
    }
    __builtin_amdgcn_sched_barrier(0);
    if (rc29_next && !s.isY) { s0 = fr_mul_c29(unscale29, s0); const fr_t y = fr_pow5_r29<PF>(fr_add<PF>(s0, rc_next[0])); s.sto(0, recode_next ? recode_signed(y) : y); }
    blk8_lane_rows<NLX>(s, Tb, b, last, rc29_next, recode_next);
}

template <int T>
__device__ __forceinline__ fr_t pair_lane_update(const uint32_t* sp, int j, const fr_t& base, const fr29_t& x0, const fr29_t& x1, const fr29_t& x2, const fr29_t& x3) {
    constexpr int W = 2 * T - 1;
    fr_wide29 u; fr_wide29_zero(u);
    fr_wide29_mac(u, c29(sp, 0 * W + T - 1 + j), x0); fr_wide29_mac(u, c29(sp, 1 * W + T - 1 + j), x1);
    fr_wide29_mac(u, c29(sp, 2 * W + T - 1 + j), x2); fr_wide29_mac(u, c29(sp, 3 * W + T - 1 + j), x3);
    return fr_add<PF>(base, fr_wide29_reduce_lazy<PF>(u));
}

template <int T, bool BLK8 = false, bool FUSE = BLK8>
__device__ __forceinline__ fr_t pair_permute(const PairState& s, const PoseidonDev& P, bool only0, int r_begin = 0) {
    static_assert(!BLK8 || T == 17, "8-round blocks exist for t = 17");
    static_assert(!FUSE || BLK8, "the fused hand-over belongs to the 8-round form");
    typedef PairCfg<T> Cfg;
    constexpr int NXD = Cfg::NXD, NXU = Cfg::NXU, W = 2 * T - 1;
    const int half = P.rf / 2;
    if constexpr (FUSE) {
        if (r_begin < half) pair_sbox_full<T, true>(s, P.rc_full + r_begin * T);
        for (int r = r_begin; r < half; ++r)
            pair_mds_sbox_mfma(s, (r == half - 1) ? P.mds_pre_frag : P.mds_frag, (r == half - 1) ? nullptr : c29(P.rc_full29, (size_t)(r + 1) * T), true);
    } else
    for (int r = r_begin; r < half; ++r) {
        if constexpr (T == 17) { pair_sbox_full<T, true>(s, P.rc_full + r * T); pair_mds_sbox_mfma(s, (r == half - 1) ? P.mds_pre_frag : P.mds_frag, nullptr, true); }
        else { pair_sbox_full<T>(s, P.rc_full + r * T); pair_apply_lu<T>(s, (r == half - 1) ? P.lu_pre29 : P.lu29); }
    }
    fr_t s0 = fr_zero<PF>();
    if (!s.isY) s0 = s.ld(0);
    if constexpr (BLK8) {
        for (int j = s.isY ? 9 : 1; j <= (s.isY ? 16 : 8); ++j) s.sto(j, recode_signed(s.ld(j)));
        __syncthreads();
        const int nb = P.rp / 8;
#pragma unroll 1
        for (int b = 0; b < nb; ++b) {
            const Blk8Tabs Tb{reinterpret_cast<const mfma_v4i*>(P.blk8_efrag) + (size_t)b * 8 * 16 * 64, reinterpret_cast<const mfma_v4i*>(P.blk8_lfrag) + (size_t)b * 16 * 8 * 64,
                              reinterpret_cast<const mfma_v4i*>(P.blk8_unit_frag), reinterpret_cast<const mfma_v4i*>(P.blk8_gfrag) + (size_t)b * 28 * 64,
                              P.rc_partial_scaled + 8 * b};
            if constexpr (FUSE) pair_block8<Blk8Cfg::NLX>(s, Tb, s0, b == nb - 1, b == nb - 1 ? c29(P.rc_full29, (size_t)half * T) : nullptr, P.rc_full + half * T, !(only0 && half == P.rf - 1), P.blk8_unscale29());
            else pair_block8<Blk8Cfg::NLX>(s, Tb, s0, b == nb - 1);
        }
        if constexpr (!FUSE) { if (!s.isY) s0 = fr_mul_c29(P.blk8_unscale29(), s0); }
    } else
    for (int b = 0; b < P.rp / 4; ++b) {
        const uint32_t* sp = c29(P.sparse29, (size_t)(4 * b) * W);
        const uint32_t* g = c29(P.gamma29, (size_t)b * 6);
        if (!s.isY) {
            fr_t keep[NXD];
#pragma unroll
            for (int j = 0; j < NXD; ++j) keep[j] = s.ld(1 + j);
            __syncthreads();
#define STARK_PAIR_ROUND(q)                                                                           \
            {                                                                                         \
                __builtin_amdgcn_sched_barrier(0);                      \
                const fr_t xq = fr_pow5_r29<PF>(fr_add<PF>(s0, P.rc_partial[4 * b + q]));              \
                s.sto(Cfg::xslot(q), xq);                                                             \
                fr_wide29 acc; fr_wide29_zero(acc);                                                   \
                fr_wide29_mac(acc, c29(sp, q * W), fr29_unpack(xq));                                  \
                if (q > 0) fr_wide29_mac(acc, c29(g, q * (q - 1) / 2 + 0), fr29_unpack(s.ld(Cfg::xslot(0)))); \
                if (q > 1) fr_wide29_mac(acc, c29(g, q * (q - 1) / 2 + 1), fr29_unpack(s.ld(Cfg::xslot(1)))); \
                if (q > 2) fr_wide29_mac(acc, c29(g, q * (q - 1) / 2 + 2), fr29_unpack(s.ld(Cfg::xslot(2)))); \
                if (1 + q + NXD > fr29_max_terms<PF>()) fr_wide29_norm(acc);    \
                _Pragma("unroll") for (int j = 0; j < NXD; ++j) fr_wide29_mac(acc, c29(sp, q * W + 1 + j), fr29_unpack(keep[j])); \
                const fr_t part = fr_wide29_reduce<PF>(acc);                                          \
                __syncthreads();                                        \
                s0 = fr_add<PF>(part, s.ld(Cfg::dslot(q)));                                           \
            }
            STARK_PAIR_ROUND(0) STARK_PAIR_ROUND(1) STARK_PAIR_ROUND(2) STARK_PAIR_ROUND(3)
#undef STARK_PAIR_ROUND
            const fr29_t x0 = fr29_unpack(s.ld(Cfg::xslot(0))), x1 = fr29_unpack(s.ld(Cfg::xslot(1))), x2 = fr29_unpack(s.ld(Cfg::xslot(2))), x3 = fr29_unpack(s.ld(Cfg::xslot(3)));
#pragma unroll
            for (int j = 1; j <= NXD; ++j) { __builtin_amdgcn_sched_barrier(0); s.sto(j, pair_lane_update<T>(sp, j, keep[j - 1], x0, x1, x2, x3)); }
#pragma unroll 1
            for (int j = NXD + 1; j <= NXU; ++j) s.sto(j, pair_lane_update<T>(sp, j, s.ld(j), x0, x1, x2, x3));
        } else {
            __syncthreads();
            for (int q = 0; q < 4; ++q) {
                DotAcc acc; acc.init();
#pragma unroll 1
                for (int j = NXD + 1; j < T; ++j) acc.mac(c29(sp, q * W + j), s.ld(j));
                const fr_t dy = acc.finish();
                s.sto(Cfg::dslot(q), dy);
                __syncthreads();
            }
            const fr29_t x0 = fr29_unpack(s.ld(Cfg::xslot(0))), x1 = fr29_unpack(s.ld(Cfg::xslot(1))), x2 = fr29_unpack(s.ld(Cfg::xslot(2))), x3 = fr29_unpack(s.ld(Cfg::xslot(3)));
#pragma unroll 1
            for (int j = NXU + 1; j < T; ++j) s.sto(j, pair_lane_update<T>(sp, j, s.ld(j), x0, x1, x2, x3));
        }
        __syncthreads();
    }
    if constexpr (!FUSE) {
        if (!s.isY) s.sto(0, s0);
        __syncthreads();
    }
    for (int r = half; r < P.rf; ++r) {
        const bool squeeze = only0 && r == P.rf - 1;
        if constexpr (FUSE) {  }
        else if constexpr (T == 17) { if (squeeze) pair_sbox_full<T>(s, P.rc_full + r * T); else pair_sbox_full<T, true>(s, P.rc_full + r * T); }
        else pair_sbox_full<T>(s, P.rc_full + r * T);
        if (squeeze) {
            const int j0 = s.isY ? Cfg::NX : 0, j1 = s.isY ? T : Cfg::NX;
            DotAcc acc; acc.init();
#pragma unroll 1
            for (int j = j0; j < j1; ++j) acc.mac(c29(P.row0_29, j), s.ld(j));
            s.sto(T + (s.isY ? 1 : 0), acc.finish());
            __syncthreads();
            fr_t out = fr_add<PF>(s.ld(T + 0), s.ld(T + 1));
            __syncthreads();
            return out;
        }
        if constexpr (FUSE) pair_mds_sbox_mfma(s, P.mds_frag, r == P.rf - 1 ? nullptr : c29(P.rc_full29, (size_t)(r + 1) * T), !(only0 && r + 1 == P.rf - 1));
        else if constexpr (T == 17) pair_mds_sbox_mfma(s, P.mds_frag, nullptr, true); else pair_apply_lu<T>(s, P.lu29);
    }
    return s.ld(0);
}

__device__ __forceinline__ PairState pair_setup(uint4* lds) {
    PairState s; s.st = lds; s.lane = threadIdx.x & 63;
    s.isY = __builtin_amdgcn_readfirstlane((int)(threadIdx.x >> 6)) != 0;
    return s;
}

template <bool BLK8>
__global__ void __launch_bounds__(128) __attribute__((amdgpu_waves_per_eu(2))) k_leaf_pair2(PoseidonDev P, const fr_t* __restrict__ leafc, const fr_t* __restrict__ f,
                                                    const fr_t* __restrict__ f_next, size_t n, size_t m, fr_t* __restrict__ h) {
    extern __shared__ uint4 lds[];
    PairState s = pair_setup(lds);
    const size_t i = (size_t)blockIdx.x * 64 + s.lane; const bool live = i < n; const size_t ii = live ? i : n - 1;
    const fr_t x4 = fr_pow5_r29<PF>(fr_add<PF>(ldg(f + ii), P.rc_full[4]));
    const fr_t x5 = fr_pow5_r29<PF>(fr_add<PF>(f_next ? ldg(f_next + ii / m) : fr_zero<PF>(), P.rc_full[5]));
    const int j0 = s.isY ? PairCfg<17>::NX : 0, j1 = s.isY ? 17 : PairCfg<17>::NX;
    const uint32_t* m45 = reinterpret_cast<const uint32_t*>(leafc + 51);
    const fr29_t x4u = fr29_unpack(x4), x5u = fr29_unpack(x5);
    for (int j = j0; j < j1; ++j) {
        fr_wide29 w; fr_wide29_zero(w);
        fr_wide29_mac(w, c29(m45, j), x4u); fr_wide29_mac(w, c29(m45, 17 + j), x5u);
        s.sto(j, fr_add<PF>(leafc[j], fr_wide29_reduce<PF>(w)));
    }
    __syncthreads();
    fr_t out = pair_permute<17, BLK8>(s, P, true, 1);
    if (live && !s.isY) stg(h + i, out);
}

template <int T, class DS, bool BLK8 = false>
__global__ void __launch_bounds__(128) __attribute__((amdgpu_waves_per_eu(2))) k_hash_ds2(PoseidonDev P, DS D, fr_t* __restrict__ out) {
    extern __shared__ uint4 lds[];
    constexpr int rate = T - 1;
    PairState s = pair_setup(lds);
    const size_t k0 = (size_t)blockIdx.x * 64 + s.lane; const bool live = k0 < D.n_out; const size_t k = live ? k0 : D.n_out - 1;
    const int o0 = s.isY ? PairCfg<T>::NX : 0, o1 = s.isY ? T : PairCfg<T>::NX;
    for (int j = o0; j < o1; ++j) s.sto(j, fr_zero<PF>());
    __syncthreads();
    const size_t total = D.total(k), nperm = (total + rate - 1) / rate;
    const size_t max_perm = (D.max_total() + rate - 1) / rate;
    const size_t skip = max_perm - nperm;
    size_t q = 0; fr_t res = fr_zero<PF>();
    for (size_t pidx = 0; pidx < max_perm; ++pidx) {
        if (pidx >= skip) {
            if (skip && pidx == skip) for (int j = o0; j < o1; ++j) s.sto(j, fr_zero<PF>());
            for (int cur = 0; cur < rate && q < total; ++cur, ++q) {
                if (cur < o0 || cur >= o1) continue;
                s.sto(cur, fr_add<PF>(s.ld(cur), D.elem(k, q)));
            }
        }
        __syncthreads();
        res = pair_permute<T, BLK8, false>(s, P, pidx + 1 == max_perm);
        __syncthreads();
    }
    if (live && !s.isY) stg(out + k0, res);
}

template <bool BLK8>
__global__ void __launch_bounds__(128) __attribute__((amdgpu_waves_per_eu(2))) k_node16_pair(PoseidonDev P, fr_t arity_f, fr_t level_f, fr_t label_f, uint64_t pos0,
                                                    const fr_t* __restrict__ in, size_t n_out, fr_t* __restrict__ out) {
    extern __shared__ uint4 lds[];
    PairState s = pair_setup(lds);
    const size_t k0 = (size_t)blockIdx.x * 64 + s.lane; const bool live = k0 < n_out; const size_t k = live ? k0 : n_out - 1;
    const fr_t* c = in + k * 16;
    static_assert(PairCfg<17>::NX == 8, "X fills elements 0..7");
    if (!s.isY) {
        s.sto(0, arity_f); s.sto(1, level_f); s.sto(2, fr_from_u64<PF>(pos0 + k)); s.sto(3, label_f);
#pragma unroll
        for (int j = 4; j < 8; ++j) s.sto(j, ldg(c + (j - 4)));
    } else {
#pragma unroll
        for (int j = 8; j < 16; ++j) s.sto(j, ldg(c + (j - 4)));
        s.sto(16, fr_zero<PF>());
    }
    __syncthreads();
    pair_permute<17, BLK8>(s, P, false);
    if (!s.isY) {
#pragma unroll
        for (int j = 0; j < 4; ++j) s.sto(j, fr_add<PF>(s.ld(j), ldg(c + 12 + j)));
        s.sto(4, fr_add<PF>(s.ld(4), fr_one<PF>()));
    }
// ... 8 lines not shown
```

stark_mlwe_amd/csrc/poseidon_params.hpp:

```cpp
#pragma once
#include "fr.hpp"
namespace stark {
struct PoseidonDev {
    int t, rf, rp;
    const fr_t* rc_full;
    const fr_t* rc_partial;
    const fr_t* lu;
    const fr_t* lu_pre;
    const fr_t* row0;
    const fr_t* sparse;
    const fr_t* mds;
    const fr_t* mds_pre;
    const fr_t* gamma;
    const uint32_t* lu29; const uint32_t* lu_pre29; const uint32_t* row0_29; const uint32_t* sparse29; const uint32_t* gamma29;
    const uint32_t* mds29; const uint32_t* mds_pre29;
    const void* mds_frag; const void* mds_pre_frag;
    const uint32_t* chain_a; const uint32_t* chain_g; const uint32_t* chain_w;
    const void* blk8_efrag; const void* blk8_lfrag; const void* blk8_unit_frag; const void* blk8_gfrag;
    const fr_t* rc_partial_scaled;
    FR_HD const uint32_t* blk8_unscale29() const { return reinterpret_cast<const uint32_t*>(rc_partial_scaled + rp); }
    const uint32_t* rc_full29;
};

}
```

Measured before the change: 11.71 million trace rows/s.

## Keep Poseidon block-8 partial-round state in lazy radix-29 form

The block-8 partial-round chain now carries the state as unreduced 29-bit limbs. Round constants are prestored in radix-29 and folded into the MFMA column sums. Each round does a lazy pow5 and adds the packed slot without a full modular reduction or pack/unpack. The lane-row outputs of non-final blocks are finished straight to recoded digits. This shortens the serial dependency chain of partial rounds, but it relies on lazy-limb bound invariants that the added host checks try to validate.

```diff
diff --git a/stark_mlwe_amd/csrc/capi_core.hip b/stark_mlwe_amd/csrc/capi_core.hip
--- a/stark_mlwe_amd/csrc/capi_core.hip
+++ b/stark_mlwe_amd/csrc/capi_core.hip
@@ -105,15 +105,15 @@
     const size_t o_frag = blob.size(), frag_elems = (k.mds_frag.size() + sizeof(fr_t) - 1) / sizeof(fr_t);
     if (!k.mds_frag.empty()) { blob.resize(o_frag + 2 * frag_elems); memcpy((void*)(blob.data() + o_frag), k.mds_frag.data(), k.mds_frag.size()); memcpy((void*)(blob.data() + o_frag + frag_elems), k.mds_pre_frag.data(), k.mds_pre_frag.size()); }
     const size_t o_b8 = blob.size(), ef_elems = (k.blk8s_efrag.size() + sizeof(fr_t) - 1) / sizeof(fr_t), lf_bytes = k.blk8s_lfrag.size() + 1024, lf_elems = (lf_bytes + sizeof(fr_t) - 1) / sizeof(fr_t),
-                 gf_elems = (k.blk8s_gfrag.size() + sizeof(fr_t) - 1) / sizeof(fr_t), rcs_elems = k.rc_partial_scaled.size(), un_elems = (k.blk8_unscale29.size() * 4 + sizeof(fr_t) - 1) / sizeof(fr_t);
+                 gf_elems = (k.blk8s_gfrag.size() + sizeof(fr_t) - 1) / sizeof(fr_t), rcs_words = k.rc_partial_scaled29.size(), un_elems = ((rcs_words + k.blk8_unscale29.size()) * 4 + sizeof(fr_t) - 1) / sizeof(fr_t);
     const bool have_b8 = !k.blk8s_efrag.empty();
-    if (have_b8) { blob.resize(o_b8 + ef_elems + lf_elems + gf_elems + rcs_elems + un_elems);
+    if (have_b8) { blob.resize(o_b8 + ef_elems + lf_elems + gf_elems + un_elems);
                    int8_t* const b8 = (int8_t*)(blob.data() + o_b8);
                    memcpy(b8, k.blk8s_efrag.data(), k.blk8s_efrag.size());
                    memcpy(b8 + ef_elems * sizeof(fr_t), k.blk8s_lfrag.data(), k.blk8s_lfrag.size()); memcpy(b8 + ef_elems * sizeof(fr_t) + k.blk8s_lfrag.size(), k.blk8_lfrag.data() + k.blk8_lfrag.size() - 1024, 1024);
                    memcpy(b8 + (ef_elems + lf_elems) * sizeof(fr_t), k.blk8s_gfrag.data(), k.blk8s_gfrag.size());
-                   memcpy(b8 + (ef_elems + lf_elems + gf_elems) * sizeof(fr_t), k.rc_partial_scaled.data(), rcs_elems * sizeof(fr_t));
-                   memcpy(b8 + (ef_elems + lf_elems + gf_elems + rcs_elems) * sizeof(fr_t), k.blk8_unscale29.data(), k.blk8_unscale29.size() * 4); }
+                   memcpy(b8 + (ef_elems + lf_elems + gf_elems) * sizeof(fr_t), k.rc_partial_scaled29.data(), rcs_words * 4);
+                   memcpy(b8 + (ef_elems + lf_elems + gf_elems) * sizeof(fr_t) + rcs_words * 4, k.blk8_unscale29.data(), k.blk8_unscale29.size() * 4); }
     STARK_TRY(P->blob.fill_sync(ctx, blob.data(), blob.size() * sizeof(fr_t)));
     fr_t* const dev = P->blob.fr();
     P->dev.t = k.t; P->dev.rf = k.rf; P->dev.rp = k.rp;
@@ -129,7 +129,7 @@
     P->dev.blk8_efrag = have_b8 ? (const void*)(dev + o_b8) : nullptr; P->dev.blk8_lfrag = have_b8 ? (const void*)(dev + o_b8 + ef_elems) : nullptr;
     P->dev.blk8_gfrag = have_b8 ? (const void*)(dev + o_b8 + ef_elems + lf_elems) : nullptr;
     P->dev.blk8_unit_frag = have_b8 ? (const void*)((const int8_t*)P->dev.blk8_lfrag + k.blk8s_lfrag.size()) : nullptr;
-    P->dev.rc_partial_scaled = have_b8 ? dev + o_b8 + ef_elems + lf_elems + gf_elems : nullptr;
+    P->dev.rc_partial_scaled29 = have_b8 ? reinterpret_cast<const uint32_t*>(dev + o_b8 + ef_elems + lf_elems + gf_elems) : nullptr;
     P->dev.mds_frag = k.mds_frag.empty() ? nullptr : (const void*)(dev + o_frag); P->dev.mds_pre_frag = k.mds_frag.empty() ? nullptr : (const void*)(dev + o_frag + frag_elems);
     return STARK_OK;
 }
diff --git a/stark_mlwe_amd/csrc/capi_poseidon.hip b/stark_mlwe_amd/csrc/capi_poseidon.hip
--- a/stark_mlwe_amd/csrc/capi_poseidon.hip
+++ b/stark_mlwe_amd/csrc/capi_poseidon.hip
@@ -211,7 +211,7 @@
 }
 static int32_t pair_block8_form(stark_ctx* ctx, const stark_params* p, bool* on) {
     *on = ctx->opt.poseidon_block8 && p->dev.t == 17 && p->dev.rp % 8 == 0;
-    if (*on && (!p->dev.blk8_efrag || !p->dev.blk8_lfrag || !p->dev.blk8_unit_frag || !p->dev.blk8_gfrag || !p->dev.rc_partial_scaled)) return ctx->fail(STARK_ERR_UNSUPPORTED, "poseidon_block8: the parameter set has no block-8 tables");
+    if (*on && (!p->dev.blk8_efrag || !p->dev.blk8_lfrag || !p->dev.blk8_unit_frag || !p->dev.blk8_gfrag || !p->dev.rc_partial_scaled29)) return ctx->fail(STARK_ERR_UNSUPPORTED, "poseidon_block8: the parameter set has no block-8 tables");
     return STARK_OK;
 }
 template <class DS>
diff --git a/stark_mlwe_amd/csrc/fr29.hpp b/stark_mlwe_amd/csrc/fr29.hpp
--- a/stark_mlwe_amd/csrc/fr29.hpp
+++ b/stark_mlwe_amd/csrc/fr29.hpp
@@ -98,8 +98,7 @@
     for (int i = 0; i < 8; ++i) z.v[i] = t[i];
     return z;
 }
-template <class F> FR_HD fr_t fr_wide29_reduce_lazy(fr_wide29& w) {
-    uint32_t l[9]; fr_wide29_mont<F>(w, l);
+FR_HD fr_t fr29_pack(const uint32_t* l) {
     fr_t z;
 #pragma unroll
     for (int wd = 0; wd < 8; ++wd) {
@@ -111,6 +110,19 @@
     }
     return z;
 }
+template <class F> FR_HD fr_t fr_wide29_reduce_lazy(fr_wide29& w) {
+    uint32_t l[9]; fr_wide29_mont<F>(w, l);
+    fr_t z;
+#pragma unroll
+    for (int wd = 0; wd < 8; ++wd) {
+        const int lo = 32 * wd, i = lo / 29, s = lo - 29 * i;
+        uint32_t v = l[i] >> s;
+        if (i + 1 < 9) v |= l[i + 1] << (29 - s);
+        if (29 - s + 29 < 32 && i + 2 < 9) v |= l[i + 2] << (58 - s);
+        z.v[wd] = v;
+    }
+    return z;
+}
 template <class F, bool MAC_POW2 = false> FR_HD fr_t fr_wide29_reduce(fr_wide29& w) {
     uint32_t l[9]; fr_wide29_mont<F, MAC_POW2>(w, l);
     return fr29_pack_reduce<F>(l);
diff --git a/stark_mlwe_amd/csrc/host_util.hpp b/stark_mlwe_amd/csrc/host_util.hpp
--- a/stark_mlwe_amd/csrc/host_util.hpp
+++ b/stark_mlwe_amd/csrc/host_util.hpp
@@ -178,7 +178,7 @@
     std::vector<uint32_t> gamma8_29;
     std::vector<fr_t> blk8_lambda, rc_partial_scaled;
     std::vector<int8_t> blk8s_efrag, blk8s_lfrag, blk8s_gfrag;
-    std::vector<uint32_t> blk8_unscale29;
+    std::vector<uint32_t> blk8_unscale29, rc_partial_scaled29;
     bool ok = false;
 };
 template <class Pred> inline std::vector<uint32_t> to_radix29(const std::vector<fr_t>& v, Pred scaled) {
@@ -283,6 +283,8 @@
             k.blk8_lambda[q + 1] = h_mul(l5k, a_inv); yinv[q] = fr_inv<PF>(l5k);
             k.rc_partial_scaled[q] = h_mul(k.blk8_lambda[q], c.rc_partial[q]);
         }
+        k.rc_partial_scaled29.assign((size_t)(c.rp + 1) * 9, 0u);
+        for (int q = 0; q < c.rp; ++q) { const fr29_t u = fr29_unpack(k.rc_partial_scaled[q]); for (int j = 0; j < 9; ++j) k.rc_partial_scaled29[(size_t)9 * q + j] = u.l[j]; }
         k.blk8_unscale29.resize(9); fr29_const_from<PF>(fr_inv<PF>(k.blk8_lambda[c.rp]), k.blk8_unscale29.data());
         for (int b = 0; b < nb; ++b) {
             for (int q = 0; q < 8; ++q) for (int j = 1; j < t; ++j) {
diff --git a/stark_mlwe_amd/csrc/hostcheck.cpp b/stark_mlwe_amd/csrc/hostcheck.cpp
--- a/stark_mlwe_amd/csrc/hostcheck.cpp
+++ b/stark_mlwe_amd/csrc/hostcheck.cpp
@@ -43,7 +43,7 @@
     P->dev.t = P->kc.t; P->dev.rf = P->kc.rf; P->dev.rp = P->kc.rp; P->dev.rc_full = P->kc.rc_full.data(); P->dev.rc_partial = P->kc.rc_partial.data();
     P->dev.lu = P->kc.lu.data(); P->dev.lu_pre = P->kc.lu_pre.data(); P->dev.row0 = P->kc.row0.data(); P->dev.sparse = P->kc.sparse.data(); P->dev.mds = P->kc.mds.data(); P->dev.mds_pre = P->kc.mds_pre.data(); P->dev.gamma = P->kc.gamma.data();
     P->dev.lu29 = P->kc.lu29.data(); P->dev.lu_pre29 = P->kc.lu_pre29.data(); P->dev.row0_29 = P->kc.row0_29.data(); P->dev.sparse29 = P->kc.sparse29.data(); P->dev.gamma29 = P->kc.gamma29.data(); P->dev.mds29 = P->kc.mds29.data(); P->dev.mds_pre29 = P->kc.mds_pre29.data(); P->dev.rc_full29 = P->kc.rc_full29.data();
-    P->dev.mds_frag = nullptr; P->dev.mds_pre_frag = nullptr; P->dev.blk8_efrag = nullptr; P->dev.blk8_lfrag = nullptr; P->dev.blk8_unit_frag = nullptr; P->dev.blk8_gfrag = nullptr; P->dev.rc_partial_scaled = nullptr;
+    P->dev.mds_frag = nullptr; P->dev.mds_pre_frag = nullptr; P->dev.blk8_efrag = nullptr; P->dev.blk8_lfrag = nullptr; P->dev.blk8_unit_frag = nullptr; P->dev.blk8_gfrag = nullptr; P->dev.rc_partial_scaled29 = nullptr;
     P->dev.chain_a = P->kc.chain_a.empty() ? nullptr : P->kc.chain_a.data(); P->dev.chain_g = P->kc.chain_g.empty() ? nullptr : P->kc.chain_g.data(); P->dev.chain_w = P->kc.chain_w.empty() ? nullptr : P->kc.chain_w.data();
 }
 
@@ -250,7 +250,7 @@
             const int8_t* fr[17]; for (int e = 0; e < t; ++e) fr[e] = &F[((size_t)i * t + e) * 1024];
             int32_t S[32]; const int rc = blk8_tile_sums(fr, xd.data(), t, S); if (rc) return rc;
             if (next < 0) o[i] = blk8_finish_sums(S);
-            else { uint32_t l[9]; blk8_finish_sums_limbs(S, l); o[i] = recode_signed(sbox_lazy29(l, &k.rc_full29[((size_t)next * t + i) * 9])); }
+            else { uint32_t l[9]; blk8_finish_sums_limbs(S, l); o[i] = sbox_lazy29_recoded(l, &k.rc_full29[((size_t)next * t + i) * 9]); }
         }
         if (next < 0) st = o; else xd = o;
         return 0; };
@@ -258,7 +258,8 @@
         for (int j = 0; j < t; ++j) st[j] = ld4(states + 4 * (s * t + j));
         sbox(0);
         for (int r = 0; r < half; ++r) { const int rc = product(r == half - 1 ? k.mds_pre_frag : k.mds_frag, r == half - 1 ? -1 : r + 1); if (rc) return rc; }
-        fr_t s0 = st[0], rec[17], y[8], yd[9], kx[23];
+        fr_t rec[17], yd[9], kx[23];
+        fr29_t u = lazy29_add_c29(fr29_unpack(st[0]).l, &k.rc_partial_scaled29[0]);
         for (int j = 1; j < t; ++j) rec[j] = recode_signed(st[j]);
         const int nb = k.rp / 8;
         for (int b = 0; b < nb; ++b) {
@@ -271,26 +272,74 @@
                 int32_t S[32]; { const int rc = blk8_tile_sums(fr, kx, 16 + q, S); if (rc) return rc; }
                 if (q == 7) { int32_t m = 0; for (int c = 0; c < 32; ++c) m = std::max(m, S[c] < 0 ? -S[c] : S[c]);
                               int32_t seen = g_blk8_row23_max.load(); while (m > seen && !g_blk8_row23_max.compare_exchange_weak(seen, m)) {} }
-                const fr_t H = blk8_finish_sums(S);
-                y[q] = fr_pow5_r29<PF>(fr_add<PF>(s0, k.rc_partial_scaled[8 * b + q]));
-                yd[q] = recode_signed(y[q]);
-                s0 = fr_add<PF>(y[q], H);
+                int64_t col[9]; uint32_t l[9]; mfma_cols_of_sums(S, col, &k.rc_partial_scaled29[(size_t)9 * (8 * b + q + 1)]); mfma_finish_limbs(col, l);
+                const fr_t slot = lazy29_to_slot(l);
+                const fr29_t x5 = pow5_lazy29(u);
+                yd[q] = recode_lazy29(x5);
+                u = lazy29_add_slot(x5, slot);
+                for (int i = 0; i < 9; ++i) if (u.l[i] >= (1u << 30)) return -4;
             }
             for (int j = 1; j < t; ++j) {
                 const int8_t* fr[9]; for (int p2 = 0; p2 < 8; ++p2) fr[p2] = lf + ((size_t)(j - 1) * 8 + p2) * 1024; fr[8] = unit;
                 yd[8] = rec[j];
                 if (b == nb - 1) {
                     int32_t S[32]; { const int rc = blk8_tile_sums(fr, yd, 9, S); if (rc) return rc; }
-                    uint32_t l[9]; blk8_finish_sums_limbs(S, l); xd[j] = recode_signed(sbox_lazy29(l, &k.rc_full29[((size_t)half * t + j) * 9]));
-                } else { fr_t z; { const int rc = blk8_tile(fr, yd, 9, z); if (rc) return rc; } rec[j] = recode_signed(z); }
+                    uint32_t l[9]; blk8_finish_sums_limbs(S, l); xd[j] = sbox_lazy29_recoded(l, &k.rc_full29[((size_t)half * t + j) * 9]);
+                } else { int32_t S[32]; { const int rc = blk8_tile_sums(fr, yd, 9, S); if (rc) return rc; } int64_t col[9]; mfma_cols_of_sums(S, col); rec[j] = mfma_finish_recoded(col); }
             }
         }
-        s0 = fr_mul_c29(k.blk8_unscale29.data(), s0);
-        xd[0] = recode_signed(fr_pow5_r29<PF>(fr_add<PF>(s0, k.rc_full[(size_t)half * t])));
+        const fr29_t x0 = fr29_mul_c29(k.blk8_unscale29.data(), u);
+        xd[0] = sbox_lazy29_recoded(x0.l, &k.rc_full29[((size_t)half * t) * 9]);
         for (int r = half; r < k.rf; ++r) { const int rc = product(k.mds_frag, r == k.rf - 1 ? -1 : r + 1); if (rc) return rc; }
         for (int j = 0; j < t; ++j) st4(states + 4 * (s * t + j), st[j]);
     }
     return 0;
+}
+int hc_mfma_finish_limbs_c(const int32_t* sums, const uint32_t* c, size_t n, uint32_t* limbs, uint32_t* slots) {
+    for (size_t s = 0; s < n; ++s) {
+        const int32_t* S = sums + 32 * s; const uint32_t* cs = c + 9 * s;
+        for (int i = 0; i < 32; ++i) if (S[i] >= (1 << 24) || S[i] <= -(1 << 24)) return -1;
+        for (int i = 0; i < 9; ++i) if (cs[i] >= (i < 8 ? 1u << 29 : 1u << 23)) return -1;
+        int64_t col[9]; mfma_cols_of_sums(S, col, cs);
+        mfma_finish_limbs(col, limbs + 9 * s);
+        const fr_t z = lazy29_to_slot(limbs + 9 * s);
+        memcpy(slots + 8 * s, z.v, 32);
+    }
+    return 0;
+}
+void hc_lazy29_add_slot(const uint32_t* x5, const uint32_t* slots, size_t n, uint32_t* u) {
+    for (size_t s = 0; s < n; ++s) { fr29_t a; fr_t z; memcpy(a.l, x5 + 9 * s, 36); memcpy(z.v, slots + 8 * s, 32); const fr29_t r = lazy29_add_slot(a, z); memcpy(u + 9 * s, r.l, 36); }
+}
+void hc_recode_lazy29(const uint32_t* x5, size_t n, int8_t* digits) {
+    for (size_t s = 0; s < n; ++s) { fr29_t a; memcpy(a.l, x5 + 9 * s, 36); const fr_t d = recode_lazy29(a); memcpy(digits + 32 * s, d.v, 32); }
+}
+int hc_chain_census(const uint32_t* u, size_t n, uint32_t* x245, uint64_t* colmax, uint8_t* topbyte) {
+    static const uint32_t zero9[9] = {0, 0, 0, 0, 0, 0, 0, 0, 0};
+    for (size_t s = 0; s < n; ++s) {
+        fr29_t a; memcpy(a.l, u + 9 * s, 36);
+        for (int i = 0; i < 9; ++i) if (a.l[i] >= (1u << 30)) return -1;
+        Lazy29Wide wide; const fr29_t x5w = wide.pow5(a.l, zero9);
+        const fr29_t x5 = pow5_lazy29(a);
+        colmax[2 * s] = (uint64_t)wide.max_col; colmax[2 * s + 1] = (uint64_t)(wide.max_col >> 64);
+        if ((wide.max_col >> 64) == 0 && memcmp(x5.l, x5w.l, 36) != 0) return -2;
+        memcpy(x245 + 27 * s, wide.x2.l, 36); memcpy(x245 + 27 * s + 9, wide.x4.l, 36); memcpy(x245 + 27 * s + 18, x5w.l, 36);
+        topbyte[s] = (uint8_t)(fr29_pack(x5w.l).v[7] >> 24);
+    }
+    return 0;
+}
+int hc_mfma_finish_recoded(const int32_t* sums, size_t n, uint32_t* limbs, int8_t* digits) {
+    for (size_t s = 0; s < n; ++s) {
+        const int32_t* S = sums + 32 * s;
+        for (int i = 0; i < 32; ++i) if (S[i] >= (1 << 24) || S[i] <= -(1 << 24)) return -1;
+        int64_t col[9]; mfma_cols_of_sums(S, col); mfma_finish_limbs_floor(col, limbs + 9 * s);
+        mfma_cols_of_sums(S, col); const fr_t d = mfma_finish_recoded(col); memcpy(digits + 32 * s, d.v, 32);
+    }
+    return 0;
+}
+size_t hc_rc_partial_scaled29_table(void* h, uint32_t* out, size_t cap) {
+    const std::vector<uint32_t>& v = ((HcParams*)h)->kc.rc_partial_scaled29;
+    if (out && !v.empty()) memcpy(out, v.data(), std::min(cap, v.size()) * 4);
+    return v.size();
 }
 size_t hc_blk8_table(void* h, int which, void* out, size_t cap) {
     HcParams* P = (HcParams*)h; const host::KernelConsts& k = P->kc;
diff --git a/stark_mlwe_amd/csrc/mfma_digits.hpp b/stark_mlwe_amd/csrc/mfma_digits.hpp
--- a/stark_mlwe_amd/csrc/mfma_digits.hpp
+++ b/stark_mlwe_amd/csrc/mfma_digits.hpp
@@ -46,7 +46,11 @@
     fr_cond_sub<PF>(z.v, 0u);
     return z;
 }
-FR_HD fr_t sbox_lazy29(const uint32_t* l, const uint32_t* __restrict__ c_) {
+FR_HD fr29_t pow5_lazy29(const fr29_t& u) {
+    const fr29_t x2 = fr29_sqr_mont<PF>(u), x4 = fr29_sqr_mont<PF>(x2);
+    return fr29_mul_mont<PF>(u, x4);
+}
+FR_HD fr29_t lazy29_add_c29(const uint32_t* l, const uint32_t* __restrict__ c_) {
 #if defined(__HIP_DEVICE_COMPILE__)
     typedef const __attribute__((address_space(4))) uint32_t* cptr_t;
     cptr_t c = (cptr_t)c_;
@@ -56,15 +60,56 @@
     fr29_t u;
 #pragma unroll
     for (int i = 0; i < 9; ++i) u.l[i] = l[i] + c[i];
-    const fr29_t x2 = fr29_sqr_mont<PF>(u), x4 = fr29_sqr_mont<PF>(x2), x5 = fr29_mul_mont<PF>(u, x4);
-    return fr29_pack_reduce<PF>(x5.l);
+    return u;
 }
+FR_HD fr_t sbox_lazy29(const uint32_t* l, const uint32_t* __restrict__ c) { return fr29_pack_reduce<PF>(pow5_lazy29(lazy29_add_c29(l, c)).l); }
+FR_HD void mfma_cols_set(int64_t* col, const uint32_t* __restrict__ c_) {
+#if defined(__HIP_DEVICE_COMPILE__)
+    typedef const __attribute__((address_space(4))) uint32_t* cptr_t;
+    cptr_t c = (cptr_t)c_;
+#else
+    const uint32_t* c = c_;
+#endif
+#pragma unroll
+    for (int k = 0; k < 9; ++k) col[k] = (int64_t)c[k];
+}
+FR_HD fr_t lazy29_to_slot(const uint32_t* l) {
+    fr_t z;
+#pragma unroll
+    for (int k = 0; k < 8; ++k) z.v[k] = l[k] | (((l[8] >> (3 * k)) & 7u) << 29);
+    return z;
+}
+FR_HD fr29_t lazy29_add_slot(const fr29_t& x5, const fr_t& slot) {
+    fr29_t u; uint32_t top = 0;
+#pragma unroll
+    for (int k = 0; k < 8; ++k) { u.l[k] = x5.l[k] + (slot.v[k] & FR_M29); top |= (slot.v[k] >> 29) << (3 * k); }
+    u.l[8] = x5.l[8] + top;
+    return u;
+}
+FR_HD fr_t recode_lazy29(const fr29_t& x5) { return recode_signed(fr29_pack(x5.l)); }
+FR_HD fr_t sbox_lazy29_recoded(const uint32_t* l, const uint32_t* __restrict__ c) { return recode_lazy29(pow5_lazy29(lazy29_add_c29(l, c))); }
+FR_HD void mfma_finish_limbs_floor(int64_t* col, uint32_t* l) {
+#pragma unroll
+    for (int k = 0; k < 8; ++k) { col[k + 1] += col[k] >> 29; l[k] = (uint32_t)col[k] & FR_M29; }
+    const int64_t top = col[8];
+    const int32_t q = (int32_t)(top >> 22);
+    l[8] = (uint32_t)top & ((1u << 22) - 1);
+    int64_t carry = 0;
+#pragma unroll
+    for (int i = 0; i < 5; ++i) { const int64_t d = (int64_t)l[i] - (int64_t)q * (int64_t)fr_p29<PF>(i) + carry; l[i] = (uint32_t)d & FR_M29; carry = d >> 29; }
+    int32_t c32 = (int32_t)carry;
+#pragma unroll
+    for (int i = 5; i < 9; ++i) { const int32_t d = (int32_t)l[i] + c32; if (i < 8) { l[i] = (uint32_t)d & FR_M29; c32 = d >> 29; } else l[8] = (uint32_t)d; }
+}
+FR_HD fr_t mfma_finish_recoded(int64_t* col) { uint32_t l[9]; mfma_finish_limbs_floor(col, l); return recode_signed(fr29_pack(l)); }
+FR_HD fr29_t fr29_mul_c29(const uint32_t* __restrict__ c, const fr29_t& u) { fr_wide29 w; fr_wide29_zero(w); fr_wide29_mac(w, c, u); fr29_t r; fr_wide29_mont<PF>(w, r.l); return r; }
 #if !defined(__HIP_DEVICE_COMPILE__)
-inline void mfma_cols_of_sums(const int32_t* S, int64_t* col) {
+inline void mfma_cols_of_sums(const int32_t* S, int64_t* col, const uint32_t* c29 = nullptr) {
     int32_t lo[16], hi[16];
     for (int reg = 0; reg < 16; ++reg) { const int row = (reg & 3) + 8 * (reg >> 2); lo[reg] = S[row]; hi[reg] = S[row + 4]; }
     for (int k = 0; k < 9; ++k) col[k] = 0;
     mfma_fold_rows(col, lo, hi);
+    if (c29) { int64_t cc[9]; mfma_cols_set(cc, c29); for (int k = 0; k < 9; ++k) col[k] += cc[k]; }
 }
 struct Lazy29Wide {
     typedef unsigned __int128 u128;
@@ -91,8 +136,9 @@
     }
     fr29_t pow5(const uint32_t* l, const uint32_t* c) {
         fr29_t u; for (int i = 0; i < 9; ++i) u.l[i] = l[i] + c[i];
-        const fr29_t x2 = sqr(u), x4 = sqr(x2); return mul(u, x4);
+        x2 = sqr(u); x4 = sqr(x2); return mul(u, x4);
     }
+    fr29_t x2, x4;
 };
 #endif
 
diff --git a/stark_mlwe_amd/csrc/poseidon_pair.hpp b/stark_mlwe_amd/csrc/poseidon_pair.hpp
--- a/stark_mlwe_amd/csrc/poseidon_pair.hpp
+++ b/stark_mlwe_amd/csrc/poseidon_pair.hpp
@@ -76,15 +76,18 @@
 #pragma unroll
         for (int r = 0; r < 16; ++r) acc[ct][r] = 0;
 }
-__device__ __forceinline__ void mfma_post_cols(const mfma_v16i (&acc)[2], int64_t* col) {
+__device__ __forceinline__ void mfma_post_cols(const mfma_v16i (&acc)[2], int64_t* col, const uint32_t* c29 = nullptr) {
     mfma_v16i lo, hi;
 #pragma unroll
     for (int r = 0; r < 16; ++r) {
         const auto sw = __builtin_amdgcn_permlane32_swap((unsigned)acc[0][r], (unsigned)acc[1][r], false, false);
         lo[r] = (int)sw[0]; hi[r] = (int)sw[1];
     }
-#pragma unroll
-    for (int k = 0; k < 9; ++k) col[k] = 0;
+    if (c29) mfma_cols_set(col, c29);
+    else {
+#pragma unroll
+        for (int k = 0; k < 9; ++k) col[k] = 0;
+    }
     mfma_fold_rows(col, lo, hi);
 }
 __device__ __forceinline__ fr_t mfma_post(const mfma_v16i (&acc)[2]) {
@@ -93,8 +96,8 @@
     return mfma_finish_cols(col);
 }
 __device__ __forceinline__ void pair_sto_sbox29(const PairState& s, int j, const uint32_t* l, const uint32_t* rc29, bool recode) {
-    const fr_t y = sbox_lazy29(l, rc29);
-    s.sto(j, recode ? recode_signed(y) : y);
+    const fr29_t x5 = pow5_lazy29(lazy29_add_c29(l, rc29));
+    s.sto(j, recode ? recode_lazy29(x5) : fr29_pack_reduce<PF>(x5.l));
 }
 __device__ __forceinline__ void pair_mds_sbox_mfma(const PairState& s, const void* frag, const uint32_t* rc29, bool recode) {
     constexpr int T = 17;
@@ -130,7 +133,7 @@
     const mfma_v4i* lfrag;
     const mfma_v4i* unit;
     const mfma_v4i* gfrag;
-    const fr_t* rc;
+    const uint32_t* rc29;
 };
 struct Blk8Cfg {
     static constexpr int NLX = 8;
@@ -146,12 +149,12 @@
     return mfma_v4i{(int)u.x, (int)u.y, (int)u.z, (int)u.w};
 }
 template <int Q>
-__device__ __forceinline__ void blk8_round_x(const PairState& s, const Blk8Tabs& Tb, fr_t& s0, mfma_v4i (&b)[8][2]) {
+__device__ __forceinline__ void blk8_round_x(const PairState& s, const Blk8Tabs& Tb, fr29_t& u, mfma_v4i (&b)[8][2]) {
     __builtin_amdgcn_sched_barrier(0);
-    const fr_t y = fr_pow5_r29<PF>(fr_add<PF>(s0, Tb.rc[Q]));
-    s.sto(Blk8Cfg::ymail(Q), recode_signed(y));
-    __syncthreads();
-    s0 = fr_add<PF>(y, s.ld(Blk8Cfg::hmail(Q)));
+    const fr29_t x5 = pow5_lazy29(u);
+    s.sto(Blk8Cfg::ymail(Q), recode_lazy29(x5));
+    __syncthreads();
+    u = lazy29_add_slot(x5, s.ld(Blk8Cfg::hmail(Q)));
     b[Q][0] = blk8_b_of_slot(s, Blk8Cfg::ymail(Q), 0); b[Q][1] = blk8_b_of_slot(s, Blk8Cfg::ymail(Q), 1);
 }
 template <int Q>
@@ -175,11 +178,11 @@
 #pragma unroll
         for (int p = 0; p <= Q; ++p) g[p] = (Tb.gfrag + (size_t)((Q + 1) * Q / 2 + p) * 64)[lane];
     }
-    s.sto(Blk8Cfg::hmail(Q), mfma_post(acc));
+    { int64_t col[9]; uint32_t l[9]; mfma_post_cols(acc, col); { int64_t cc[9]; mfma_cols_set(cc, c29(Tb.rc29, Q)); _Pragma("unroll") for (int k = 0; k < 9; ++k) col[k] += cc[k]; } mfma_finish_limbs(col, l); s.sto(Blk8Cfg::hmail(Q), lazy29_to_slot(l)); }
     __syncthreads();
     b[Q][0] = blk8_b_of_slot(s, Blk8Cfg::ymail(Q), 0); b[Q][1] = blk8_b_of_slot(s, Blk8Cfg::ymail(Q), 1);
 }
-template <int NLX>
+template <int NLX, bool LAZY = false>
 __device__ __forceinline__ void blk8_lane_rows(const PairState& s, const Blk8Tabs& Tb, const mfma_v4i (&b)[8][2], bool last, const uint32_t* rc29_next = nullptr, bool recode_next = true) {
     static_assert(NLX >= 1 && NLX <= 15, "shares");
     const int lane = s.lane;
@@ -202,17 +205,18 @@
 #pragma unroll
         for (int p = 0; p < 8; ++p) a[p] = (Tb.lfrag + ((size_t)(jn - 1) * 8 + p) * 64)[lane];
         if (rc29_next) { int64_t col[9]; uint32_t l[9]; mfma_post_cols(acc, col); mfma_finish_limbs(col, l); pair_sto_sbox29(s, j, l, c29(rc29_next, j), recode_next); }
+        else if (LAZY && !last) { int64_t col[9]; mfma_post_cols(acc, col); s.sto(j, mfma_finish_recoded(col)); }
         else { const fr_t z = mfma_post(acc); s.sto(j, last ? z : recode_signed(z)); }
     }
     __syncthreads();
 }
-template <int NLX>
-__device__ __forceinline__ void pair_block8(const PairState& s, const Blk8Tabs& Tb, fr_t& s0, bool last, const uint32_t* rc29_next = nullptr, const fr_t* rc_next = nullptr, bool recode_next = true,
+template <int NLX, bool LAZY = false>
+__device__ __forceinline__ void pair_block8(const PairState& s, const Blk8Tabs& Tb, fr29_t& u, bool last, const uint32_t* rc29_next = nullptr, bool recode_next = true,
                                             const uint32_t* unscale29 = nullptr) {
     mfma_v4i b[8][2];
     if (!s.isY) {
-        blk8_round_x<0>(s, Tb, s0, b); blk8_round_x<1>(s, Tb, s0, b); blk8_round_x<2>(s, Tb, s0, b); blk8_round_x<3>(s, Tb, s0, b);
-        blk8_round_x<4>(s, Tb, s0, b); blk8_round_x<5>(s, Tb, s0, b); blk8_round_x<6>(s, Tb, s0, b); blk8_round_x<7>(s, Tb, s0, b);
+        blk8_round_x<0>(s, Tb, u, b); blk8_round_x<1>(s, Tb, u, b); blk8_round_x<2>(s, Tb, u, b); blk8_round_x<3>(s, Tb, u, b);
+        blk8_round_x<4>(s, Tb, u, b); blk8_round_x<5>(s, Tb, u, b); blk8_round_x<6>(s, Tb, u, b); blk8_round_x<7>(s, Tb, u, b);
     } else {
         mfma_v4i a[16], g[7];
         blk8_load_frags16(a, Tb.efrag, s.lane);
@@ -220,8 +224,8 @@
         blk8_round_y<4>(s, Tb, b, a, g); blk8_round_y<5>(s, Tb, b, a, g); blk8_round_y<6>(s, Tb, b, a, g); blk8_round_y<7>(s, Tb, b, a, g);
     }
     __builtin_amdgcn_sched_barrier(0);
-    if (rc29_next && !s.isY) { s0 = fr_mul_c29(unscale29, s0); const fr_t y = fr_pow5_r29<PF>(fr_add<PF>(s0, rc_next[0])); s.sto(0, recode_next ? recode_signed(y) : y); }
-    blk8_lane_rows<NLX>(s, Tb, b, last, rc29_next, recode_next);
+    if (rc29_next && !s.isY) { const fr29_t x = fr29_mul_c29(unscale29, u); pair_sto_sbox29(s, 0, x.l, c29(rc29_next, 0), recode_next); }
+    blk8_lane_rows<NLX, LAZY>(s, Tb, b, last, rc29_next, recode_next);
 }
 
 template <int T>
@@ -252,6 +256,8 @@
     fr_t s0 = fr_zero<PF>();
     if (!s.isY) s0 = s.ld(0);
     if constexpr (BLK8) {
+        fr29_t u = fr29_unpack(s0);
+        if (!s.isY) u = lazy29_add_c29(u.l, c29(P.rc_partial_scaled29, 0));
         for (int j = s.isY ? 9 : 1; j <= (s.isY ? 16 : 8); ++j) s.sto(j, recode_signed(s.ld(j)));
         __syncthreads();
         const int nb = P.rp / 8;
@@ -259,11 +265,11 @@
         for (int b = 0; b < nb; ++b) {
             const Blk8Tabs Tb{reinterpret_cast<const mfma_v4i*>(P.blk8_efrag) + (size_t)b * 8 * 16 * 64, reinterpret_cast<const mfma_v4i*>(P.blk8_lfrag) + (size_t)b * 16 * 8 * 64,
                               reinterpret_cast<const mfma_v4i*>(P.blk8_unit_frag), reinterpret_cast<const mfma_v4i*>(P.blk8_gfrag) + (size_t)b * 28 * 64,
-                              P.rc_partial_scaled + 8 * b};
-            if constexpr (FUSE) pair_block8<Blk8Cfg::NLX>(s, Tb, s0, b == nb - 1, b == nb - 1 ? c29(P.rc_full29, (size_t)half * T) : nullptr, P.rc_full + half * T, !(only0 && half == P.rf - 1), P.blk8_unscale29());
-            else pair_block8<Blk8Cfg::NLX>(s, Tb, s0, b == nb - 1);
+                              c29(P.rc_partial_scaled29, (size_t)8 * b + 1)};
+            if constexpr (FUSE) pair_block8<Blk8Cfg::NLX, true>(s, Tb, u, b == nb - 1, b == nb - 1 ? c29(P.rc_full29, (size_t)half * T) : nullptr, !(only0 && half == P.rf - 1), P.blk8_unscale29());
+            else pair_block8<Blk8Cfg::NLX>(s, Tb, u, b == nb - 1);
         }
-        if constexpr (!FUSE) { if (!s.isY) s0 = fr_mul_c29(P.blk8_unscale29(), s0); }
+        if constexpr (!FUSE) { if (!s.isY) s0 = fr29_pack_reduce<PF>(fr29_mul_c29(P.blk8_unscale29(), u).l); }
     } else
     for (int b = 0; b < P.rp / 4; ++b) {
         const uint32_t* sp = c29(P.sparse29, (size_t)(4 * b) * W);
diff --git a/stark_mlwe_amd/csrc/poseidon_params.hpp b/stark_mlwe_amd/csrc/poseidon_params.hpp
--- a/stark_mlwe_amd/csrc/poseidon_params.hpp
+++ b/stark_mlwe_amd/csrc/poseidon_params.hpp
@@ -17,8 +17,8 @@
     const void* mds_frag; const void* mds_pre_frag;
     const uint32_t* chain_a; const uint32_t* chain_g; const uint32_t* chain_w;
     const void* blk8_efrag; const void* blk8_lfrag; const void* blk8_unit_frag; const void* blk8_gfrag;
-    const fr_t* rc_partial_scaled;
-    FR_HD const uint32_t* blk8_unscale29() const { return reinterpret_cast<const uint32_t*>(rc_partial_scaled + rp); }
+    const uint32_t* rc_partial_scaled29;
+    FR_HD const uint32_t* blk8_unscale29() const { return rc_partial_scaled29 + (size_t)(rp + 1) * 9; }
     const uint32_t* rc_full29;
 };
 
```

Measured after the change: 12.09 million trace rows/s (median of 6 runs). 3.2% higher.
